# KarypisLab/SLIM

Measured on AMD Instinct MI355X. Metric: item-columns solved/sec (whole node), higher is better.
Workload: dtype f32

## Files before the change

### slim_amd/csrc/cd_gramr.hpp

```cpp
#pragma once
#include <utility>

#include "cd_tile.hpp"
#include "gram_pack.hpp"

#ifndef SLIM_GRAMR_AUX
#define SLIM_GRAMR_AUX 0
#endif
#ifndef SLIM_GRAMR_PROF
#define SLIM_GRAMR_PROF 0
#endif
#ifndef SLIM_GRAMR_FROM_PLANES
#define SLIM_GRAMR_FROM_PLANES 1
#endif
#ifndef SLIM_GRAMR_PREFETCH
#define SLIM_GRAMR_PREFETCH 0
#endif
#ifndef SLIM_GRAMR_LATE_GATHERS
#define SLIM_GRAMR_LATE_GATHERS 1
#endif
#ifndef SLIM_GRAMR_DRAIN
#define SLIM_GRAMR_DRAIN 0
#endif
#ifndef SLIM_GRAMR_SYNCROW
#define SLIM_GRAMR_SYNCROW 0
#endif

namespace slimamd {

typedef float gramr_v16 __attribute__((ext_vector_type(16)));

template <int N>
struct GramrRegs {
  gramr_v16 v;
  GramrRegs<N - 1> rest;
};
template <>
struct GramrRegs<0> {};
template <int I, int N>
__device__ __forceinline__ gramr_v16& gramr_reg(GramrRegs<N>& r) {
  if constexpr (I == 0) return r.v;
  else return gramr_reg<I - 1>(r.rest);
}
template <class F, int... Is>
__device__ __forceinline__ void static_for_impl(F&& f, std::integer_sequence<int, Is...>) {
  (f(std::integral_constant<int, Is>{}), ...);
}
template <int N, class F>
__device__ __forceinline__ void static_for(F&& f) {
  static_for_impl(f, std::make_integer_sequence<int, N>{});
}

template <int N, int KRA>
__device__ __forceinline__ float gramr_sel_from(GramrRegs<KRA>& gr, const int k, const int e) {
  if (k == N) {
    const gramr_v16 t = gramr_reg<N>(gr);
    asm volatile("" ::"v"(t));
    return t[e];
  }
  if constexpr (N + 1 < KRA) return gramr_sel_from<N + 1, KRA>(gr, k, e);
  return 0.0f;
}
template <int KRA>
__device__ __forceinline__ float gramr_sel(GramrRegs<KRA>& gr, const int k, const int e) {
  return gramr_sel_from<0, KRA>(gr, k, e);
}

#ifndef SLIM_GRAMR_ASMEXPORT
#define SLIM_GRAMR_ASMEXPORT 1
#endif
#define SLIM_GRAMR_EXPORT_ASM                                   \
  "s_mov_b32 %[sm0], m0\n\t"                                   \
  "s_mov_b64 %[sx], exec\n"                                     \
  "1:\n\t"                                                      \
  "s_ff1_i32_b64 %[sb], %[mine]\n\t"                            \
  "v_readlane_b32 %[sr], %[r], %[sb]\n\t"                       \
  "s_bitset0_b64 %[mine], %[sb]\n\t"                            \
  "s_bfe_u32 %[sl], %[sr], 0x60004\n\t"                         \
  "s_lshr_b32 %[sidx], %[sr], 13\n\t"                           \
  "s_and_b32 %[sr], %[sr], 15\n\t"                              \
  "s_lshl4_add_u32 %[sidx], %[sidx], %[sr]\n\t"                 \
  "s_set_gpr_idx_on %[sidx], gpr_idx(SRC0)\n\t"                 \
  "v_mov_b32 %[vt], v16\n\t"                                    \
  "s_set_gpr_idx_off\n\t"                                       \
  "v_readlane_b32 %[sv], %[vt], %[sl]\n\t"                      \
  "s_lshl_b64 exec, 1, %[sb]\n\t"                               \
  "v_mov_b32 %[res], %[sv]\n\t"                                 \
  "s_mov_b64 exec, %[sx]\n\t"                                   \
  "s_cmp_lg_u64 %[mine], 0\n\t"                                 \
  "s_cbranch_scc1 1b\n\t"                                       \
  "s_mov_b32 m0, %[sm0]\n"
#define SLIM_GRAMR_EXPORT_OUT                                                                           \
  [res] "+v"(res), [mine] "+s"(mine), [sb] "=&s"(sb), [sr] "=&s"(sr), [sl] "=&s"(sl), [sidx] "=&s"(sidx), \
      [sv] "=&s"(sv), [vt] "=&v"(vt), [sm0] "=&s"(sm0), [sx] "=&s"(sx)
template <int KRA>
__device__ __forceinline__ float gramr_export(GramrRegs<KRA>& gr, const int r, uint64_t mine) {
  float res = 0.0f, vt;
  int sb, sr, sl, sidx, sm0;
  float sv;
  uint64_t sx;
  static_assert(KRA == 1 || KRA == 3 || KRA == 6 || KRA == 10, "one operand list per instantiation");
  if constexpr (KRA == 1) {
    asm volatile(SLIM_GRAMR_EXPORT_ASM : SLIM_GRAMR_EXPORT_OUT : [r] "v"(r), "{v[16:31]}"(gramr_reg<0>(gr)) : "scc");
  } else if constexpr (KRA == 3) {
    asm volatile(SLIM_GRAMR_EXPORT_ASM
                 : SLIM_GRAMR_EXPORT_OUT
                 : [r] "v"(r), "{v[16:31]}"(gramr_reg<0>(gr)), "{v[32:47]}"(gramr_reg<1>(gr)),
                   "{v[48:63]}"(gramr_reg<2>(gr))
                 : "scc");
  } else if constexpr (KRA == 6) {
    asm volatile(SLIM_GRAMR_EXPORT_ASM
                 : SLIM_GRAMR_EXPORT_OUT
                 : [r] "v"(r), "{v[16:31]}"(gramr_reg<0>(gr)), "{v[32:47]}"(gramr_reg<1>(gr)),
                   "{v[48:63]}"(gramr_reg<2>(gr)), "{v[64:79]}"(gramr_reg<3>(gr)), "{v[80:95]}"(gramr_reg<4>(gr)),
                   "{v[96:111]}"(gramr_reg<5>(gr))
                 : "scc");
  } else {
    asm volatile(SLIM_GRAMR_EXPORT_ASM
                 : SLIM_GRAMR_EXPORT_OUT
                 : [r] "v"(r), "{v[16:31]}"(gramr_reg<0>(gr)), "{v[32:47]}"(gramr_reg<1>(gr)),
                   "{v[48:63]}"(gramr_reg<2>(gr)), "{v[64:79]}"(gramr_reg<3>(gr)), "{v[80:95]}"(gramr_reg<4>(gr)),
                   "{v[96:111]}"(gramr_reg<5>(gr)), "{v[112:127]}"(gramr_reg<6>(gr)),
                   "{v[128:143]}"(gramr_reg<7>(gr)), "{v[144:159]}"(gramr_reg<8>(gr)),
                   "{v[160:175]}"(gramr_reg<9>(gr))
                 : "scc");
  }
  return res;
}

constexpr int gramr_ring_bytes(int ah) { return (kGramrNT / 64) * (ah + 2) * 1024; }
constexpr int kGramrHdr = 1280;
constexpr int kGramrDump = SLIM_GRAMR_PREFETCH ? 256 : 0;
constexpr int gramr_hdr_bytes() { return (kGramrNT / 64) * (2 * kGramrHdr + kGramrDump); }

template <int KR, int KL, bool DMA = false, int WPS = ((KR <= 2 && KL == 0) ? 4 : 2), int AH = 2>
__global__ __launch_bounds__(kGramrNT, WPS) void cd_gramr_kernel(
    const DevMatrix A, const SolveArgs S, const GramPacked P) {
  constexpr int NT = kGramrNT, K = KR + KL;
  constexpr int kGramrAhead = AH, kGramrSlots = AH + 2;
  constexpr int KRA = KR > 0 ? KR : 1;
  constexpr int R0 = KR * kPackGroup;
  static_assert(KR <= 12, "register select covers 12 groups");
  static_assert(KR + KL <= 16, "one base byte per group in a 16-byte load");
  extern __shared__ __attribute__((aligned(16))) float g_lds[];
  __shared__ float s_gB[2][64];
  __shared__ int s_p, s_na;
  __shared__ unsigned long long s_D;
  __shared__ double s_e2[64], s_reg[64];
  __shared__ unsigned long long s_off;
  __shared__ int s_nz;

  const int tid = threadIdx.x;
  const int lane = tid & 63;
  const int wave = uni(tid >> 6);
  const int ncols = A.ncols;
#if !SLIM_GRAMR_FROM_PLANES
  const int n4 = S.ncols_pad >> 2;
#endif
  const int nchunks = P.nchunks;
  const float l1 = S.l1, l2 = S.l2;
#if !SLIM_GRAMR_FROM_PLANES
  const float* __restrict__ Gm = S.G;
  const int64_t ld = S.G_ld;
#endif
  float* const x = S.xslab + (int64_t)blockIdx.x * S.x_stride;
#if !SLIM_GRAMR_FROM_PLANES
  float4* const x4 = reinterpret_cast<float4*>(x);
#endif
  float4* const gl4 = reinterpret_cast<float4*>(g_lds);
  const int64_t* __restrict__ colptr = A.colptr;

  GramrRegs<KRA> gr;

  const uint32_t voff0 = 16u * (uint32_t)tid;
  const uint32_t vlast = 16u * (uint32_t)(nchunks - 1);
#if SLIM_GRAMR_DRAIN
#define SLIM_VMCNT(n) __builtin_amdgcn_s_waitcnt(0 | (7 << 4) | (15 << 8))
#else
#define SLIM_VMCNT(n) __builtin_amdgcn_s_waitcnt(((n) & 15) | (((n) >> 4) << 14) | (7 << 4) | (15 << 8))
#endif
  char* const ring_w = reinterpret_cast<char*>(g_lds) + KL * kPackGroup * 4 + wave * (kGramrSlots * 1024);
#if SLIM_GRAMR_PROF
  unsigned long long pt_first_v = 0, pt_mark_v = 0, pt_export_v = 0, pt_mark = 0;
  unsigned long long* const pt_first_p = &pt_first_v;
  unsigned long long* const pt_mark_p = &pt_mark_v;
#endif
  char* const hdr_w = reinterpret_cast<char*>(g_lds) + KL * kPackGroup * 4 + (DMA ? gramr_ring_bytes(AH) : 0) +
                      wave * (2 * kGramrHdr + kGramrDump);
  char* const dump_w = hdr_w + 2 * kGramrHdr;
  auto apply = [&](const uint8_t* __restrict__ plo, const uint8_t* __restrict__ phi,
                   const uint8_t* __restrict__ ph2, const uint8_t* __restrict__ pbase, const int hk,
                   const int h2k, const int cdiag, const int ediag, const float vdiag,
                   const float nd, const int rg, uint32_t (&gq)[4],
                   const uint8_t* __restrict__ plo_next) __attribute__((always_inline)) {
    const bool gin1 = rg < hk * kPackGroup, gin2 = rg < h2k * kPackGroup;
    auto gathers = [&]() __attribute__((always_inline)) {
      gq[0] = __hip_atomic_load(plo + rg, __ATOMIC_RELAXED, __HIP_MEMORY_SCOPE_WAVEFRONT);
      gq[1] = __hip_atomic_load(phi + (gin1 ? rg : 0), __ATOMIC_RELAXED, __HIP_MEMORY_SCOPE_WAVEFRONT);
      gq[2] = __hip_atomic_load(ph2 + (gin2 ? rg : 0), __ATOMIC_RELAXED, __HIP_MEMORY_SCOPE_WAVEFRONT);
      gq[3] = __hip_atomic_load(pbase + (((rg >> 4) & (NT - 1)) * 16 + (rg >> 13)), __ATOMIC_RELAXED,
                                __HIP_MEMORY_SCOPE_WAVEFRONT);
    };
    if constexpr (!(DMA && SLIM_GRAMR_LATE_GATHERS)) gathers();
    const int kdiag = cdiag / NT, tdiag = cdiag % NT;
    uint32_t bwords[4];
    if constexpr (DMA) {
      uint32_t vzb = voff0;
      asm volatile("" : "+v"(vzb));
      __builtin_amdgcn_global_load_lds(pbase + vzb, ring_w + (kGramrAhead + 1) * 1024, 16, 0, 0);
    } else {
      const uint4 bw = ld_off<uint4>(pbase, voff0);
      bwords[0] = bw.x;
      bwords[1] = bw.y;
      bwords[2] = bw.z;
      bwords[3] = bw.w;
    }
    auto consume = [&](auto kc, const uint4 lo, auto&& hi_of) __attribute__((always_inline)) {
      constexpr int k = decltype(kc)::value;
      float f[16];
      unpack16(lo, f);
      {
        typedef float gramr_v2 __attribute__((ext_vector_type(2)));
        const float bf = 16.0f * (float)((bwords[(k >> 2) & 3] >> (8 * (k & 3))) & 255u);
#pragma unroll
        for (int e = 0; e < 16; e += 2) {
          gramr_v2 v = {f[e], f[e + 1]};
          asm volatile("" : "+v"(v));
          v += (gramr_v2)(bf);
          f[e] = v.x;
          f[e + 1] = v.y;
        }
      }
      if (k < hk) {
        unpack16_add(hi_of(), 256.0f, f);
        if (k < h2k) {
          uint32_t vz = voff0;
          asm volatile("" : "+v"(vz));
          const uint32_t vo = min(vz + (uint32_t)(kPackGroup * k), vlast);
          unpack16_add(ld_off<uint4>(ph2, vo), 65536.0f, f);
        }
      }
      if (k == kdiag && tid == tdiag) {
#pragma unroll
        for (int e = 0; e < 16; ++e) f[e] = e == ediag ? vdiag : f[e];
      }
      if constexpr (k < KR) {
        gramr_v16& g = gramr_reg<k>(gr);
#pragma unroll
        for (int e = 0; e < 16; ++e) g[e] = fmaf(nd, f[e], g[e]);
        asm volatile("" : "+v"(g));
      } else {
        float4* const gp = gl4 + (k - KR) * 4 * NT + tid;
#pragma unroll
        for (int j = 0; j < 4; ++j) {
          float4 v = gp[j * NT];
          v.x = fmaf(nd, f[4 * j + 0], v.x);
          v.y = fmaf(nd, f[4 * j + 1], v.y);
          v.z = fmaf(nd, f[4 * j + 2], v.z);
          v.w = fmaf(nd, f[4 * j + 3], v.w);
          gp[j * NT] = v;
        }
      }
    };
    if constexpr (DMA) {
      constexpr int S = kGramrAhead + 1;
      uint4 h01[2];
      static_for<2>([&](auto kc) __attribute__((always_inline)) {
        constexpr int k = decltype(kc)::value;
        if constexpr (k < K) {
          if (k < hk) h01[k] = ld_off<uint4>(phi, min(voff0 + (uint32_t)(kPackGroup * k), vlast));
        }
      });
      auto request = [&](auto kc) __attribute__((always_inline)) {
        constexpr int k = decltype(kc)::value;
        uint32_t vz = voff0;
        asm volatile("" : "+v"(vz));
        const uint32_t vo = min(vz + (uint32_t)(kPackGroup * k), vlast);
        __builtin_amdgcn_global_load_lds(plo + vo, ring_w + (k % S) * 1024, 16, 0, SLIM_GRAMR_AUX);
      };
      static_for<(kGramrAhead < K ? kGramrAhead : K)>([&](auto kc) __attribute__((always_inline)) { request(kc); });
      constexpr int kLate = (SLIM_GRAMR_LATE_GATHERS ? 4 : 0) + (SLIM_GRAMR_PREFETCH ? 1 : 0);
      if constexpr (SLIM_GRAMR_LATE_GATHERS) gathers();
      if constexpr (SLIM_GRAMR_PREFETCH) {
        const int ln = lane < 8 * kGramrAhead ? lane : 0;
        const uint32_t po = min((uint32_t)(kPackGroup * (ln >> 3)) + 1024u * (uint32_t)wave + 128u * (uint32_t)(ln & 7), vlast);
        __builtin_amdgcn_global_load_lds(plo_next + po, dump_w, 4, 0, 0);
      }
      static_for<K>([&](auto kc) __attribute__((always_inline)) {
        constexpr int k = decltype(kc)::value;
        if constexpr (k + kGramrAhead < K) request(std::integral_constant<int, k + kGramrAhead>{});
        constexpr int ahead = (K - 1 - k) < kGramrAhead ? (K - 1 - k) : kGramrAhead;
        SLIM_VMCNT(ahead + (k < kGramrAhead ? kLate : 0));
        asm volatile("" ::: "memory");
        if constexpr (k == 0) {
          const uint4 bw = *reinterpret_cast<const uint4*>(ring_w + (kGramrAhead + 1) * 1024 + lane * 16);
          bwords[0] = bw.x;
          bwords[1] = bw.y;
          bwords[2] = bw.z;
          bwords[3] = bw.w;
        }
#if SLIM_GRAMR_PROF
        if constexpr (k == 0) *pt_first_p += __builtin_readcyclecounter() - *pt_mark_p;
#endif
        const uint4 lo = *reinterpret_cast<const uint4*>(ring_w + (k % S) * 1024 + lane * 16);
        consume(kc, lo, [&]() __attribute__((always_inline)) -> uint4 {
          if constexpr (k < 2) return h01[k];
          else {
            uint32_t vz = voff0;
            asm volatile("" : "+v"(vz));
            return ld_off<uint4>(phi, min(vz + (uint32_t)(kPackGroup * k), vlast));
          }
        });
        __builtin_amdgcn_sched_barrier(0);
      });
    } else {
      constexpr int GRP = 4;
      static_for<(K + GRP - 1) / GRP>([&](auto k0c) __attribute__((always_inline)) {
        constexpr int k0 = decltype(k0c)::value * GRP;
        uint4 l[GRP], h[GRP];
        static_for<GRP>([&](auto uc) __attribute__((always_inline)) {
          constexpr int u = decltype(uc)::value, k = k0 + u;
          if constexpr (k < K) {
            const uint32_t vo = min(voff0 + (uint32_t)(kPackGroup * k), vlast);
            l[u] = ld_off<uint4>(plo, vo);
            if (k < hk) h[u] = ld_off<uint4>(phi, vo);
          }
        });
        __builtin_amdgcn_sched_barrier(0);
        static_for<GRP>([&](auto uc) __attribute__((always_inline)) {
          constexpr int u = decltype(uc)::value, k = k0 + u;
          if constexpr (k < K)
            consume(std::integral_constant<int, k>{}, l[u], [&]() __attribute__((always_inline)) -> uint4 { return h[u]; });
          __builtin_amdgcn_sched_barrier(0);
        });
      });
    }
  };
#undef SLIM_VMCNT
  int nrows_read = 0, nhi16_read = 0;
  auto lds_index = [&](const int r) __attribute__((always_inline)) -> int {
    const int rr = r - R0;
    const int kk = rr >> 13, t = (rr >> 4) & (NT - 1), e = rr & 15;
    return ((kk * 4 + (e >> 2)) * NT + t) * 4 + (e & 3);
  };

  int gb_par = 0;
  auto fetch_g = [&](const bool want, const int r) __attribute__((always_inline)) -> float {
    float* const gb = s_gB[gb_par];
    gb_par ^= 1;
    const bool in_lds = r >= R0;
    const bool my_wave = (((r >> 4) & (NT - 1)) >> 6) == wave;
    if (KR > 0) {
      uint64_t mine = __ballot(want && !in_lds && my_wave);
#if SLIM_GRAMR_ASMEXPORT
      if (mine) {
        const bool own = want && !in_lds && my_wave;
        const float res = gramr_export<KRA>(gr, r, mine);
        if (own) gb[lane] = res;
      }
#else
      while (mine) {
        const int b = __builtin_ctzll(mine);
        mine &= mine - 1ull;
        const int rb = lane_bcast(r, b);
        const float v = gramr_sel<KRA>(gr, rb >> 13, rb & 15);
        if (lane == ((rb >> 4) & 63)) gb[b] = v;
      }
#endif
    }
    if (KL > 0 && want && in_lds && my_wave) gb[lane] = g_lds[lds_index(r)];
#if SLIM_GRAMR_PROF
    pt_export_v += __builtin_readcyclecounter() - pt_mark;
#endif
    asm volatile("" ::: "memory");
    __builtin_amdgcn_s_waitcnt(15 | (7 << 4) | (0 << 8) | (3 << 14));
    __builtin_amdgcn_s_barrier();
    asm volatile("" ::: "memory");
    return gb[lane];
  };

  for (;;) {
    if (tid == 0) {
      s_p = atomicAdd(S.queue, 1);
      s_na = 0;
      s_D = 0;
    }
    __syncthreads();
    const int p = s_p;
    if (p >= S.nwork) break;
    const int item = uni(S.order[p]);
    const int grp = p >> 5;
    const uint32_t gkey = (uint32_t)(grp * S.shard_count + S.shard_index);
    const int* __restrict__ ul = S.ulist + (int64_t)grp * S.u_stride;
    const int nunion = uni(S.tile_nunion[grp]);
#if SLIM_GRAMR_FROM_PLANES
    uint4 irec;
    {
      const uint4 mr = P.meta[item];
      irec = make_uint4(uni(mr.x), uni(mr.y), uni(mr.z), uni(mr.w));
    }
#endif
#if !SLIM_GRAMR_FROM_PLANES
    const float* __restrict__ arow = Gm + (int64_t)item * ld;
#endif

#if SLIM_GRAMR_FROM_PLANES
    {
      const int hk0 = (int)((irec.x >> 17) & 15u), h2k0 = (int)((irec.x >> 21) & 15u);
      const uint8_t* __restrict__ plo0 = P.lo + (int64_t)item * P.ldb;
      const uint8_t* __restrict__ phi0 = P.hi + (int64_t)irec.y * kPackGroup;
      const uint8_t* __restrict__ ph20 = phi0 + (int64_t)hk0 * kPackGroup;
      const uint8_t* __restrict__ pb0 = P.base + (int64_t)item * kPackGroup;
      int na = 0;
      int64_t dact = 0;
      for (int c = tid; c < nchunks; c += NT) {
        const int kg = c / NT;
        float f[16];
        unpack16(*reinterpret_cast<const uint4*>(plo0 + 16 * (int64_t)c), f);
        const float bf = 16.0f * (float)pb0[(c & (NT - 1)) * 16 + kg];
#pragma unroll
        for (int e = 0; e < 16; ++e) f[e] += bf;
        if (kg < hk0) unpack16_add(*reinterpret_cast<const uint4*>(phi0 + 16 * (int64_t)c), 256.0f, f);
        if (kg < h2k0) unpack16_add(*reinterpret_cast<const uint4*>(ph20 + 16 * (int64_t)c), 65536.0f, f);
        const int4* __restrict__ io = reinterpret_cast<const int4*>(P.item_of + 16 * (int64_t)c);
#pragma unroll
        for (int j = 0; j < 4; ++j) {
          const int4 q = io[j];
          const int it[4] = {q.x, q.y, q.z, q.w};
#pragma unroll
          for (int u = 0; u < 4; ++u) {
            if (it[u] >= 0) {
              const bool act = it[u] != item && f[4 * j + u] > l1;
              x[it[u]] = act ? 0.0f : kInactive;
              if (act) {
                ++na;
                dact += (int64_t)P.meta[it[u]].z;
              }
            }
          }
        }
      }
      na = (int)wave_sum((float)na);
      if (lane == 0 && na) atomicAdd(&s_na, na);
      if (dact) atomicAdd(&s_D, (unsigned long long)dact);
    }
#else
    {
      const float4* __restrict__ a4 = reinterpret_cast<const float4*>(arow);
      int na = 0;
      int64_t dact = 0;
      for (int c = tid; c < n4; c += NT) {
        const float4 a = a4[c];
        const int i0 = c << 2;
        float4 xs;
        const bool a0 = i0 + 0 < ncols && i0 + 0 != item && a.x > l1;
        const bool a1 = i0 + 1 < ncols && i0 + 1 != item && a.y > l1;
        const bool a2 = i0 + 2 < ncols && i0 + 2 != item && a.z > l1;
        const bool a3 = i0 + 3 < ncols && i0 + 3 != item && a.w > l1;
        xs.x = a0 ? 0.0f : kInactive;
        xs.y = a1 ? 0.0f : kInactive;
        xs.z = a2 ? 0.0f : kInactive;
        xs.w = a3 ? 0.0f : kInactive;
        na += (int)a0 + (int)a1 + (int)a2 + (int)a3;
        x4[c] = xs;
        if (a0 | a1 | a2 | a3) {
          const int64_t c0 = colptr[i0], c1 = colptr[i0 + 1];
          const int64_t c2 = i0 + 2 <= ncols ? colptr[i0 + 2] : c1, c3 = i0 + 3 <= ncols ? colptr[i0 + 3] : c2;
          const int64_t c4 = i0 + 4 <= ncols ? colptr[i0 + 4] : c3;
          dact += (a0 ? c1 - c0 : 0) + (a1 ? c2 - c1 : 0) + (a2 ? c3 - c2 : 0) + (a3 ? c4 - c3 : 0);
        }
      }
      na = (int)wave_sum((float)na);
      if (lane == 0 && na) atomicAdd(&s_na, na);
      if (dact) atomicAdd(&s_D, (unsigned long long)dact);
    }
#endif
    int64_t fe = 0, we = 0;
    auto warm_x = [&]() __attribute__((always_inline)) {
      if (S.icolptr != nullptr && item < S.incols) {
        __syncthreads();
        fe = uni(S.icolptr[item]);
        we = uni(S.icolptr[item + 1]);
        for (int64_t e = fe + tid; e < we; e += NT) {
          const int k = S.icolind[e];
          if (k < ncols && tile_active(x[k])) {
            const float v = S.icolval[e];
            x[k] = v < 0.0f ? 0.0f : v;
          }
        }
      }
    };
    warm_x();
    constexpr bool kCarry = K <= kGramrCarryMaxGroups;
    const bool carried = kCarry && S.g_load != nullptr;
    if (carried) {
      const float4* __restrict__ gs = reinterpret_cast<const float4*>(S.g_load + (int64_t)item * S.g_stride);
      static_for<KRA>([&](auto kc) __attribute__((always_inline)) {
        constexpr int k = decltype(kc)::value;
        gramr_v16 v;
#pragma unroll
        for (int j = 0; j < 4; ++j) {
          const float4 q = gs[(k * NT + tid) * 4 + j];
          v[4 * j] = q.x; v[4 * j + 1] = q.y; v[4 * j + 2] = q.z; v[4 * j + 3] = q.w;
        }
        gramr_reg<k>(gr) = v;
      });
#pragma unroll
      for (int k = 0; k < KL; ++k)
#pragma unroll
        for (int j = 0; j < 4; ++j) gl4[(k * 4 + j) * NT + tid] = gs[((KRA + k) * NT + tid) * 4 + j];
    } else {
    static_for<KRA>([&](auto kc) __attribute__((always_inline)) {
      gramr_reg<decltype(kc)::value>(gr) = (gramr_v16)(0.0f);
    });
#pragma unroll
    for (int k = 0; k < KL; ++k)
#pragma unroll
      for (int j = 0; j < 4; ++j) gl4[(k * 4 + j) * NT + tid] = make_float4(0.f, 0.f, 0.f, 0.f);
    }
    __syncthreads();

    int maxit = 0;
    {
      const int64_t cap = 50 * (uni(colptr[item + 1]) - uni(colptr[item]));
      maxit = cap < (int64_t)S.maxniters ? (int)cap : S.maxniters;
    }
    int niters = 0, conv = 0;
    nrows_read = 0;
    nhi16_read = 0;

    if (wave == 0) {
      s_e2[lane] = 0.0;
      s_reg[lane] = 0.0;
    }
    int phase = 0;
    bool init_row = !carried;
    if (carried) fe = we;
    int t = 0, p0 = 0;
    float dlt = 0.0f;
    PermCtx pc = perm_make(1u, 0u);
    int i_a = 0;
    int i_n = 0;
    int hw = 0;
    auto header_a = [&](const int q0) __attribute__((always_inline)) {
      const int pos = q0 + lane;
      i_a = pos < nunion ? ul[perm_index(pc, (uint32_t)pos)] : -1;
    };
    auto header_b = [&]() __attribute__((always_inline)) {
      i_n = i_a < 0 ? 0 : i_a;
      char* const hb = hdr_w + hw * kGramrHdr;
      __builtin_amdgcn_global_load_lds(x + i_n, hb, 4, 0, 0);
      __builtin_amdgcn_global_load_lds(P.meta + i_n, hb + 256, 16, 0, 0);
      hw ^= 1;
    };
    int ib = 0, wpos = 0, nz = 0;
    unsigned long long off = 0;
    bool fits = false;
    unsigned long long Uu = 0;
#if SLIM_GRAMR_PROF
    unsigned long long pt_fetch = 0, pt_dec = 0, pt_apply = 0;
    pt_first_v = 0;
    pt_export_v = 0;
#define SLIM_PT(acc) { const unsigned long long now_ = __builtin_readcyclecounter(); acc += now_ - pt_mark; pt_mark = now_; }
#else
#define SLIM_PT(acc)
#endif

    for (;;) {
      bool want = false;
      int r = 0, i = 0;
      uint4 mrow = make_uint4(0u, 0u, 0u, 0u);
      float xi = kInactive;
      bool part = false, keep = false;
      uint64_t mkeep = 0;
      if (phase == 1) {
        i = i_n;
        __builtin_amdgcn_s_waitcnt(0 | (7 << 4) | (15 << 8));
        asm volatile("" ::: "memory");
        {
          const char* const hcur = hdr_w + (hw ^ 1) * kGramrHdr;
          const bool valid = p0 + lane < nunion;
          int lz = lane;
          asm volatile("" : "+v"(lz));
          const float xv = *reinterpret_cast<const float*>(hcur + lz * 4);
          mrow = *reinterpret_cast<const uint4*>(hcur + 256 + lz * 16);
          r = (int)(mrow.x & 0x1FFFFu);
          xi = valid ? xv : kInactive;
        }
        asm volatile("" ::: "memory");
        part = tile_active(xi);
        header_b();
        header_a(p0 + 128);
        want = part;
      } else if (phase == 2) {
        i = ib + lane;
        xi = i < ncols ? x[i] : kInactive;
        const bool act = tile_active(xi);
        keep = act && fabsf(xi) > kEps;
        if (act && wave == 0)
          s_reg[lane] += 0.5 * (double)l2 * (double)xi * (double)xi + (double)l1 * (double)fabsf(xi);
        mkeep = __ballot(keep);
        if (mkeep == 0) {
          ib += 64;
          if (ib >= ncols) break;
          continue;
        }
        r = keep ? (int)(P.meta[i].x & 0x1FFFFu) : 0;
        want = keep;
      }
#if SLIM_GRAMR_PROF
      pt_mark = __builtin_readcyclecounter();
#endif
      const float g0 = fetch_g(want, r);
      SLIM_PT(pt_fetch)
      float gi = g0;
      uint64_t pend = 0;
      if (phase == 1) {
        pend = __ballot(part);
      }
      for (;;) {
        int row = 0;
        float nd = 0.0f;
        uint4 rec = make_uint4(0u, 0u, 0u, 0u);
        if (phase == 0) {
          bool have = false;
          if (init_row) {
            row = item;
            nd = 1.0f;
            have = true;
          } else {
            while (fe < we) {
              const int kk = uni(S.icolind[fe]);
              ++fe;
              if (kk < ncols) {
                const float xk = uni(x[kk]);
                if (xk > kEps) {
                  row = kk;
                  nd = -xk;
                  have = true;
                  break;
                }
              }
            }
          }
          if (!have) break;
        } else if (phase == 1) {
          if (pend == 0) break;
          const float xeff = (xi > kEps || xi < -kEps) ? xi : 0.0f;
          const float sq = __uint_as_float(mrow.w);
          const float cn = sqrtf(sq);
          const float num = cd_num(gi, xeff, sq);
          const float nx = num > l1 ? (num - l1) / cd_den(cn, l2) : 0.0f;
          const float neff = (nx > kEps || nx < -kEps) ? nx : 0.0f;
          const float d = neff - xeff;
          const uint64_t m = __ballot(part && nx != xi) & pend;
          if (m == 0) break;
          const int f = __builtin_ctzll(m);
          const float d_f = lane_bcast(d, f);
          const float nx_f = lane_bcast(nx, f), xi_f = lane_bcast(xi, f);
          dlt = fmaf(nx_f - xi_f, nx_f - xi_f, dlt);
          row = lane_bcast(i, f);
          if (wave == 0 && lane == f) x[row] = nx;
          pend = f == 63 ? 0ull : (pend & ~((2ull << f) - 1ull));
          if (d_f == 0.0f) continue;
          nd = -d_f;
          rec.x = (uint32_t)lane_bcast((int)mrow.x, f);
          rec.y = (uint32_t)lane_bcast((int)mrow.y, f);
          rec.z = (uint32_t)lane_bcast((int)mrow.z, f);
          rec.w = (uint32_t)lane_bcast((int)mrow.w, f);
          Uu += (unsigned long long)rec.z;
        } else {
          break;
        }
        if (phase == 0) {
          const uint4 mr = P.meta[row];
          rec.x = uni(mr.x);
          rec.y = uni(mr.y);
          rec.z = uni(mr.z);
          rec.w = uni(mr.w);
        }
        const int hk = (int)((rec.x >> 17) & 15u), h2k = (int)((rec.x >> 21) & 15u);
        const uint8_t* __restrict__ plo = P.lo + (int64_t)row * P.ldb;
        const uint8_t* __restrict__ phi = P.hi + (int64_t)rec.y * kPackGroup;
        const uint8_t* __restrict__ ph2 = phi + (int64_t)hk * kPackGroup;
        const uint8_t* __restrict__ pbase = P.base + (int64_t)row * kPackGroup;
        const bool in1 = r < hk * kPackGroup, in2 = r < h2k * kPackGroup;
        uint32_t gq[4];
        const int rdiag = (int)(rec.x & 0x1FFFFu);
        SLIM_PT(pt_dec)
#if SLIM_GRAMR_PROF
        pt_mark_v = pt_mark;
#endif
        const uint8_t* __restrict__ plo_next = plo;
        if (SLIM_GRAMR_PREFETCH && phase == 1) {
          const uint64_t cand = __ballot(part && xi != 0.0f) & pend;
          if (cand) plo_next = P.lo + (int64_t)lane_bcast(i, __builtin_ctzll(cand)) * P.ldb;
        }
        apply(plo, phi, ph2, pbase, hk, h2k, rdiag >> 4, rdiag & 15, __uint_as_float(rec.w), nd, r, gq, plo_next);
        float gsel = (float)gq[0] + 16.0f * (float)gq[3];
        gsel = in1 ? fmaf(256.0f, (float)gq[1], gsel) : gsel;
        gsel = in2 ? fmaf(65536.0f, (float)gq[2], gsel) : gsel;
        if (init_row) {
          init_row = false;
        } else {
          ++nrows_read;
          nhi16_read += min(hk * (kPackGroup / 16), nchunks) + min(h2k * (kPackGroup / 16), nchunks);
        }
        gi = fmaf(nd, gsel, gi);
#if SLIM_GRAMR_SYNCROW
        __syncthreads();
#endif
        SLIM_PT(pt_apply)
      }
      if (phase == 1) {
        p0 += 64;
        if (p0 < nunion) continue;
        if (dlt < S.opt_tol) {
          conv = 1;
          niters = t + 1;
        } else {
          ++t;
        }
      } else if (phase == 2) {
        if (keep) {
#if SLIM_GRAMR_FROM_PLANES
          float aty = 0.0f;
          if (wave == 0) {
            const int hk0 = (int)((irec.x >> 17) & 15u), h2k0 = (int)((irec.x >> 21) & 15u);
            const uint8_t* __restrict__ plo0 = P.lo + (int64_t)item * P.ldb;
            const uint8_t* __restrict__ phi0 = P.hi + (int64_t)irec.y * kPackGroup;
            const uint8_t* __restrict__ ph20 = phi0 + (int64_t)hk0 * kPackGroup;
            const uint8_t* __restrict__ pb0 = P.base + (int64_t)item * kPackGroup;
            const bool j1 = r < hk0 * kPackGroup, j2 = r < h2k0 * kPackGroup;
            aty = (float)plo0[r] + 16.0f * (float)pb0[((r >> 4) & (NT - 1)) * 16 + (r >> 13)];
            if (j1) aty = fmaf(256.0f, (float)phi0[r], aty);
            if (j2) aty = fmaf(65536.0f, (float)ph20[r], aty);
          }
          if (wave == 0) s_e2[lane] += (double)xi * ((double)aty + (double)g0);
#else
          if (wave == 0) s_e2[lane] += (double)xi * ((double)arow[i] + (double)g0);
#endif
          if (fits && wave == 0) {
            const int64_t dst = (int64_t)off + wpos + __popcll(mkeep & ((1ull << lane) - 1ull));
            S.out_ind[dst] = i;
            S.out_val[dst] = xi;
          }
        }
        wpos += __popcll(mkeep);
        ib += 64;
        if (ib >= ncols) break;
        continue;
      }
      bool sweep = false;
      if (!conv) {
        if (t >= maxit) {
          niters = maxit + 1;
        } else if (nunion == 0) {
          conv = 1;
          niters = t + 1;
        } else {
          sweep = true;
        }
      }
      if (sweep) {
        __syncthreads();
        phase = 1;
        p0 = 0;
        dlt = 0.0f;
        pc = perm_make((uint32_t)nunion, perm_key(S.seed, gkey, (uint32_t)t));
        header_a(0);
        header_b();
        header_a(64);
        continue;
      }
      if (wave == 0) {
        int cnt = 0;
        for (int jb = 0; jb < ncols; jb += 64) {
          const int j = jb + lane;
          const float xv = j < ncols ? x[j] : kInactive;
          cnt += __popcll(__ballot(tile_active(xv) && fabsf(xv) > kEps));
        }
        if (lane == 0) {
          s_off = atomicAdd(S.out_cursor, (unsigned long long)cnt);
          s_nz = cnt;
        }
      }
      __syncthreads();
      off = s_off;
      nz = s_nz;
      fits = (int64_t)(off + (unsigned long long)nz) <= S.out_cap;
      phase = 2;
      ib = 0;
      wpos = 0;
      if (ncols <= 0) break;
    }
    if (kCarry && S.g_save != nullptr) {
      float4* __restrict__ gs = reinterpret_cast<float4*>(S.g_save + (int64_t)item * S.g_stride);
      static_for<KRA>([&](auto kc) __attribute__((always_inline)) {
        constexpr int k = decltype(kc)::value;
        const gramr_v16 v = gramr_reg<k>(gr);
#pragma unroll
        for (int j = 0; j < 4; ++j)
          gs[(k * NT + tid) * 4 + j] = make_float4(v[4 * j], v[4 * j + 1], v[4 * j + 2], v[4 * j + 3]);
      });
#pragma unroll
      for (int k = 0; k < KL; ++k)
#pragma unroll
        for (int j = 0; j < 4; ++j) gs[((KRA + k) * NT + tid) * 4 + j] = gl4[(k * 4 + j) * NT + tid];
    }
    if (wave == 0) {
      double e2 = s_e2[lane], reg = s_reg[lane];
      for (int o = 32; o > 0; o >>= 1) {
        e2 += __shfl_xor(e2, o);
        reg += __shfl_xor(reg, o);
      }
      if (lane == 0) {
        const float err = (float)(0.5 * ((double)A.csq[item] - e2));
        if (!fits) atomicMax(S.overflow, 1);
        S.out_cnt[item] = fits ? nz : -nz - 1;
        S.out_off[item] = (int64_t)off;
        S.st_na[item] = s_na;
        S.st_sweeps[item] = niters;
        S.st_conv[item] = conv;
#if SLIM_GRAMR_PROF
        S.st_D[item] = (int64_t)pt_fetch;
        S.st_U[item] = (int64_t)pt_dec;
        S.st_B[item] = (int64_t)pt_apply;
        S.st_G[item] = (int)(pt_first_v >> 8);
        S.st_na[item] = (int)(pt_export_v >> 8);
#else
        S.st_D[item] = (int64_t)s_D * (int64_t)(conv ? niters : maxit);
        S.st_U[item] = (int64_t)Uu;
        S.st_G[item] = nrows_read;
        S.st_B[item] = (int64_t)nrows_read * (P.ldb + 16 * (int64_t)(nchunks < NT ? nchunks : NT)) + (int64_t)nhi16_read * 16 +
                       ((carried ? 4 : 0) + (kCarry && S.g_save != nullptr ? 4 : 0)) * S.g_stride;
#endif
        S.st_err[item] = err;
        S.st_obj[item] = err + (float)reg;
      }
    }
    __syncthreads();
  }
}

constexpr int kGramrUnionNT = 256;
#ifdef SLIM_GRAM_PACK_KERNELS
__global__ __launch_bounds__(kGramrUnionNT) void gramr_union_kernel(const DevMatrix A, const SolveArgs S,
                                                                     const GramPacked P) {
  constexpr int NT = kGramrUnionNT;
  constexpr int kWords = kGramrMaxGroups * kPackGroup / 32;
  __shared__ uint32_t s_bits[kWords];
  __shared__ int s_scan[NT];
  const int tid = threadIdx.x;
  const int grp = blockIdx.x;
  const int base = grp * 32;
  const int nprob = (S.nwork - base) < 32 ? (S.nwork - base) : 32;
  const int ncols = A.ncols;
  const int nwords = (ncols + 31) >> 5;
  const int nchunks = P.nchunks;
  int* __restrict__ ul = S.ulist + (int64_t)grp * S.u_stride;
  for (int w = tid; w < nwords; w += NT) s_bits[w] = 0u;
  __syncthreads();
  for (int q = 0; q < nprob; ++q) {
    const int it0 = uni(S.order[base + q]);
    const uint4 mr = P.meta[it0];
    const uint32_t rx = uni(mr.x), ry = uni(mr.y);
    const int hk = (int)((rx >> 17) & 15u), h2k = (int)((rx >> 21) & 15u);
    const uint8_t* __restrict__ plo = P.lo + (int64_t)it0 * P.ldb;
    const uint8_t* __restrict__ phi = P.hi + (int64_t)ry * kPackGroup;
    const uint8_t* __restrict__ ph2 = phi + (int64_t)hk * kPackGroup;
    const uint8_t* __restrict__ pb = P.base + (int64_t)it0 * kPackGroup;
    for (int c = tid; c < nchunks; c += NT) {
      const int kg = c / kGramrNT;
      float f[16];
      unpack16(*reinterpret_cast<const uint4*>(plo + 16 * (int64_t)c), f);
      const float bf = 16.0f * (float)pb[(c & (kGramrNT - 1)) * 16 + kg];
#pragma unroll
      for (int e = 0; e < 16; ++e) f[e] += bf;
      if (kg < hk) unpack16_add(*reinterpret_cast<const uint4*>(phi + 16 * (int64_t)c), 256.0f, f);
      if (kg < h2k) unpack16_add(*reinterpret_cast<const uint4*>(ph2 + 16 * (int64_t)c), 65536.0f, f);
      const int4* __restrict__ io = reinterpret_cast<const int4*>(P.item_of + 16 * (int64_t)c);
#pragma unroll
      for (int j = 0; j < 4; ++j) {
        const int4 qv = io[j];
        const int it[4] = {qv.x, qv.y, qv.z, qv.w};
#pragma unroll
        for (int u = 0; u < 4; ++u)
          if (it[u] >= 0 && it[u] != it0 && f[4 * j + u] > S.l1) atomicOr(&s_bits[it[u] >> 5], 1u << (it[u] & 31));
      }
    }
  }
  __syncthreads();
  const int W = (nwords + NT - 1) / NT;
  const int w0 = tid * W, w1 = min(nwords, w0 + W);
  int cnt = 0;
  for (int w = w0; w < w1; ++w) cnt += __popc(s_bits[w]);
  s_scan[tid] = cnt;
  __syncthreads();
  for (int o = 1; o < NT; o <<= 1) {
    const int v = tid >= o ? s_scan[tid - o] : 0;
    __syncthreads();
    s_scan[tid] += v;
    __syncthreads();
  }
  int pos = s_scan[tid] - cnt;
  for (int w = w0; w < w1; ++w) {
    uint32_t b = s_bits[w];
    while (b) {
      const int j = __builtin_ctz(b);
      b &= b - 1u;
      ul[pos++] = (w << 5) + j;
    }
  }
  if (tid == NT - 1) S.tile_nunion[grp] = s_scan[tid];
}
#endif

}
```

### slim_amd/csrc/cd_wave.hpp

```cpp
#pragma once
#include <hip/hip_runtime.h>

#include <cstdint>

#include "cd_perm.hpp"

namespace slimamd {

struct DevMatrix {
  int32_t nrows, ncols;
  int64_t nnz;
  const int64_t* rowptr;
  const int32_t* rowind;
  const float* rowval;
  const int64_t* colptr;
  const int32_t* colind;
  const float* colval;
  const float* cnorm;
  const float* csq;
};

struct SolveArgs {
  float l1, l2, opt_tol;
  int32_t maxniters;
  uint32_t seed;
  int32_t nnbrs;
  int32_t simtype;
  const int32_t* order;
  int32_t nwork;
  int32_t* queue;
  const int64_t* icolptr;
  const int32_t* icolind;
  const float* icolval;
  int32_t incols;
  float* slab;
  int64_t slab_stride;
  int32_t nrows_pad, ncols_pad;
  float* xslab;
  int64_t x_stride;
  int32_t* ulist;
  int64_t u_stride;
  int32_t ngroups;
  uint64_t* trace;
  int32_t cluster;
  const int32_t* ubounds;
  const int64_t* csplit;
  unsigned long long* mailbox;
  float* atypart;
  int32_t exact_gram;
  int32_t bm_shift, bm_words;
  int32_t nheavy;
  int32_t cluster_hi;
  const int32_t* ubounds_hi;
  const int64_t* csplit_hi;
  unsigned long long* mailbox_hi;
  int32_t* queue_hi;
  int64_t nnz_last;
  int32_t hi_prefetch;
  int32_t shard_count, shard_index;
  int32_t xcd_swizzle;
  float* gram;
  int32_t gram_mode;
  float* G;
  int64_t G_ld;
  int32_t* tile_nunion;
  const int32_t* gram_pos;
  int32_t gram_bits;
  int32_t gram_split_stride;
  int32_t gram_accum;
  const uint4* gview;
  const int64_t* gview_base;
  const uint16_t* gview_cnt;
  int32_t gview_ngroups;
  int32_t gview_range0;
  int32_t gview_sentinel;
  int32_t gram_part16;
  float* g_save;
  const float* g_load;
  int64_t g_stride;
  int32_t* out_cnt;
  int64_t* out_off;
  int32_t* out_ind;
  float* out_val;
  unsigned long long* out_cursor;
  int64_t out_cap;
  int32_t* overflow;
  int32_t* st_na;
  int32_t* st_sweeps;
  int32_t* st_conv;
  int64_t* st_G;
  int64_t* st_D;
  int64_t* st_U;
  int64_t* st_B;
  float* st_err;
  float* st_obj;
};

constexpr float kEps = 1e-7f;


__device__ __forceinline__ float cd_num(float g, float xeff, float sq) {
  float p = xeff * sq;
  asm volatile("" : "+v"(p));
  return g + p;
}
__device__ __forceinline__ float cd_den(float cn, float l2) { return fmaf(cn, cn, l2); }
__device__ __forceinline__ int uni(int v) { return __builtin_amdgcn_readfirstlane(v); }
__device__ __forceinline__ uint32_t uni(uint32_t v) {
  return (uint32_t)__builtin_amdgcn_readfirstlane((int)v);
}
__device__ __forceinline__ float uni(float v) {
  return __int_as_float(__builtin_amdgcn_readfirstlane(__float_as_int(v)));
}
__device__ __forceinline__ int64_t uni(int64_t v) {
  uint32_t lo = uni((uint32_t)v), hi = uni((uint32_t)((uint64_t)v >> 32));
  return (int64_t)(((uint64_t)hi << 32) | lo);
}
__device__ __forceinline__ int lane_bcast(int v, int src) {
  return __builtin_amdgcn_readlane(v, src);
}
__device__ __forceinline__ float lane_bcast(float v, int src) {
  return __int_as_float(__builtin_amdgcn_readlane(__float_as_int(v), src));
}
__device__ __forceinline__ int64_t lane_bcast(int64_t v, int src) {
  uint32_t lo = (uint32_t)__builtin_amdgcn_readlane((int)(uint32_t)v, src);
  uint32_t hi = (uint32_t)__builtin_amdgcn_readlane((int)(uint32_t)((uint64_t)v >> 32), src);
  return (int64_t)(((uint64_t)hi << 32) | lo);
}

template <int CTRL>
__device__ __forceinline__ float dpp_mov(float v) {
  return __int_as_float(
      __builtin_amdgcn_update_dpp(0, __float_as_int(v), CTRL, 0xF, 0xF, true));
}

__device__ __forceinline__ float wave_sum(float v) {
  v += dpp_mov<0xB1>(v);
  v += dpp_mov<0x4E>(v);
  v += dpp_mov<0x141>(v);
  v += dpp_mov<0x140>(v);
  return (lane_bcast(v, 0) + lane_bcast(v, 16)) + (lane_bcast(v, 32) + lane_bcast(v, 48));
}

template <bool USE_LDS>
__device__ __forceinline__ void wave_sync() {
  if (USE_LDS) {
    __builtin_amdgcn_fence(__ATOMIC_ACQ_REL, "wavefront");
    __builtin_amdgcn_wave_barrier();
  } else {
    __builtin_amdgcn_fence(__ATOMIC_ACQ_REL, "workgroup");
    __builtin_amdgcn_wave_barrier();
  }
}


template <bool USE_LDS, bool HAS_VAL>
__global__ __launch_bounds__(64) void cd_wave_kernel(const DevMatrix A, const SolveArgs S) {
  extern __shared__ __attribute__((aligned(16))) char smem[];
  const int lane = threadIdx.x;
  const uint64_t lane_lt = (1ull << lane) - 1ull;

  float* r;
  float* aty;
  float* x;
  if (USE_LDS) {
    r = reinterpret_cast<float*>(smem);
  } else {
    r = S.slab + (int64_t)blockIdx.x * S.slab_stride;
  }
  aty = r + S.nrows_pad;
  x = aty + S.ncols_pad;
  int* ids = reinterpret_cast<int*>(aty);

  const int nrows = A.nrows, ncols = A.ncols;
  const float l1 = S.l1, l2 = S.l2;

  for (;;) {
    int w = 0;
    if (lane == 0) w = atomicAdd(S.queue, 1);
    w = uni(w);
    if (w >= S.nwork) break;
    const int iC = uni(S.order[w]);
    const int64_t cs = uni(A.colptr[iC]), ce = uni(A.colptr[iC + 1]);

    for (int u = lane; u < nrows; u += 64) r[u] = 0.0f;
    for (int i = lane; i < ncols; i += 64) aty[i] = 0.0f;
    wave_sync<USE_LDS>();

    int64_t G = 0;
    if (S.exact_gram) {
      for (int64_t j = cs + lane; j < ce; j += 64) {
        const int u = A.colind[j];
        r[u] = HAS_VAL ? A.colval[j] : 1.0f;
        G += A.rowptr[u + 1] - A.rowptr[u];
      }
      for (int off = 32; off > 0; off >>= 1) G += __shfl_xor(G, off);
      wave_sync<USE_LDS>();
      for (int ib = 0; ib < ncols; ib += 64) {
        const int i = ib + lane;
        float acc = 0.0f;
        if (i < ncols) {
          const int64_t s = A.colptr[i], e = A.colptr[i + 1];
          bool co = false;
          for (int64_t k = s; k < e; ++k) {
            const float yv = r[A.colind[k]];
            acc += (HAS_VAL ? A.colval[k] : 1.0f) * yv;
            co = co || yv != 0.0f;
          }
          aty[i] = (acc == 0.0f && co) ? -0.0f : acc;
        }
      }
    } else {
    for (int64_t jb = cs; jb < ce; jb += 64) {
      const int64_t j = jb + lane;
      const bool ok = j < ce;
      const int u_l = ok ? A.colind[j] : 0;
      const float v_l = ok ? (HAS_VAL ? A.colval[j] : 1.0f) : 0.0f;
      const int64_t rs_l = ok ? A.rowptr[u_l] : 0;
      const int64_t re_l = ok ? A.rowptr[u_l + 1] : 0;
      if (ok) r[u_l] = v_l;
      const int cnt = (int)((ce - jb) < 64 ? (ce - jb) : 64);
      for (int k = 0; k < cnt; ++k) {
        const int64_t rs = lane_bcast(rs_l, k), re = lane_bcast(re_l, k);
        const float v = lane_bcast(v_l, k);
        G += re - rs;
        for (int64_t e = rs + lane; e < re; e += 64) {
          const float rv = HAS_VAL ? A.rowval[e] : 1.0f;
          atomicAdd(&aty[A.rowind[e]], v * rv);
        }
      }
    }
    }
// ... 238 lines not shown
```

### slim_amd/csrc/engine.hip

```cpp
#include <hip/hip_runtime.h>

#include <algorithm>
#include <atomic>
#include <chrono>
#include <cmath>
#include <cstdio>
#include <cstdlib>
#include <cstring>
#include <functional>
#include <mutex>
#include <new>
#include <numeric>
#include <memory>
#include <string>
#include <thread>

#include <rocprim/device/device_radix_sort.hpp>

#include "tile_inst.hpp"
#include "gram_inst.hpp"
#include "gramr_inst.hpp"
#include "fslim_gram_inst.hpp"
#include "cd_wave.hpp"
#include "engine.hpp"
#include "hip_check.hpp"
#include "host_csr.hpp"

inline uint64_t slimgpu_next_uid() {
  static std::atomic<uint64_t> n{0};
  return ++n;
}

using slimamd::DeviceBuffer;

struct UserSplit {
  DeviceBuffer<int32_t> ubounds;
  DeviceBuffer<int64_t> csplit;
  int32_t nranges = 0, max_rows = 0;
};

struct slimgpu_matrix {
  const uint64_t uid = slimgpu_next_uid();
  int device = 0;
  hipStream_t stream = nullptr;
  int32_t nrows = 0, ncols = 0;
  int64_t nnz = 0;
  bool binary = false;
  bool owns_csr = false;
  bool exact_gram = false;
  bool nonpositive = false;
  bool merged = false;
  int64_t* d_rowptr = nullptr;
  int32_t* d_rowind = nullptr;
  float* d_rowval = nullptr;
  DeviceBuffer<int64_t> d_colptr;
  DeviceBuffer<int32_t> d_colind;
  DeviceBuffer<float> d_colval, d_cnorm, d_csq;
  std::vector<int64_t> h_cost;
  std::vector<int64_t> h_rowptr;
  UserSplit split[6];
  UserSplit gsplit;
  double setup_ms = 0;
  int num_cus = 256;
  std::vector<slimgpu_matrix*> replicas;
  DeviceBuffer<float> ws_gram;
  std::vector<int32_t> gram_order;
  int gram_geom[6] = {0, 0, 0, 0, 0, 0};
  DeviceBuffer<float> ws_G;
  DeviceBuffer<int32_t> ws_nunion;
  int64_t G_ld = 0;
  bool G_ready = false;
  double G_build_ms = 0, G_alloc_ms = 0, G_sums_ms = 0, G_sums_kernel_ms = 0, G_pack_ms = 0;
  DeviceBuffer<uint8_t> ws_Glo, ws_Ghi, ws_Gbase;
  DeviceBuffer<float> ws_Gdiag;
  DeviceBuffer<uint4> ws_Gmeta;
  DeviceBuffer<int64_t> ws_hioff, ws_hi2off;
  DeviceBuffer<int32_t> ws_hik, ws_hi2k, ws_rankof, ws_itemof;
  int64_t Gp_ldb = 0, Gp_pool_bytes = 0;
  int32_t Gp_nchunks = 0;
  bool Gp_ready = false, Gp_tried = false;
  bool Gf_dropped = false;
  double Gp_bytes_per_row = 0;
  int expect_solves = 0;
  std::vector<int32_t> last_order;
  DeviceBuffer<int32_t> ws_order, ws_cnt, ws_stat_i, ws_misc, ws_arena_i, ws_ulist;
  DeviceBuffer<int64_t> ws_off, ws_stat_l, ws_icolptr;
  DeviceBuffer<float> ws_stat_f, ws_arena_v, ws_slab, ws_xslab, ws_part, ws_icolval;
  DeviceBuffer<int32_t> ws_fn, ws_fid, ws_fslot;
  DeviceBuffer<float> ws_faty;
  DeviceBuffer<uint64_t> ws_trace;
  DeviceBuffer<uint4> ws_gview;
  DeviceBuffer<int64_t> ws_gvbase;
  DeviceBuffer<int32_t> ws_gvrows;
  DeviceBuffer<uint16_t> ws_gvcnt;
  DeviceBuffer<unsigned long long> ws_mailbox;
  DeviceBuffer<int32_t> ws_icolind;
  DeviceBuffer<uint32_t> ws_tkeys[2];
  DeviceBuffer<uint64_t> ws_tpay[2];
  DeviceBuffer<uint8_t> ws_ttmp;

  ~slimgpu_matrix() {
    (void)hipSetDevice(device);
    if (owns_csr) {
      (void)hipFree(d_rowptr);
      (void)hipFree(d_rowind);
      (void)hipFree(d_rowval);
    }
  }
};

struct slimgpu_model {
  int device = 0;
  int32_t n = 0;
  int64_t nnz = 0;
  int32_t max_row = 0;
  bool rows_sorted = true;
  DeviceBuffer<int64_t> d_colptr, d_rowptr;
  DeviceBuffer<int32_t> d_colind, d_rowind;
  DeviceBuffer<float> d_colval, d_rowval;
  mutable DeviceBuffer<float> d_gsave;
  mutable bool gsave_valid = false;
  int64_t gsave_stride = 0;
  double gsave_l1 = 0;
  uint64_t gsave_owner = 0;
  std::thread fetcher;
  bool fetch_begun = false;
  slim_csr_t* fetched = nullptr;
  int32_t fetch_status = 0;
  std::string fetch_error;
  double fetch_ms = 0;

  ~slimgpu_model() { (void)hipSetDevice(device); }
};

namespace slimamd {

namespace {

thread_local slimgpu_stats_t g_stats;
thread_local ColumnStats g_colstats;

struct InputError {
  std::string msg;
};

double now_ms() {
  using namespace std::chrono;
  return duration<double, std::milli>(steady_clock::now().time_since_epoch()).count();
}

void report(const HipFail& e, const char* what) {
  set_error(std::string(what) + ": HIP error '" + hipGetErrorString(e.code) + "' in " + e.where +
            " -- the SLIM CD path needs a gfx950 GPU; there is no CPU fallback");
}

void drop_screen_cache(slimgpu_matrix* m) {
  m->ws_gram.reset();
  m->gram_order.clear();
}

auto evict_cache(slimgpu_matrix* m) {
  return [m] {
    if (!m->ws_gram.get()) return false;
    drop_screen_cache(m);
    return true;
  };
}


__global__ void k_gview_rows(const int32_t* __restrict__ order, int32_t nwork, const int64_t* __restrict__ csplit,
                             int32_t stride, int32_t ngroups, int32_t nblocks, int32_t* __restrict__ rows,
                             uint16_t* __restrict__ cnt) {
  const int b = (int)blockIdx.x * ((int)blockDim.x >> 6) + ((int)threadIdx.x >> 6);
  if (b >= nblocks) return;
  const int r = b / ngroups, pl = (b % ngroups) * 64 + ((int)threadIdx.x & 63);
  int len = 0;
  if (pl < nwork) {
    const int64_t* const c = csplit + (int64_t)order[pl] * stride + r;
    len = (int)(c[1] - c[0]);
  }
  int n = (len + 7) >> 3;
  cnt[(int64_t)b * 64 + (threadIdx.x & 63)] = (uint16_t)n;
  for (int off = 32; off > 0; off >>= 1) n += __shfl_xor(n, off);
  if ((threadIdx.x & 63) == 0) rows[b] = n;
}

__global__ void k_gview_fill(const int32_t* __restrict__ order, int32_t nwork, const int64_t* __restrict__ csplit,
                             int32_t stride, const int32_t* __restrict__ ubounds, const int32_t* __restrict__ ci,
                             int32_t ngroups, int32_t nblocks, const int64_t* __restrict__ base, uint32_t sentinel,
                             uint4* __restrict__ view) {
  const int b = (int)blockIdx.x * ((int)blockDim.x >> 6) + ((int)threadIdx.x >> 6);
  if (b >= nblocks) return;
  const int lane = (int)threadIdx.x & 63;
  const int r = b / ngroups, pl = (b % ngroups) * 64 + lane;
  const int64_t end = base[b + 1];
  const int32_t u0 = ubounds[r];
  int64_t cs = 0;
  int len = 0;
  if (pl < nwork) {
    const int64_t* const c = csplit + (int64_t)order[pl] * stride + r;
    cs = c[0];
    len = (int)(c[1] - cs);
  }
  int64_t at = base[b];
  for (int c = 0;; ++c) {
    const bool mine = 8 * c < len;
    const uint64_t who = __ballot(mine);
    if (who == 0ull) break;
    if (mine) {
      const int64_t slot = at + __popcll(who & ((1ull << lane) - 1ull));
      uint32_t id[8];
#pragma unroll
      for (int j = 0; j < 8; ++j) id[j] = 8 * c + j < len ? (uint32_t)(ci[cs + 8 * c + j] - u0) : sentinel;
      if (slot < end)
        view[slot] = make_uint4(id[0] | (id[1] << 16), id[2] | (id[3] << 16), id[4] | (id[5] << 16),
                                id[6] | (id[7] << 16));
    }
    at += __popcll(who);
  }
}


__global__ void k_max_index(const int32_t* __restrict__ ind, int64_t n, int32_t* out) {
  int32_t m = -1;
  for (int64_t k = (int64_t)blockIdx.x * blockDim.x + threadIdx.x; k < n;
       k += (int64_t)gridDim.x * blockDim.x)
    m = max(m, ind[k]);
  for (int off = 32; off > 0; off >>= 1) m = max(m, __shfl_xor(m, off));
  if ((threadIdx.x & 63) == 0) atomicMax(out, m);
}

constexpr int kBadRowptr = 1;
constexpr int kBadColumn = 2;
constexpr int kDupEntry = 4;

__global__ void k_pack_rows(int32_t nrows, int32_t ncols, int64_t nnz,
                            const int64_t* __restrict__ rowptr,
                            const int32_t* __restrict__ rowind,
// ... 479 lines not shown
  });
}

void matrix_free(slimgpu_matrix_t* m) { destroy(m); }

slimgpu_matrix_t* matrix_clone_to_device(const slimgpu_matrix_t* src, int32_t device,
                                         int32_t* status) {
  const double t0 = now_ms();
  return make_matrix("SLIMGPU_MatrixFromHost (device-to-device copy of the staged matrix)", status,
                     [&](slimgpu_matrix* m) {
    (void)hipGetLastError();
    LearnOptions o;
    o.device = device;
    pick_device(m, o);
    m->nrows = src->nrows;
    m->ncols = src->ncols;
    m->nnz = src->nnz;
    m->binary = src->binary;
    m->exact_gram = src->exact_gram;
    m->nonpositive = src->nonpositive;
    m->merged = src->merged;
    m->owns_csr = true;
    m->h_cost = src->h_cost;
    const size_t nz = (size_t)std::max<int64_t>(m->nnz, 1);
    m->d_rowptr = DeviceBuffer<int64_t>((size_t)m->nrows + 1).release();
    m->d_rowind = DeviceBuffer<int32_t>(nz).release();
    m->d_rowval = m->binary ? nullptr : DeviceBuffer<float>(nz).release();
    m->d_colptr = DeviceBuffer<int64_t>((size_t)m->ncols + 1);
    m->d_colind = DeviceBuffer<int32_t>(nz + 64);
    if (!m->binary) m->d_colval = DeviceBuffer<float>(nz);
    m->d_cnorm = DeviceBuffer<float>((size_t)m->ncols);
    m->d_csq = DeviceBuffer<float>((size_t)m->ncols);
    int can_peer = m->device == src->device ? 1 : 0;
    if (!can_peer) {
      if (hipDeviceCanAccessPeer(&can_peer, m->device, src->device) != hipSuccess) can_peer = 0;
      (void)hipGetLastError();
    }
    if (const char* e = std::getenv("SLIM_GPU_PEER")) can_peer = can_peer && std::atoi(e) != 0;
    void* bounce = nullptr;
    const size_t bounce_bytes = size_t(256) << 20;
    struct BounceFree {
      void** p;
      ~BounceFree() {
        if (*p) (void)hipHostFree(*p);
      }
    } bounce_guard{&bounce};
    auto peer = [&](void* dst, const void* from, size_t bytes) {
      if (bytes == 0 || !dst || !from) return;
      if (can_peer) {
        HIP_TRY(hipMemcpyPeerAsync(dst, m->device, from, src->device, bytes, m->stream));
        return;
      }
      if (!bounce) HIP_TRY(hipHostMalloc(&bounce, bounce_bytes, hipHostMallocDefault));
      for (size_t off = 0; off < bytes; off += bounce_bytes) {
        const size_t n = std::min(bounce_bytes, bytes - off);
        HIP_TRY(hipSetDevice(src->device));
        HIP_TRY(hipMemcpy(bounce, static_cast<const char*>(from) + off, n, hipMemcpyDeviceToHost));
        HIP_TRY(hipSetDevice(m->device));
        HIP_TRY(hipMemcpy(static_cast<char*>(dst) + off, bounce, n, hipMemcpyHostToDevice));
      }
    };
    peer(m->d_rowptr, src->d_rowptr, sizeof(int64_t) * ((size_t)m->nrows + 1));
    peer(m->d_colptr.get(), src->d_colptr.get(), sizeof(int64_t) * ((size_t)m->ncols + 1));
    peer(m->d_cnorm.get(), src->d_cnorm.get(), sizeof(float) * (size_t)m->ncols);
    peer(m->d_csq.get(), src->d_csq.get(), sizeof(float) * (size_t)m->ncols);
    if (m->nnz > 0) {
      peer(m->d_rowind, src->d_rowind, sizeof(int32_t) * (size_t)m->nnz);
      peer(m->d_colind.get(), src->d_colind.get(), sizeof(int32_t) * (size_t)m->nnz);
      peer(m->d_rowval, src->d_rowval, sizeof(float) * (size_t)m->nnz);
      peer(m->d_colval.get(), src->d_colval.get(), sizeof(float) * (size_t)m->nnz);
    }
    HIP_TRY(hipStreamSynchronize(m->stream));
    m->setup_ms = now_ms() - t0;
  });
}

void matrix_add_replica(slimgpu_matrix_t* m, slimgpu_matrix_t* replica) {
  m->replicas.push_back(replica);
}
const std::vector<slimgpu_matrix_t*>& matrix_replicas(const slimgpu_matrix_t* m) {
  return m->replicas;
}
void matrix_adopt_csr(slimgpu_matrix_t* m) { m->owns_csr = true; }
int32_t matrix_device(const slimgpu_matrix_t* m) { return m ? m->device : -1; }
void matrix_set_setup_ms(slimgpu_matrix_t* m, double ms) { m->setup_ms = ms; }

int32_t matrix_info(const slimgpu_matrix_t* m, int32_t* nrows, int32_t* ncols, int64_t* nnz) {
  if (!m) return SLIM_ERROR_INPUT;
  if (nrows) *nrows = m->nrows;
  if (ncols) *ncols = m->ncols;
  if (nnz) *nnz = m->nnz;
  return SLIM_OK;
}

double matrix_setup_ms(const slimgpu_matrix_t* m) { return m ? m->setup_ms : 0.0; }

void matrix_expect_solves(slimgpu_matrix_t* m, int32_t n) {
  if (!m) return;
  m->expect_solves = n;
  for (slimgpu_matrix* r : m->replicas) r->expect_solves = n;
}

int32_t matrix_column_cost(const slimgpu_matrix_t* m, int64_t* cost) {
  if (!m || !cost) return SLIM_ERROR_INPUT;
  std::memcpy(cost, m->h_cost.data(), sizeof(int64_t) * m->h_cost.size());
  return SLIM_OK;
}

int32_t matrix_get_column_view(const slimgpu_matrix_t* m, int64_t* colptr, int32_t* colind,
                               float* colval, float* cnorms) {
  if (!m) return SLIM_ERROR_INPUT;
  try {
    HIP_TRY(hipSetDevice(m->device));
    if (colptr)
      HIP_TRY(hipMemcpy(colptr, m->d_colptr.get(), sizeof(int64_t) * ((size_t)m->ncols + 1),
                        hipMemcpyDeviceToHost));
    if (colind && m->nnz)
      HIP_TRY(hipMemcpy(colind, m->d_colind.get(), sizeof(int32_t) * (size_t)m->nnz,
                        hipMemcpyDeviceToHost));
    if (colval && m->nnz && m->d_colval.get())
      HIP_TRY(hipMemcpy(colval, m->d_colval.get(), sizeof(float) * (size_t)m->nnz,
                        hipMemcpyDeviceToHost));
    if (cnorms)
      HIP_TRY(hipMemcpy(cnorms, m->d_cnorm.get(), sizeof(float) * (size_t)m->ncols,
                        hipMemcpyDeviceToHost));
    return SLIM_OK;
  } catch (const HipFail& e) {
    report(e, "SLIMGPU_MatrixGetColumnView");
    return status_of(e);
  }
}


namespace {

KernelFn pick_kernel(bool lds, bool has_val) {
  if (lds) return has_val ? cd_wave_kernel<true, true> : cd_wave_kernel<true, false>;
  return has_val ? cd_wave_kernel<false, true> : cd_wave_kernel<false, false>;
}

int round_up(int v, int q) { return (v + q - 1) / q * q; }

bool test_hook(const char* name) {
  const char* master = std::getenv("SLIM_GPU_TEST_HOOKS");
  return master && std::atoi(master) == 1 && std::getenv(name) != nullptr;
}

constexpr int kBitmapBytes = 64 * 1024;

}

namespace {

bool pack_gram(slimgpu_matrix* m) {
  if (std::getenv("SLIM_GPU_NO_GRAMR")) return false;
  m->Gp_tried = true;
  const int32_t ncols = m->ncols;
  hipStream_t st = m->stream;
  const double t0 = now_ms();
  std::vector<int64_t> cp((size_t)ncols + 1);
  HIP_TRY(hipMemcpy(cp.data(), m->d_colptr.get(), sizeof(int64_t) * cp.size(), hipMemcpyDeviceToHost));
  const int32_t nchunks = (ncols + 15) / 16;
  static_assert(kGramrMaxGroups <= 15 && kGramrMaxGroups * kPackGroup <= (1 << 17),
                "row record: 17 bits of rank, 4 bits per plane length; base bytes: 16 groups per thread");
  if ((nchunks + kGramrNT - 1) / kGramrNT > kGramrMaxGroups) return false;
  std::vector<int32_t> item_of((size_t)nchunks * 16, -1), rank_of((size_t)ncols);
  std::iota(item_of.begin(), item_of.begin() + ncols, 0);
  std::stable_sort(item_of.begin(), item_of.begin() + ncols, [&](int32_t a, int32_t b) {
    return cp[(size_t)a + 1] - cp[(size_t)a] > cp[(size_t)b + 1] - cp[(size_t)b];
  });
  for (int32_t r = 0; r < ncols; ++r) rank_of[(size_t)item_of[(size_t)r]] = r;
  int32_t* d_item_of = m->ws_itemof.reserve(item_of.size());
  int32_t* d_rank_of = m->ws_rankof.reserve(rank_of.size());
  HIP_TRY(hipMemcpyAsync(d_item_of, item_of.data(), sizeof(int32_t) * item_of.size(), hipMemcpyHostToDevice, st));
  HIP_TRY(hipMemcpyAsync(d_rank_of, rank_of.data(), sizeof(int32_t) * rank_of.size(), hipMemcpyHostToDevice, st));
  int32_t* d_hik = m->ws_hik.reserve((size_t)ncols + 1);
  int32_t* d_hi2k = m->ws_hi2k.reserve((size_t)ncols);
  int32_t* d_flag = d_hik + ncols;
  HIP_TRY(hipMemsetAsync(d_flag, 0, sizeof(int32_t), st));
  const float* dG = m->ws_G.get();
  int use_base = 1;
  if (const char* e = std::getenv("SLIM_GPU_PACK_BASE")) use_base = std::atoi(e) != 0;
  bool gather = false;
  if (const char* e = std::getenv("SLIM_GPU_PACK_GATHER")) gather = std::atoi(e) != 0;
  const dim3 tgrid(kGramrNT / kPackTS, (ncols + kPackJT - 1) / kPackJT);
  if (gather) {
    hipLaunchKernelGGL(gram_pack_scan_fn(), dim3(ncols), dim3(256), 0, st, dG, m->G_ld, ncols, d_item_of, nchunks,
                       use_base, d_hik, d_hi2k, d_flag);
    HIP_TRY(hipGetLastError());
  } else {
    HIP_TRY(hipMemsetAsync(d_hik, 0xff, sizeof(int32_t) * (size_t)ncols, st));
    HIP_TRY(hipMemsetAsync(d_hi2k, 0xff, sizeof(int32_t) * (size_t)ncols, st));
    hipLaunchKernelGGL(gram_pack_scan_t_fn(), tgrid, dim3(256), 0, st, dG, m->G_ld, ncols, d_item_of, d_rank_of,
                       nchunks, use_base, d_hik, d_hi2k, d_flag);
    HIP_TRY(hipGetLastError());
    hipLaunchKernelGGL(gram_pack_groups_fn(), dim3((ncols + 255) / 256), dim3(256), 0, st, ncols, d_hik, d_hi2k);
    HIP_TRY(hipGetLastError());
  }
  std::vector<int32_t> hk((size_t)ncols + 1), h2k((size_t)ncols);
  HIP_TRY(hipMemcpyAsync(hk.data(), d_hik, sizeof(int32_t) * hk.size(), hipMemcpyDeviceToHost, st));
  HIP_TRY(hipMemcpyAsync(h2k.data(), d_hi2k, sizeof(int32_t) * h2k.size(), hipMemcpyDeviceToHost, st));
  HIP_TRY(hipStreamSynchronize(st));
  if (hk[(size_t)ncols] != 0) return false;
  std::vector<int64_t> off1((size_t)ncols), off2((size_t)ncols);
  int64_t n1 = 0, n2 = 0, npool = 0;
  for (int32_t i = 0; i < ncols; ++i) {
    off1[(size_t)i] = npool;
    npool += (int64_t)hk[(size_t)i] * kPackGroup;
    off2[(size_t)i] = npool;
    npool += (int64_t)h2k[(size_t)i] * kPackGroup;
    n1 += (int64_t)hk[(size_t)i] * kPackGroup;
    n2 += (int64_t)h2k[(size_t)i] * kPackGroup;
  }
  const int64_t ldb = (int64_t)nchunks * 16;
  const size_t need = (size_t)ncols * ((size_t)ldb + kPackGroup) + (size_t)n1 + (size_t)n2 + 2 * (size_t)kPackGroup;
  size_t free_b = 0, total_b = 0;
  HIP_TRY(hipMemGetInfo(&free_b, &total_b));
  if (need + (size_t(4) << 30) > free_b + m->ws_Glo.bytes() + m->ws_Ghi.bytes() + m->ws_Gbase.bytes()) return false;
  uint8_t* d_lo = m->ws_Glo.reserve((size_t)ncols * (size_t)ldb);
  uint8_t* d_hi = m->ws_Ghi.reserve((size_t)npool + kPackGroup);
  uint8_t* d_hi2 = d_hi;
  uint8_t* d_base = m->ws_Gbase.reserve((size_t)ncols * kPackGroup);
  if (gather) {
    HIP_TRY(hipMemsetAsync(d_base, 0, (size_t)ncols * kPackGroup, st));
  }
  float* d_diag = m->ws_Gdiag.reserve((size_t)ncols);
  HIP_TRY(hipMemsetAsync(d_diag, 0, sizeof(float) * (size_t)ncols, st));
  int64_t* d_off1 = m->ws_hioff.reserve((size_t)ncols);
  int64_t* d_off2 = m->ws_hi2off.reserve((size_t)ncols);
  HIP_TRY(hipMemcpyAsync(d_off1, off1.data(), sizeof(int64_t) * off1.size(), hipMemcpyHostToDevice, st));
  HIP_TRY(hipMemcpyAsync(d_off2, off2.data(), sizeof(int64_t) * off2.size(), hipMemcpyHostToDevice, st));
  HIP_TRY(hipMemsetAsync(d_hi + npool, 0, kPackGroup, st));
  if (gather) {
    hipLaunchKernelGGL(gram_pack_write_fn(), dim3(ncols), dim3(256), 0, st, dG, m->G_ld, ncols, d_item_of, nchunks,
                       d_lo, ldb, d_hi, d_off1, d_hik, d_hi2, d_off2, d_hi2k, d_base, d_diag);
  } else {
    hipLaunchKernelGGL(gram_pack_write_t_fn(), tgrid, dim3(256), 0, st, dG, m->G_ld, ncols, d_item_of, d_rank_of,
                       nchunks, d_lo, ldb, d_hi, d_off1, d_hik, d_hi2, d_off2, d_hi2k, d_base, d_diag);
  }
  HIP_TRY(hipGetLastError());
  uint4* d_meta = m->ws_Gmeta.reserve((size_t)ncols);
  hipLaunchKernelGGL(gram_pack_meta_fn(), dim3((ncols + 255) / 256), dim3(256), 0, st, ncols, d_rank_of, d_hik,
                     d_hi2k, d_off1, d_diag, m->d_colptr.get(), m->d_csq.get(), m->d_cnorm.get(), d_meta, d_flag);
  HIP_TRY(hipGetLastError());
  int32_t meta_flag = 0;
  HIP_TRY(hipMemcpyAsync(&meta_flag, d_flag, sizeof(int32_t), hipMemcpyDeviceToHost, st));
  HIP_TRY(hipStreamSynchronize(st));
  if (meta_flag & 2) return false;
  m->Gp_ldb = ldb;
  m->Gp_pool_bytes = npool + kPackGroup;
  m->Gp_nchunks = nchunks;
  m->Gp_bytes_per_row = (double)ldb + 16.0 * std::min(nchunks, kGramrNT) + (double)(n1 + n2) / std::max(1, ncols);
  m->Gp_ready = true;
  if (const char* te = std::getenv("SLIM_GPU_TRACE"); te && std::atoi(te) >= 1)
    std::fprintf(stderr, "[trace] G packed (%s): lo %.2f GB + base %.2f GB + hi %.2f GB + hi2 %.3f GB = %.3f bytes per entry, %.1f ms\n",
                 gather ? "gathers" : "streamed tiles", (double)ncols * ldb * 1e-9, (double)ncols * kPackGroup * 1e-9, n1 * 1e-9, n2 * 1e-9,
                 m->Gp_bytes_per_row / std::max(1, ncols), now_ms() - t0);
  return true;
}

void drop_float_gram(slimgpu_matrix* m) {
  if (!m->Gp_ready || !m->ws_G.get() || std::getenv("SLIM_GPU_KEEP_G") || std::getenv("SLIM_GPU_NO_GRAMR")) return;
  if ((m->Gp_nchunks + kGramrNT - 1) / kGramrNT > kGramrMaxGroups) return;
  double min_gb = 8.0;
  if (const char* e = std::getenv("SLIM_GPU_DROP_G_MIN_GB")) min_gb = std::atof(e);
  if ((double)m->ws_G.bytes() < min_gb * 1073741824.0) return;
  (void)hipStreamSynchronize(m->stream);
  m->ws_G.reset();
  m->Gf_dropped = true;
}


struct Refusal {
  int32_t status;
  std::string msg;
};

int64_t gram_ld(int32_t ncols) { return round_up(round_up(ncols, 64), 64); }

struct WorkList {
  std::vector<int32_t> order;
  int32_t G_block = 0;
};

WorkList work_list(const slimgpu_matrix* m, const LearnOptions& opt, const int32_t* columns,
                   int32_t ncolumns) {
  const int32_t ncols = m->ncols;
  WorkList w;
  if (columns) {
    std::vector<char> seen((size_t)ncols, 0);
    for (int32_t k = 0; k < ncolumns; ++k) {
      if (columns[k] < 0 || columns[k] >= ncols || seen[(size_t)columns[k]])
        throw Refusal{SLIM_ERROR_INPUT, "SLIMGPU_LearnColumns: column ids must be distinct and inside [0, ncols)"};
      seen[(size_t)columns[k]] = 1;
    }
    w.order.assign(columns, columns + ncolumns);
  } else {
    int32_t cb = std::max(0, opt.col_begin);
    const int32_t ce = opt.col_end < 0 ? ncols : std::min(opt.col_end, ncols);
    if (cb > ce) cb = ce;
    w.order.resize((size_t)(ce - cb));
    std::iota(w.order.begin(), w.order.end(), cb);
  }
  if (opt.shard_index < 0 || opt.shard_index >= opt.shard_count)
    throw Refusal{SLIM_ERROR_INPUT, "SLIMGPU_Learn: shard index outside [0, shard count)"};
  std::vector<int32_t>& order = w.order;
  std::stable_sort(order.begin(), order.end(),
                   [&](int32_t a, int32_t b) { return m->h_cost[a] > m->h_cost[b]; });
  if (opt.shard_count > 1) {
    std::vector<int32_t> mine;
    for (int32_t t = 0; t < (int32_t)order.size(); ++t)
      if ((t / 32) % opt.shard_count == opt.shard_index) mine.push_back(order[(size_t)t]);
    order.swap(mine);
  }
  if (opt.build_G && opt.G_rows_end >= 0) {
    auto in_block = [&](int32_t c) { return c >= opt.G_rows_begin && c < opt.G_rows_end; };
    std::stable_partition(order.begin(), order.end(), in_block);
    w.G_block = (int32_t)std::count_if(order.begin(), order.end(), in_block);
  }
  return w;
}

int32_t build_gram(slimgpu_matrix* m, LearnOptions bo, bool zero_first, double* alloc_ms = nullptr) {
  if (zero_first) {
    const double t0 = now_ms();
    const int64_t G_ld = gram_ld(m->ncols);
    drop_screen_cache(m);
    float* dG = m->ws_G.reserve((size_t)m->ncols * (size_t)G_ld);
    if (alloc_ms) *alloc_ms = now_ms() - t0;
    HIP_TRY(hipMemsetAsync(dG, 0, sizeof(float) * (size_t)m->ncols * (size_t)G_ld, m->stream));
    m->G_ld = G_ld;
  }
  if (bo.G_rows_end >= 0 && bo.G_rows_begin == bo.G_rows_end) return SLIM_OK;
  bo.kernel = SLIMGPU_KERNEL_TILE;
  bo.build_G = true;
  bo.heavy_tiles = 0;
  int32_t st = SLIM_OK;
  if (slim_csr_t* none = learn_cd(m, bo, nullptr, &st, nullptr, 0, false)) csr_free(none);
  return st;
}

struct Path {
  int kernel = 0;
  bool use_gram = false, use_gramr = false, use_tile = false, use_lds = false;
  int nrows_pad = 0, ncols_pad = 0;
  size_t vec_floats = 0, lds_need = 0;
  int gram_nw = 0, gram_v = 0;
  GramrFn fn_r = nullptr;
  int gramr_kr = 0, gramr_kl = 0;
  size_t gram_lds = 0;
  KernelFn fn = nullptr;
  int tileP = 32, tileNW = 16;
  int req_cluster = 0;
  size_t gram_bits_lds = 0;
  int gram_passes = 1;
  int wg_slots = 0;
  int nwaves = 1;
  int trace_level = 0;
  bool has_imodel = false;
  bool exact_gram = false;
  bool use_fgram = false, f_block = false;
  int f_stride = 0, f_ustride = 0, f_tab_n = 0, f_waves = 1;
  size_t f_wave_lds = 0, f_union_lds = 0;
  FslimFn fn_f = nullptr;
};

Path choose_kernel(slimgpu_matrix* m, const LearnOptions& opt, int32_t nwork) {
  const int32_t ncols = m->ncols;
  Path p;
  p.nrows_pad = round_up(std::max(m->nrows, 1), 64);
  p.ncols_pad = round_up(ncols, 64);
  p.vec_floats = (size_t)p.nrows_pad + 2 * (size_t)p.ncols_pad;
  p.lds_need = p.vec_floats * sizeof(float);
  p.kernel = opt.kernel;
  const bool gram_fits =
      gram_geometry(p.ncols_pad, &p.gram_nw, &p.gram_v) && opt.nnbrs == 0 && !opt.build_G && ncols > 0;
  const size_t G_bytes = sizeof(float) * (size_t)ncols * (size_t)gram_ld(ncols);
  if (p.kernel == SLIMGPU_KERNEL_GRAM_FSLIM) {
    if (opt.nnbrs <= 0 || opt.build_G)
      throw Refusal{SLIM_ERROR_INPUT, "SLIMGPU_Learn: the item-space FSLIM kernel needs nnbrs > 0"};
    if (m->nonpositive)
      throw Refusal{SLIM_ERROR_INPUT, "SLIMGPU_Learn: the item-space FSLIM kernel needs ratings > 0: with a rating <= 0 "
                                      "a co-rating sum can cancel to 0 and G cannot mark the column as co-rated "
                                      "(the tile kernel solves such matrices)"};
    if (std::min(opt.nnbrs, ncols - 1) > kFslimMaxNbrs)
      throw Refusal{SLIM_ERROR_INPUT, "SLIMGPU_Learn: the item-space FSLIM kernel holds at most 4096 neighbours per "
                                      "problem in LDS (min(nnbrs, ncols - 1) is larger)"};
    if (m->G_ready && m->Gf_dropped) {
      m->G_ready = false;
      m->Gf_dropped = false;
    }
    size_t free_b = 0, total_b = 0;
    HIP_TRY(hipMemGetInfo(&free_b, &total_b));
    if (!m->G_ready && G_bytes + (size_t(4) << 30) > free_b + m->ws_gram.bytes())
      throw Refusal{SLIM_ERROR_MEMORY, "SLIMGPU_Learn: G = R^T R (4 ncols^2 bytes) does not fit the free HBM"};
    p.use_fgram = true;
    return p;
  }
  if (p.kernel == SLIMGPU_KERNEL_GRAM) {
    if (!gram_fits) throw Refusal{SLIM_ERROR_INPUT, "SLIMGPU_Learn: the item-space kernel has no FSLIM form"};
    size_t free_b = 0, total_b = 0;
    HIP_TRY(hipMemGetInfo(&free_b, &total_b));
    if (!m->G_ready && G_bytes + (size_t(4) << 30) > free_b + m->ws_gram.bytes())
      throw Refusal{SLIM_ERROR_MEMORY, "SLIMGPU_Learn: G = R^T R (4 ncols^2 bytes) does not fit the free HBM"};
    p.use_gram = true;
  } else if (p.kernel == SLIMGPU_KERNEL_AUTO && gram_fits && p.lds_need > 64 * 1024 &&
             !std::getenv("SLIM_GPU_NO_GRAMCD")) {
    const double rho = (double)ncols * (double)ncols / std::max(1.0, (double)m->nnz) / 45.0;
    const double solves = (double)std::max(1, m->expect_solves);
    const bool tile_geometry_asked = opt.cluster != 0 || opt.heavy_tiles >= 0 || opt.heavy_cluster != 0;
    bool item_space = rho < 1.0 && !tile_geometry_asked &&
                      (m->G_ready || (double)nwork * solves * (1.0 - rho) > (double)ncols / 32.0);
    if (const char* e = std::getenv("SLIM_GPU_GRAMCD"); e && std::strcmp(e, "never-first") == 0)
      item_space = item_space && (m->G_ready || m->expect_solves >= 2);
    if (item_space) {
      size_t free_b = 0, total_b = 0;
      HIP_TRY(hipMemGetInfo(&free_b, &total_b));
      p.use_gram = m->G_ready || G_bytes + (size_t(8) << 30) <= free_b + m->ws_gram.bytes();
    }
  }
  if (p.use_gram) p.kernel = SLIMGPU_KERNEL_GRAM;
  if (p.use_gram && m->G_ready && m->Gf_dropped && std::getenv("SLIM_GPU_NO_GRAMR")) {
    m->G_ready = false;
    m->Gf_dropped = false;
  }
  return p;
}

int32_t gram_for_solve(slimgpu_matrix* m, const LearnOptions& opt, int32_t trace_level, bool floats_only) {
  const double tb = now_ms();
  LearnOptions bo = opt;
  bo.col_begin = 0;
  bo.col_end = -1;
  bo.shard_count = 1;
  bo.shard_index = 0;
  bo.nnbrs = 0;
  bo.cluster = 0;
  bo.dbglvl = 0;
  double alloc_ms = 0;
  const int32_t st = build_gram(m, bo, true, &alloc_ms);
  if (st != SLIM_OK) return st;
  const double t_sums = now_ms();
  const double sums_kernel_ms = last_stats().kernel_ms;
  m->G_ready = true;
  m->Gf_dropped = false;
  if (!floats_only) {
    if (!m->Gp_ready) {
      m->Gp_tried = false;
      if (!pack_gram(m)) m->Gp_ready = false;
    }
    drop_float_gram(m);
  }
  m->G_build_ms = now_ms() - tb;
  m->G_alloc_ms = alloc_ms;
  m->G_sums_ms = t_sums - tb - alloc_ms;
  m->G_sums_kernel_ms = sums_kernel_ms;
  m->G_pack_ms = now_ms() - t_sums;
  if (trace_level >= 1)
    std::fprintf(stderr, "[trace] G = R^T R (%d x %d, %.2f GB) built in %.1f ms: allocation %.1f, sums %.1f "
                 "(kernel %.1f), byte planes %.1f\n", m->ncols, m->ncols,
                 sizeof(float) * (double)m->ncols * (double)m->G_ld * 1e-9, m->G_build_ms, m->G_alloc_ms,
                 m->G_sums_ms, sums_kernel_ms, m->G_pack_ms);
  return SLIM_OK;
}

void finish_path(slimgpu_matrix* m, const LearnOptions& opt, int32_t nwork, const slim_csr_t* imodel,
                 const slimgpu_model* warm_dev, Path& p) {
  p.exact_gram = m->exact_gram || std::getenv("SLIM_GPU_EXACT_GRAM") || (opt.nnbrs > 0 && m->nonpositive);
  if (p.kernel == SLIMGPU_KERNEL_AUTO)
    p.kernel = p.lds_need <= 64 * 1024 ? SLIMGPU_KERNEL_WAVE_LDS : SLIMGPU_KERNEL_TILE;
  if (p.kernel == SLIMGPU_KERNEL_WAVE_LDS && p.lds_need > 160 * 1024)
    throw Refusal{SLIM_ERROR_INPUT, "SLIMGPU_Learn: work vectors do not fit the 160 KiB LDS of a CU"};
  if (p.kernel < SLIMGPU_KERNEL_WAVE_LDS || p.kernel > SLIMGPU_KERNEL_GRAM_FSLIM)
    throw Refusal{SLIM_ERROR_INPUT, "SLIMGPU_Learn: unknown kernel selection"};
  if (p.use_fgram) {
    p.f_stride = std::max(64, round_up(std::min(opt.nnbrs, m->ncols - 1), 64));
    p.f_ustride = (int)std::min<int64_t>((int64_t)32 * p.f_stride, p.ncols_pad);
    p.f_block = p.f_stride <= kFslimBlockMaxStride;
    if (const char* e = std::getenv("SLIM_GPU_FSLIM_BLOCK")) p.f_block = p.f_block && std::atoi(e) != 0;
    p.f_tab_n = p.f_block ? round_up(p.f_ustride, 8) : 0;
    p.f_wave_lds = fslim_wave_lds(p.f_stride, p.f_block, p.f_tab_n);
    p.f_waves = (int)std::max<size_t>(1, std::min<size_t>(p.f_block ? kFslimMaxWaves : 4, (size_t(150) << 10) / p.f_wave_lds));
    p.fn_f = fslim_solve_fn(p.f_block);
    p.f_union_lds = fslim_union_lds(m->ncols);
    if (p.f_union_lds > (size_t(150) << 10))
      throw Refusal{SLIM_ERROR_INPUT, "SLIMGPU_Learn: the item-space FSLIM kernel's item bitmap does not fit the LDS of a CU"};
    HIP_TRY(hipFuncSetAttribute(reinterpret_cast<const void*>(fslim_union_fn()),
                                hipFuncAttributeMaxDynamicSharedMemorySize, (int)p.f_union_lds));
    const size_t lds = p.f_wave_lds * (size_t)p.f_waves;
    int per_cu = 0;
    HIP_TRY(hipFuncSetAttribute(reinterpret_cast<const void*>(p.fn_f), hipFuncAttributeMaxDynamicSharedMemorySize, (int)lds));
    HIP_TRY(hipOccupancyMaxActiveBlocksPerMultiprocessor(&per_cu, reinterpret_cast<const void*>(p.fn_f), 64 * p.f_waves, lds));
    if (per_cu < 1)
      throw Refusal{SLIM_ERROR, "SLIMGPU_Learn: the item-space FSLIM kernel does not fit a compute unit of this device"};
    p.nwaves = std::max(1, std::min((nwork + p.f_waves - 1) / p.f_waves, m->num_cus * per_cu));
    if (warm_dev && warm_dev->device != m->device)
      throw Refusal{SLIM_ERROR_INPUT, "SLIMGPU_LearnResident: the warm-start model lives on another device"};
    p.has_imodel = false;
    if (p.trace_level >= 1)
      std::fprintf(stderr, "[trace] item-space FSLIM: form %s, lists of %d, %d wavefronts per workgroup (%zu KB of LDS "
                   "each), %d workgroups per CU\n", p.f_block ? "block in LDS" : "gathered", p.f_stride, p.f_waves,
                   p.f_wave_lds >> 10, per_cu);
    return;
  }
  p.use_lds = p.kernel == SLIMGPU_KERNEL_WAVE_LDS;
  if (p.use_gram && p.gram_v == 0)
    if (const char* e = std::getenv("SLIM_GPU_GRAM_NW")) p.gram_nw = std::atoi(e) == 8 ? 8 : 16;
  if (p.use_gram && m->G_ready && !m->Gp_tried && !m->Gf_dropped) {
    (void)pack_gram(m);
    drop_float_gram(m);
  }
  size_t gramr_lds = 0;
  bool gramr_ring = false;
  int gramr_wps = 0;
  bool gramr_dma = (m->Gp_nchunks + kGramrNT - 1) / kGramrNT > 6;
  if (const char* e = std::getenv("SLIM_GPU_GRAMR_DMA")) gramr_dma = std::atoi(e) != 0;
  if (p.use_gram && m->Gp_ready && !std::getenv("SLIM_GPU_NO_GRAMR"))
    p.fn_r = gramr_kernel(m->Gp_nchunks, gramr_dma, &p.gramr_kr, &p.gramr_kl, &gramr_lds, &gramr_ring, &gramr_wps);
  p.use_gramr = p.fn_r != nullptr;
  if (p.use_gram && !p.use_gramr && m->Gf_dropped)
    throw Refusal{SLIM_ERROR, "SLIMGPU_Learn: the floats of G were dropped and the byte-plane kernel cannot run this solve"};
  if (p.use_gramr) {
    p.gram_nw = kGramrNT / 64;
    p.gram_v = 1;
  }
  p.gram_lds = p.use_gramr ? gramr_lds : (p.gram_v > 0 ? sizeof(float) * (size_t)p.ncols_pad : 0);
  if (p.use_gram && p.trace_level >= 1) {
    if (p.use_gramr)
      std::fprintf(stderr, "[trace] item-space kernel: packed <%d,%d>, %s loads, WPS %d\n", p.gramr_kr, p.gramr_kl,
                   gramr_ring ? "ring" : "register", gramr_wps);
    else
      std::fprintf(stderr, "[trace] item-space kernel: float <%d,%d>\n", p.gram_nw, p.gram_v);
  }
  p.tileP = p.kernel == SLIMGPU_KERNEL_TILE16 ? 16 : 32;
  if (p.kernel == SLIMGPU_KERNEL_TILE && ((int64_t)p.nrows_pad + 64) * 128 >= (int64_t(1) << 32)) p.tileP = 16;
  p.use_tile = p.kernel == SLIMGPU_KERNEL_TILE || p.kernel == SLIMGPU_KERNEL_TILE16;
  if (p.use_tile && ((int64_t)p.nrows_pad + 64) * 4 * p.tileP >= (int64_t(1) << 32)) {
    p.use_tile = false;
    p.kernel = SLIMGPU_KERNEL_WAVE_HBM;
  }
  if (p.use_tile && p.tileP == 16 && opt.nnbrs > 0) {
    p.use_tile = false;
    p.kernel = SLIMGPU_KERNEL_WAVE_HBM;
  }
  if (p.use_tile) p.kernel = p.tileP == 32 ? SLIMGPU_KERNEL_TILE : SLIMGPU_KERNEL_TILE16;
  if (opt.build_G && !p.use_tile)
    throw Refusal{SLIM_ERROR_INPUT, "SLIMGPU_Learn: G = R^T R is built by the tile kernel, which this matrix cannot use"};
  p.fn = p.use_gram ? gram_kernel(p.gram_nw, p.gram_v) : pick_kernel(p.use_lds, !m->binary);
  p.tileNW = (nwork + p.tileP - 1) / p.tileP >= 2 * m->num_cus ? 8 : 16;
  p.req_cluster = opt.cluster;
  if (opt.build_G && p.use_tile && p.tileP == 32 && m->binary && !std::getenv("SLIM_GPU_NO_GBITS")) {
    ensure_cluster_split(m, 5);
    const size_t need = sizeof(uint32_t) * (size_t)(round_up(m->split[5].max_rows, 64) + 64);
    size_t words_cap = 148 * 1024;
    if (test_hook("SLIM_GPU_TEST_GBITS_ROWS"))
      words_cap = sizeof(uint32_t) * (size_t)(round_up(std::max(64, std::atoi(std::getenv("SLIM_GPU_TEST_GBITS_ROWS"))), 64) + 64);
    if (need <= words_cap && m->num_cus >= 32) {
      p.gram_bits_lds = need;
      p.req_cluster = 32;
      p.tileNW = 16;
    } else if (m->num_cus >= 32 && !std::getenv("SLIM_GPU_NO_GPASSES")) {
      const int64_t rows_cap = (int64_t)(words_cap / sizeof(uint32_t)) - 128;
      int np = (int)((m->split[5].max_rows + rows_cap - 1) / rows_cap);
      for (; np <= 64; ++np) {
        ensure_split(m, m->gsplit, 32 * np, false);
        const size_t need_p = sizeof(uint32_t) * (size_t)(round_up(m->gsplit.max_rows, 64) + 64);
        if (need_p <= words_cap) {
          p.gram_bits_lds = need_p;
          p.req_cluster = 32;
          p.tileNW = 16;
          p.gram_passes = np;
          if (p.trace_level >= 1)
            std::fprintf(stderr, "[trace] G builder: %d user passes (32 members x %d users at most, %zu KB of words)\n",
                         np, m->gsplit.max_rows, need_p >> 10);
          break;
        }
      }
    }
  }
  if (const char* e = std::getenv("SLIM_GPU_TILE_NW")) p.tileNW = std::atoi(e) == 16 ? 16 : 8;
  if (warm_dev && warm_dev->device != m->device)
    throw Refusal{SLIM_ERROR_INPUT, "SLIMGPU_LearnResident: the warm-start model lives on another device"};
  p.has_imodel = warm_dev ? warm_dev->n > 0 : (imodel && imodel->colptr && imodel->ncols > 0);
  bool row_fold = true;
  if (const char* e = std::getenv("SLIM_GPU_FOLD")) row_fold = std::strcmp(e, "col") != 0;
  if (p.use_tile) {
    const bool prof = p.trace_level >= 2;
    const bool val = !m->binary;
    const bool nw16 = p.tileNW == 16;
    const char* form = "colfold";
    bool profiled = false;
    if (p.tileP == 32 && opt.nnbrs > 0) {
      p.fn = tile_kernel_p32_fslim(val, nw16);
      form = "fslim";
    } else if (p.tileP == 32 && !prof && !p.has_imodel) {
      p.fn = tile_kernel_p32_cold(val, nw16);
      form = "cold";
    } else if (p.tileP == 32 && !prof && row_fold) {
      p.fn = tile_kernel_p32_rowfold(val, nw16);
      form = "rowfold";
    } else if (p.tileP == 32) {
      p.fn = nw16 ? tile_kernel_p32_nw16(val, prof) : tile_kernel_p32_nw8(val, prof);
      profiled = prof;
    } else {
      p.fn = nw16 ? tile_kernel_p16_nw16(val, prof) : tile_kernel_p16_nw8(val, prof);
      profiled = prof;
    }
    if (p.trace_level >= 1)
      std::fprintf(stderr, "[trace] tile kernel: P %d, %d wavefronts, form %s, %s%s\n", p.tileP, nw16 ? 16 : 8,
                   form, val ? "valued" : "binary", profiled ? ", profiled" : "");
  }
  int waves_per_cu;
  if (p.use_gram) {
    int per_cu = 0;
    const void* kfn = p.use_gramr ? reinterpret_cast<const void*>(p.fn_r) : reinterpret_cast<const void*>(p.fn);
    HIP_TRY(hipFuncSetAttribute(kfn, hipFuncAttributeMaxDynamicSharedMemorySize, (int)p.gram_lds));
    HIP_TRY(hipOccupancyMaxActiveBlocksPerMultiprocessor(&per_cu, kfn, 64 * p.gram_nw, p.gram_lds));
    if (per_cu < 1)
      throw Refusal{SLIM_ERROR, "SLIMGPU_Learn: the item-space kernel does not fit a compute unit of this device"};
    waves_per_cu = per_cu;
  } else if (p.use_lds) {
    waves_per_cu = (int)std::min<size_t>(16, (160 * 1024) / std::max<size_t>(p.lds_need, 1));
    if (waves_per_cu < 1) waves_per_cu = 1;
    if (p.lds_need > 64 * 1024)
      HIP_TRY(hipFuncSetAttribute(reinterpret_cast<const void*>(p.fn),
                                  hipFuncAttributeMaxDynamicSharedMemorySize, (int)p.lds_need));
  } else {
    waves_per_cu = 8;
  }
  p.nwaves = std::max(1, std::min(nwork, m->num_cus * waves_per_cu));
  if (!p.use_gram && !p.use_tile && p.trace_level >= 1)
    std::fprintf(stderr, "[trace] wave kernel: %s, %s, sums %s, %d wavefronts, %zu bytes of LDS\n",
                 p.use_lds ? "lds" : "hbm", m->binary ? "binary" : "valued", p.exact_gram ? "ordered" : "atomic",
                 p.nwaves, p.use_lds ? p.lds_need : (size_t)0);
  p.wg_slots = m->num_cus * (16 / p.tileNW);
  if (p.use_tile) {
    int per_cu = 0;
    const size_t worst_lds = std::max<size_t>(kBitmapBytes, p.gram_bits_lds);
    HIP_TRY(hipFuncSetAttribute(reinterpret_cast<const void*>(p.fn),
                                hipFuncAttributeMaxDynamicSharedMemorySize, (int)worst_lds));
    HIP_TRY(hipOccupancyMaxActiveBlocksPerMultiprocessor(&per_cu, reinterpret_cast<const void*>(p.fn),
                                                         64 * p.tileNW, worst_lds));
    if (per_cu < 1)
      throw Refusal{SLIM_ERROR, "SLIMGPU_Learn: the tile kernel does not fit a compute unit of this device"};
    p.wg_slots = m->num_cus * std::min(per_cu, 16 / p.tileNW);
  }
}

struct TileGeom {
  bool force_k1 = false;
  int clusterK = 1, cluster_lg = 0, nclusters = 0;
  int clusterHi = 0, hi_lg = 0, nheavy = 0, nclusters_hi = 0;
  size_t tile_r = 0, tile_x = 0, tile_u = 0;
  int nwaves = 0;
};

TileGeom plan_tiles(slimgpu_matrix* m, const LearnOptions& opt, const Path& p,
                    const std::vector<int32_t>& order, bool force_k1) {
  const int32_t ncols = m->ncols, nwork = (int32_t)order.size();
  const int tileP = p.tileP;
  TileGeom t;
  t.force_k1 = force_k1;
  int auto_heavy = 0;
  const int ngroups_all = (nwork + tileP - 1) / tileP;
  const int req = p.req_cluster;
  if (force_k1) {
    t.clusterK = 1;
  } else if (req == 1 || req == 2 || req == 4 || req == 8 || req == 16 || req == 32) {
    t.clusterK = req;
  } else {
    int cap = 1;
    while (cap < 16 && (m->nnz / std::max(ncols, 1)) / (2 * cap) >= 512) cap *= 2;
    if (opt.heavy_tiles < 0 && p.tileNW == 16 && ngroups_all >= 16) {
      auto tile_cost = [&](int gI) {
        int64_t c = 0;
        for (int k = gI * tileP; k < std::min((gI + 1) * tileP, nwork); ++k) c += m->h_cost[order[(size_t)k]];
        return c;
      };
      const int64_t med = tile_cost(ngroups_all / 2);
      while (auto_heavy < ngroups_all / 16 && tile_cost(auto_heavy) >= 12 * med) ++auto_heavy;
    }
    const int64_t fill = auto_heavy > 0 ? 4 : 8;
    while (t.clusterK < cap && (int64_t)ngroups_all * t.clusterK < fill * (int64_t)p.wg_slots) t.clusterK *= 2;
  }
  while (t.clusterK > 1 && p.wg_slots / t.clusterK < 1) t.clusterK /= 2;
  for (t.cluster_lg = 0; (1 << t.cluster_lg) < t.clusterK; ++t.cluster_lg) {}
  ensure_cluster_split(m, t.cluster_lg);
  t.tile_r = (size_t)(round_up(m->split[t.cluster_lg].max_rows, 64) + 64) * tileP;
  if (opt.build_G && p.gram_bits_lds && t.clusterK == 32 && !force_k1) t.tile_r = (size_t)64 * tileP;
  t.tile_x = (size_t)p.ncols_pad * tileP;
  t.tile_u = (size_t)p.ncols_pad;
  t.nclusters = std::max(1, std::min(ngroups_all, p.wg_slots / t.clusterK));
  t.nheavy = std::min(opt.heavy_tiles < 0 ? auto_heavy : opt.heavy_tiles, ngroups_all);
  t.clusterHi = opt.heavy_cluster;
  if (const char* e = std::getenv("SLIM_GPU_HEAVY")) {
    int a = 0, b = 0;
    if (std::sscanf(e, "%d,%d", &a, &b) == 2) {
      t.nheavy = std::min(std::max(a, 0), ngroups_all);
      t.clusterHi = b;
    }
  }
  if (t.clusterHi != 2 && t.clusterHi != 4 && t.clusterHi != 8 && t.clusterHi != 16 && t.clusterHi != 32)
    t.clusterHi = std::max(16, std::min(4 * t.clusterK, kTileKMax));
  if (t.clusterHi <= t.clusterK || t.nclusters * t.clusterK < t.clusterHi || force_k1) t.nheavy = 0;
  if (t.nheavy > 0) {
    for (t.hi_lg = 0; (1 << t.hi_lg) < t.clusterHi; ++t.hi_lg) {}
    ensure_cluster_split(m, t.hi_lg);
    t.nclusters_hi = t.nclusters * t.clusterK / t.clusterHi;
    t.tile_r = std::max(t.tile_r, (size_t)(round_up(m->split[t.hi_lg].max_rows, 64) + 64) * tileP);
  }
  size_t free_b = 0, total_b = 0;
  HIP_TRY(hipMemGetInfo(&free_b, &total_b));
  const size_t per_cl = ((t.tile_r + 2 * t.tile_x) * sizeof(float) + t.tile_u * sizeof(int32_t)) * t.clusterK;
  const size_t have = free_b + m->ws_slab.bytes() + m->ws_xslab.bytes() + m->ws_ulist.bytes() +
                      m->ws_part.bytes() + m->ws_gram.bytes();
  const size_t budget = have > (size_t(6) << 30) ? have - (size_t(6) << 30) : have / 2;
  if ((size_t)t.nclusters * per_cl > budget) {
    t.nclusters = (int)std::max<size_t>(1, budget / per_cl);
    t.nclusters_hi = t.nclusters * t.clusterK / std::max(t.clusterHi, 1);
    if (t.nclusters_hi < 1) t.nheavy = 0;
  }
  t.nwaves = t.nclusters * t.clusterK;
  return t;
}

size_t mailbox_stride(int tileP) { return 2 * (size_t)kTileKMax * (size_t)tileP + 8; }

struct Slabs {
  float *slab = nullptr, *xslab = nullptr, *part = nullptr;
  int32_t *ulist = nullptr, *nunion = nullptr;
  unsigned long long* mailbox = nullptr;
  size_t mailbox_words = 0;
  int bm_shift = 0, bm_words = 1;
  size_t tile_lds = 0;
  int32_t *f_n = nullptr, *f_id = nullptr, *f_slot = nullptr;
  float* f_aty = nullptr;
  int f_slice_tiles = 0;
};

Slabs alloc_slabs(slimgpu_matrix* m, const LearnOptions& opt, const Path& p, const TileGeom& t, int32_t nwork,
                  int nwaves) {
  Slabs s;
  const auto evict = evict_cache(m);
  if (p.use_fgram) {
    const size_t ngroups0 = std::max<size_t>(1, ((size_t)nwork + 31) / 32);
    const size_t per_tile = (size_t)32 * (size_t)p.f_stride * 12;
    size_t free_b = 0, total_b = 0;
    HIP_TRY(hipMemGetInfo(&free_b, &total_b));
    const size_t have = free_b + m->ws_fid.bytes() + m->ws_faty.bytes() + m->ws_fslot.bytes();
    size_t tiles = ngroups0;
    if (tiles * per_tile > have / 4) tiles = std::max<size_t>(1, have / 4 / per_tile);
    if (const char* e = std::getenv("SLIM_GPU_FSLIM_SLICE_TILES"); e && std::atoi(e) > 0)
      tiles = std::min<size_t>(tiles, (size_t)std::atoi(e));
    s.f_slice_tiles = (int)tiles;
    const size_t npos = std::min<size_t>((size_t)std::max(nwork, 1), tiles * 32);
    s.f_n = m->ws_fn.reserve(npos, evict);
    s.f_id = m->ws_fid.reserve(npos * (size_t)p.f_stride, evict);
    s.f_aty = m->ws_faty.reserve(npos * (size_t)p.f_stride, evict);
    s.f_slot = m->ws_fslot.reserve(npos * (size_t)p.f_stride, evict);
    s.ulist = m->ws_ulist.reserve((size_t)p.f_ustride * tiles, evict);
    s.nunion = m->ws_nunion.reserve(tiles, evict);
  } else if (p.use_gram) {
    const size_t ngroups0 = ((size_t)nwork + 31) / 32;
    s.xslab = m->ws_xslab.reserve((size_t)p.ncols_pad * (size_t)nwaves, evict);
    if (p.gram_v == 0) s.slab = m->ws_slab.reserve((size_t)p.ncols_pad * (size_t)nwaves, evict);
    s.ulist = m->ws_ulist.reserve((size_t)p.ncols_pad * ngroups0, evict);
    s.nunion = m->ws_nunion.reserve(ngroups0, evict);
  } else if (p.use_tile) {
    s.mailbox_words = (size_t)(std::max(t.nclusters, 1) + t.nclusters_hi) * mailbox_stride(p.tileP);
    s.slab = m->ws_slab.reserve(t.tile_r * (size_t)nwaves, evict);
    s.xslab = m->ws_xslab.reserve(t.tile_x * (size_t)nwaves, evict);
    s.ulist = m->ws_ulist.reserve(t.tile_u * (size_t)nwaves, evict);
    s.mailbox = m->ws_mailbox.reserve(s.mailbox_words, evict);
    s.part = m->ws_part.reserve(t.tile_x * (size_t)nwaves, evict);
    const int64_t range = (int64_t)(t.tile_r / (size_t)p.tileP);
    auto words_at = [&](int sh) { return ((range >> sh) + 1 + 31) / 32; };
    while (words_at(s.bm_shift) * 4 > kBitmapBytes) ++s.bm_shift;
    s.bm_words = (int)words_at(s.bm_shift);
    if (opt.nnbrs > 0) s.bm_words = std::max(s.bm_words, p.tileP * 256);
    s.tile_lds = sizeof(uint32_t) * (size_t)s.bm_words;
    if (p.gram_bits_lds && t.clusterK == 32 && !t.force_k1) {
      s.bm_shift = 0;
      s.bm_words = (int)(p.gram_bits_lds / sizeof(uint32_t));
      s.tile_lds = p.gram_bits_lds;
    }
  } else if (!p.use_lds) {
    s.slab = m->ws_slab.reserve(p.vec_floats * (size_t)nwaves);
  }
  return s;
}

struct ArenaSeg {
  const int32_t* ind;
  const float* val;
  int64_t n;
  DeviceBuffer<int32_t> own_i;
  DeviceBuffer<float> own_v;
};

struct Launch {
  Path p;
  TileGeom t;
  Slabs s;
  int nwaves = 1;
  int32_t *order = nullptr, *cnt = nullptr, *sti = nullptr, *misc = nullptr;
  int64_t *off = nullptr, *stl = nullptr;
  float* stf = nullptr;
  const int64_t* icolptr = nullptr;
  const int32_t* icolind = nullptr;
  const float* icolval = nullptr;
  int32_t incols = 0;
  int gram_mode = 0;
  float* gram = nullptr;
  int gram_geom[6] = {0, 0, 0, 0, 0, 0};
  int gram_pass = 0;
  DeviceBuffer<float> carry;
  int64_t carry_stride = 0;
  bool carry_from_warm = false;
  bool cluster_fallback = false;
  int64_t arena_cap = 0;
  int32_t G_block = 0;
  bool gview_tried = false;
  const uint4* gview = nullptr;
  const int64_t* gview_base = nullptr;
  const uint16_t* gview_cnt = nullptr;
  int32_t gview_ngroups = 0, gview_sentinel = 0;
  size_t gview_bytes = 0;
  double gview_ms = 0;
  const char* gview_why = "";
};

void prepare_launch(slimgpu_matrix* m, const LearnOptions& opt, const std::vector<int32_t>& order,
                    const slim_csr_t* imodel, const slimgpu_model* warm_dev, bool resident, bool all_columns,
                    Launch& L) {
  const int32_t ncols = m->ncols, nwork = (int32_t)order.size();
  const Path& p = L.p;
  hipStream_t stream = m->stream;
  L.nwaves = p.nwaves;
  if (p.use_tile) {
    L.t = plan_tiles(m, opt, p, order, false);
    L.nwaves = L.t.nwaves;
  }
  L.order = m->ws_order.reserve((size_t)nwork);
  L.cnt = m->ws_cnt.reserve((size_t)ncols);
  L.off = m->ws_off.reserve((size_t)ncols);
  L.sti = m->ws_stat_i.reserve(3 * (size_t)ncols);
  L.stl = m->ws_stat_l.reserve(4 * (size_t)ncols);
  L.stf = m->ws_stat_f.reserve(2 * (size_t)ncols);
  L.misc = m->ws_misc.reserve(16);
  L.s = alloc_slabs(m, opt, p, L.t, nwork, L.nwaves);

  L.arena_cap = std::max<int64_t>(1 << 20, (int64_t)nwork * std::min<int64_t>(ncols, 8192));
  if (const char* env_cap = std::getenv("SLIM_GPU_ARENA")) L.arena_cap = std::max<int64_t>(1, std::atoll(env_cap));

  if (p.has_imodel && warm_dev) {
    L.incols = warm_dev->n;
    L.icolptr = warm_dev->d_colptr.get();
    L.icolind = warm_dev->d_colind.get();
    L.icolval = warm_dev->d_colval.get();
  } else if (p.has_imodel) {
    L.incols = imodel->ncols;
    const int64_t innz = imodel->colptr[L.incols];
    int64_t* cp = m->ws_icolptr.reserve((size_t)L.incols + 1);
    int32_t* ci = m->ws_icolind.reserve((size_t)innz);
    float* cv = m->ws_icolval.reserve((size_t)innz);
    HIP_TRY(hipMemcpyAsync(cp, imodel->colptr, sizeof(int64_t) * ((size_t)L.incols + 1),
                           hipMemcpyHostToDevice, stream));
    if (innz > 0) {
      HIP_TRY(hipMemcpyAsync(ci, imodel->colind, sizeof(int32_t) * (size_t)innz, hipMemcpyHostToDevice, stream));
      HIP_TRY(hipMemcpyAsync(cv, imodel->colval, sizeof(float) * (size_t)innz, hipMemcpyHostToDevice, stream));
    }
    L.icolptr = cp;
    L.icolind = ci;
    L.icolval = cv;
  }
  HIP_TRY(hipMemsetAsync(L.cnt, 0, sizeof(int32_t) * (size_t)ncols, stream));
  HIP_TRY(hipMemsetAsync(L.off, 0, sizeof(int64_t) * (size_t)ncols, stream));
  HIP_TRY(hipMemsetAsync(L.sti, 0, sizeof(int32_t) * 3 * (size_t)ncols, stream));
  HIP_TRY(hipMemsetAsync(L.stl, 0, sizeof(int64_t) * 4 * (size_t)ncols, stream));
  HIP_TRY(hipMemsetAsync(L.stf, 0, sizeof(float) * 2 * (size_t)ncols, stream));

  const TileGeom& t = L.t;
  const int geom[6] = {p.tileP, t.clusterK, t.nheavy > 0 ? t.clusterHi : 0, t.nheavy, opt.shard_count,
                       opt.shard_index};
  std::copy(geom, geom + 6, L.gram_geom);
  if (p.use_tile && !opt.build_G && !std::getenv("SLIM_GPU_NO_GRAM")) {
    const size_t ngroups0 = ((size_t)nwork + p.tileP - 1) / p.tileP;
    const size_t need = ngroups0 * t.tile_x * sizeof(float);
    if (!m->gram_order.empty() && m->gram_order == order && m->ws_gram.bytes() >= need &&
        std::equal(geom, geom + 6, m->gram_geom)) {
      L.gram_mode = 2;
      L.gram = m->ws_gram.get();
    } else {
      size_t free_b = 0, total_b = 0;
      HIP_TRY(hipMemGetInfo(&free_b, &total_b));
      if (need <= (size_t(32) << 30) && need <= (free_b + m->ws_gram.bytes()) / 4) {
        m->gram_order.clear();
        L.gram = m->ws_gram.reserve(need / sizeof(float));
        L.gram_mode = 1;
      }
    }
  }

  const int carry_groups = std::max(p.gramr_kr, 1) + p.gramr_kl;
  if (resident && p.use_gramr && carry_groups <= kGramrCarryMaxGroups && all_columns && nwork == ncols &&
      opt.shard_count == 1 && !std::getenv("SLIM_GPU_NO_CARRY")) {
    L.carry_stride = (int64_t)carry_groups * 8192;
    const size_t carry_bytes = sizeof(float) * (size_t)ncols * (size_t)L.carry_stride;
    if (warm_dev && warm_dev->d_gsave.get() && warm_dev->gsave_owner == m->uid &&
        warm_dev->gsave_stride == L.carry_stride && warm_dev->n == ncols) {
      L.carry_from_warm = warm_dev->gsave_valid && warm_dev->gsave_l1 == opt.l1r;
      L.carry = std::move(warm_dev->d_gsave);
      warm_dev->gsave_valid = false;
    } else {
      size_t free_b = 0, total_b = 0;
      HIP_TRY(hipMemGetInfo(&free_b, &total_b));
      if (carry_bytes <= (size_t(8) << 30) && carry_bytes * 4 <= free_b)
        L.carry = DeviceBuffer<float>((size_t)ncols * (size_t)L.carry_stride);
    }
  }
}

SolveArgs solve_args(slimgpu_matrix* m, const LearnOptions& opt, Launch& L, const std::vector<int32_t>& pending,
                     int attempt, int32_t* d_ai, float* d_av) {
  const Path& p = L.p;
  const TileGeom& t = L.t;
  const int32_t ncols = m->ncols, npend = (int32_t)pending.size();
  hipStream_t stream = m->stream;
  SolveArgs S;
  S.l1 = (float)opt.l1r;
  S.l2 = (float)opt.l2r;
  S.opt_tol = (float)opt.optTol;
  S.maxniters = opt.maxniters;
  S.seed = opt.seed;
  S.nnbrs = opt.nnbrs;
  S.simtype = opt.simtype;
  S.order = L.order;
  S.nwork = npend;
  S.queue = L.misc;
  S.icolptr = L.icolptr;
  S.icolind = L.icolind;
  S.icolval = L.icolval;
  S.incols = L.incols;
  S.slab = L.s.slab;
  S.slab_stride = p.use_tile ? (int64_t)t.tile_r : (int64_t)p.vec_floats;
  S.nrows_pad = p.nrows_pad;
  S.ncols_pad = p.ncols_pad;
  S.xslab = L.s.xslab;
  S.x_stride = (int64_t)t.tile_x;
  S.ulist = L.s.ulist;
  S.u_stride = (int64_t)t.tile_u;
  S.ngroups = (npend + p.tileP - 1) / p.tileP;
  if (opt.build_G && opt.G_rows_end >= 0) S.ngroups = (L.G_block + p.tileP - 1) / p.tileP;
  S.cluster = t.clusterK;
  S.ubounds = p.use_tile ? m->split[t.cluster_lg].ubounds.get() : nullptr;
  S.csplit = p.use_tile ? m->split[t.cluster_lg].csplit.get() : nullptr;
  S.mailbox = L.s.mailbox;
  S.exact_gram = p.exact_gram ? 1 : 0;
  S.atypart = L.s.part;
  S.bm_shift = L.s.bm_shift;
  S.bm_words = L.s.bm_words;
  S.nheavy = p.use_tile ? t.nheavy : 0;
  S.cluster_hi = t.clusterHi;
  S.ubounds_hi = t.nheavy > 0 ? m->split[t.hi_lg].ubounds.get() : nullptr;
  S.csplit_hi = t.nheavy > 0 ? m->split[t.hi_lg].csplit.get() : nullptr;
  S.mailbox_hi = L.s.mailbox ? L.s.mailbox + (size_t)std::max(t.nclusters, 1) * mailbox_stride(p.tileP) : nullptr;
  S.queue_hi = L.misc + 4;
  S.hi_prefetch = 1;
  S.shard_count = opt.shard_count;
  S.shard_index = opt.shard_index;
  S.nnz_last = m->nnz > 0 ? m->nnz - 1 : 0;
  S.xcd_swizzle = 0;
  S.gram_mode = (attempt == 0 && !L.cluster_fallback) ? L.gram_mode : 0;
  S.gram = L.gram;
  S.G = m->ws_G.get();
  S.G_ld = m->G_ld;
  S.tile_nunion = L.s.nunion;
  S.gram_pos = nullptr;
  S.gram_bits = (p.gram_bits_lds && t.clusterK == 32 && L.s.tile_lds == p.gram_bits_lds) ? 2 : 0;
  if (const char* e = std::getenv("SLIM_GPU_GBITS"); e && S.gram_bits) S.gram_bits = std::atoi(e) == 1 ? 1 : 2;
  S.gram_split_stride = t.clusterK + 1;
  S.gram_accum = 0;
  S.gview = nullptr;
  S.gview_base = nullptr;
  S.gview_cnt = nullptr;
  S.gview_ngroups = 0;
  S.gview_range0 = 0;
  S.gview_sentinel = 0;
  S.gram_part16 = S.gram_bits == 2 ? 1 : 0;
  if (const char* e = std::getenv("SLIM_GPU_GPART16"); e && std::atoi(e) == 0) S.gram_part16 = 0;
  S.g_save = nullptr;
  S.g_load = nullptr;
  S.g_stride = 0;
  if (L.carry.get()) {
    S.g_save = L.carry.get();
    S.g_stride = L.carry_stride;
    S.g_load = (L.carry_from_warm && attempt == 0) ? L.carry.get() : nullptr;
  }
  if (L.p.gram_passes > 1) {
    if (S.gram_bits) {
      S.ubounds = m->gsplit.ubounds.get() + 32 * L.gram_pass;
      S.csplit = m->gsplit.csplit.get() + 32 * L.gram_pass;
      S.gram_split_stride = 32 * L.p.gram_passes + 1;
      S.gram_accum = L.gram_pass > 0;
    } else {
      L.p.gram_passes = 1;
      L.gram_pass = 0;
    }
  }
  if (opt.build_G) {
    if (npend != ncols)
      throw Refusal{SLIM_ERROR, "SLIMGPU_Learn: internal: G = R^T R must be built over all columns at once"};
    std::vector<int32_t> pos((size_t)ncols, 0);
    for (int32_t k = 0; k < npend; ++k) pos[(size_t)pending[(size_t)k]] = k;
    int32_t* d_pos = m->ws_nunion.reserve((size_t)ncols, evict_cache(m));
    HIP_TRY(hipMemcpyAsync(d_pos, pos.data(), sizeof(int32_t) * (size_t)ncols, hipMemcpyHostToDevice, stream));
    HIP_TRY(hipStreamSynchronize(stream));
    S.gram_pos = d_pos;
    S.gram_mode = 3;
  }
  if (p.use_gram) {
    S.slab_stride = (int64_t)p.ncols_pad;
    S.x_stride = (int64_t)p.ncols_pad;
    S.u_stride = (int64_t)p.ncols_pad;
    S.ngroups = (npend + 31) / 32;
  }
  if (p.use_fgram) {
    S.u_stride = (int64_t)p.f_ustride;
    S.ngroups = (npend + 31) / 32;
  }
  if (const char* e = std::getenv("SLIM_GPU_HI_PREFETCH")) S.hi_prefetch = std::atoi(e);
  if (p.use_tile)
    HIP_TRY(hipMemsetAsync(L.s.mailbox, 0, sizeof(unsigned long long) * L.s.mailbox_words, stream));
  S.trace = nullptr;
  if (p.use_tile && p.trace_level >= 1) {
    S.trace = m->ws_trace.reserve(16 * (size_t)S.ngroups);
    HIP_TRY(hipMemsetAsync(S.trace, 0, sizeof(uint64_t) * 16 * (size_t)S.ngroups, stream));
  }
  S.out_cnt = L.cnt;
  S.out_off = L.off;
  S.out_ind = d_ai;
  S.out_val = d_av;
  S.out_cursor = reinterpret_cast<unsigned long long*>(L.misc + 2);
  S.out_cap = L.arena_cap;
  S.overflow = L.misc + 1;
  S.st_na = L.sti;
  S.st_sweeps = L.sti + ncols;
  S.st_conv = L.sti + 2 * (size_t)ncols;
  S.st_G = L.stl;
  S.st_D = L.stl + ncols;
  S.st_U = L.stl + 2 * (size_t)ncols;
  S.st_B = L.stl + 3 * (size_t)ncols;
  S.st_err = L.stf;
  S.st_obj = L.stf + ncols;
  return S;
}

void build_gview(slimgpu_matrix* m, Launch& L, const SolveArgs& S, const int32_t* d_colind) {
  L.gview_tried = true;
  if (const char* e = std::getenv("SLIM_GPU_GVIEW"); e && std::atoi(e) == 0) {
    L.gview_why = " (SLIM_GPU_GVIEW=0)";
    return;
  }
  hipStream_t stream = m->stream;
  const double t0 = now_ms();
  const int nranges = 32 * L.p.gram_passes;
  const int ngroups = (S.nwork + 63) / 64;
  const int sentinel = S.bm_words - 64;
  if ((int64_t)nranges * ngroups >= (int64_t(1) << 31) || sentinel >= 65536 || sentinel < 0) {
    L.gview_why = " (ranges beyond 16-bit ids)";
    return;
  }
  const int nblocks = nranges * ngroups;
  try {
    int32_t* d_rows = m->ws_gvrows.reserve((size_t)nblocks);
    int64_t* d_base = m->ws_gvbase.reserve((size_t)nblocks + 1);
    uint16_t* d_cnt = m->ws_gvcnt.reserve((size_t)nblocks * 64);
    const dim3 grid((unsigned)((nblocks + 3) / 4)), block(256);
    hipLaunchKernelGGL(k_gview_rows, grid, block, 0, stream, S.order, S.nwork, S.csplit, S.gram_split_stride, ngroups,
                       nblocks, d_rows, d_cnt);
    HIP_TRY(hipGetLastError());
    std::vector<int32_t> rows((size_t)nblocks);
    HIP_TRY(hipMemcpyAsync(rows.data(), d_rows, sizeof(int32_t) * rows.size(), hipMemcpyDeviceToHost, stream));
    HIP_TRY(hipStreamSynchronize(stream));
    std::vector<int64_t> base((size_t)nblocks + 1, 0);
    for (int b = 0; b < nblocks; ++b) base[(size_t)b + 1] = base[(size_t)b] + rows[(size_t)b];
    const int64_t total = base[(size_t)nblocks];
    uint4* d_view = m->ws_gview.reserve((size_t)std::max<int64_t>(total, 1), evict_cache(m));
    HIP_TRY(hipMemcpyAsync(d_base, base.data(), sizeof(int64_t) * base.size(), hipMemcpyHostToDevice, stream));
    hipLaunchKernelGGL(k_gview_fill, grid, block, 0, stream, S.order, S.nwork, S.csplit, S.gram_split_stride, S.ubounds,
                       d_colind, ngroups, nblocks, d_base, (uint32_t)sentinel, d_view);
    HIP_TRY(hipGetLastError());
    HIP_TRY(hipStreamSynchronize(stream));
    L.gview = d_view;
    L.gview_base = d_base;
    L.gview_cnt = d_cnt;
    L.gview_ngroups = ngroups;
    L.gview_sentinel = sentinel;
    L.gview_bytes = (size_t)total * 16;
    L.gview_ms = now_ms() - t0;
  } catch (const HipFail& e) {
    if (e.code != hipErrorOutOfMemory) throw;
    (void)hipGetLastError();
    m->ws_gview.reset();
    L.gview_why = " (no room for the 16-bit view)";
  }
}

void print_tile_trace(const slimgpu_matrix* m, const Launch& L, const SolveArgs& S, const std::vector<int32_t>& pending,
                      int launch_waves, float ms) {
  const int clusterK = L.t.clusterK, tileP = L.p.tileP, npend = (int)pending.size();
  std::vector<uint64_t> tr(16 * (size_t)S.ngroups);
  HIP_TRY(hipMemcpy(tr.data(), S.trace, sizeof(uint64_t) * tr.size(), hipMemcpyDeviceToHost));
  uint64_t t0 = ~0ull, t1 = 0;
  double busy = 0, setup = 0, sweeps = 0, fold = 0;
  std::vector<double> dur;
  for (int gI = 0; gI < S.ngroups; ++gI) {
    const uint64_t* e = &tr[8 * (size_t)gI];
    t0 = std::min(t0, e[0]);
    t1 = std::max(t1, e[3]);
    const double wk = double(e[6]) / clusterK;
    busy += double(e[3] - e[0]) * wk;
    setup += double(e[1] - e[0]) * wk;
    sweeps += double(e[2] - e[1]) * wk;
    fold += double(e[7] - e[1]) * wk;
    dur.push_back(double(e[3] - e[0]) * 1e-5);
  }
  std::sort(dur.begin(), dur.end());
  const double span = double(t1 - t0);
  std::fprintf(stderr,
               "[trace] tiles %d (%d heavy, clusters of %d) on %d workgroups (clusters of %d): span %.2f ms (event %.2f ms), busy/"
               "(span*wgs) %.2f, setup %.1f%% sweeps %.1f%% (fold %.1f%%) of busy; tile ms min %.2f med "
               "%.2f p90 %.2f max %.2f\n",
               S.ngroups, S.nheavy, S.nheavy > 0 ? L.t.clusterHi : 0, launch_waves, clusterK, span * 1e-5, ms,
               busy * clusterK / (span * launch_waves), 100 * setup / busy, 100 * sweeps / busy,
               100 * fold / busy,
               dur.front(), dur[dur.size() / 2], dur[dur.size() * 9 / 10], dur.back());
  if (S.ngroups >= 16) {
    std::fprintf(stderr, "[trace] tile cost -> ms, queue order:");
    for (int k = 0; k < 19; ++k) {
      const int gI = k < 12 ? k : (int)((int64_t)S.ngroups * (k - 11) / 8) - (k == 19 ? 1 : 0);
      if (gI >= S.ngroups) break;
      double c = 0;
      for (int j = gI * tileP; j < std::min((gI + 1) * tileP, npend); ++j)
        c += (double)m->h_cost[pending[(size_t)j]];
      std::fprintf(stderr, " [%d] %.3g -> %.0f", gI, c,
                   double(tr[8 * (size_t)gI + 3] - tr[8 * (size_t)gI]) * 1e-5);
    }
    std::fprintf(stderr, "\n");
  }
  if (L.p.trace_level >= 2) {
    double ph[7] = {0, 0, 0, 0, 0, 0, 0};
    for (int gI = 0; gI < S.ngroups; ++gI)
      for (int k = 0; k < 7; ++k) ph[k] += double(tr[8 * (size_t)S.ngroups + 8 * (size_t)gI + k]);
    const double tot = ph[0] + ph[1] + ph[2] + ph[3] + ph[4];
    std::fprintf(stderr,
                 "[trace] visit phases (shader clocks/visit): loads %.0f reduce+barrier %.0f "
                 "math %.0f stores %.0f closing barrier %.0f | total %.0f; visits %.0f, "
                 "%.1f%% with update\n",
                 ph[0] / ph[5], ph[1] / ph[5], ph[2] / ph[5], ph[3] / ph[5], ph[4] / ph[5],
                 tot / ph[5], ph[5], 100 * ph[6] / ph[5]);
  }
}

struct Entries {
  std::vector<int32_t> cnt;
  std::vector<int64_t> off;
  int64_t total = 0;
  std::vector<int32_t> ind;
  std::vector<float> val;
  std::vector<ArenaSeg> segs;
  double kernel_ms = 0, d2h_ms = 0;
};

Entries run_launches(slimgpu_matrix* m, const LearnOptions& opt, const std::vector<int32_t>& order, bool resident,
                     Launch& L) {
  const int32_t ncols = m->ncols;
  hipStream_t stream = m->stream;
  const Path& p = L.p;
  struct EventPair {
    hipEvent_t a = nullptr, b = nullptr;
    ~EventPair() {
      if (a) (void)hipEventDestroy(a);
      if (b) (void)hipEventDestroy(b);
    }
  } events;
  HIP_TRY(hipEventCreate(&events.a));
  HIP_TRY(hipEventCreate(&events.b));
  const hipEvent_t ev0 = events.a, ev1 = events.b;
  DevMatrix A;
  A.nrows = m->nrows;
  A.ncols = ncols;
  A.nnz = m->nnz;
  A.rowptr = m->d_rowptr;
  A.rowind = m->d_rowind;
  A.rowval = m->d_rowval;
  A.colptr = m->d_colptr.get();
  A.colind = m->d_colind.get();
  A.colval = m->d_colval.get();
  A.cnorm = m->d_cnorm.get();
  A.csq = m->d_csq.get();
  GramPacked P{};
  if (p.use_gramr) {
    P.lo = m->ws_Glo.get();
    P.ldb = m->Gp_ldb;
    P.hi = m->ws_Ghi.get();
    P.hi_off = m->ws_hioff.get();
    P.hi_k = m->ws_hik.get();
    P.hi2_off = m->ws_hi2off.get();
    P.hi2_k = m->ws_hi2k.get();
    P.base = m->ws_Gbase.get();
    P.diag = m->ws_Gdiag.get();
    P.meta = m->ws_Gmeta.get();
    P.rank_of = m->ws_rankof.get();
    P.item_of = m->ws_itemof.get();
    P.nchunks = m->Gp_nchunks;
  }

  struct DropView {
    slimgpu_matrix* m;
    ~DropView() {
      m->ws_gview.reset();
      m->ws_gvbase.reset();
      m->ws_gvrows.reset();
      m->ws_gvcnt.reset();
    }
  } drop_view{m};

  Entries E;
  E.cnt.assign((size_t)ncols, 0);
  E.off.assign((size_t)ncols, 0);
  std::vector<int32_t> h_cnt((size_t)ncols, 0);
  std::vector<int64_t> h_off((size_t)ncols, 0);
  std::vector<int32_t> pending = order;
  for (int attempt = 0; attempt < 8 && !pending.empty(); ++attempt) {
    const int32_t npend = (int32_t)pending.size();
    int32_t* d_ai = m->ws_arena_i.reserve((size_t)L.arena_cap, evict_cache(m));
    float* d_av = m->ws_arena_v.reserve((size_t)L.arena_cap, evict_cache(m));
    if (L.gram_mode != 0 && m->ws_gram.get() != L.gram) {
      L.gram_mode = 0;
      L.gram = nullptr;
    }
    HIP_TRY(hipMemcpyAsync(L.order, pending.data(), sizeof(int32_t) * (size_t)npend, hipMemcpyHostToDevice, stream));
    HIP_TRY(hipMemsetAsync(L.misc, 0, sizeof(int32_t) * 16, stream));
    if (attempt > 0) L.t.nheavy = 0;
    SolveArgs S = solve_args(m, opt, L, pending, attempt, d_ai, d_av);
    const int clusterK = L.t.clusterK;
    if (opt.build_G && S.gram_bits == 2 && !L.gview_tried) build_gview(m, L, S, A.colind);
    if (opt.build_G && S.gram_bits == 2 && L.gview) {
      S.gview = L.gview;
      S.gview_base = L.gview_base;
      S.gview_cnt = L.gview_cnt;
      S.gview_ngroups = L.gview_ngroups;
      S.gview_range0 = 32 * L.gram_pass;
      S.gview_sentinel = L.gview_sentinel;
    }
    if (opt.build_G && p.trace_level >= 1) {
      const bool in_passes = S.gram_bits != 0 && p.gram_passes > 1;
      std::fprintf(stderr, "[trace] G builder: form %s, clusters of %d, pass %d of %d, %d users at most per member\n",
                   S.gram_bits == 2 ? "bits2" : (S.gram_bits == 1 ? "bits1" : "lines"), clusterK, L.gram_pass + 1,
                   p.gram_passes, in_passes ? m->gsplit.max_rows : m->split[L.t.cluster_lg].max_rows);
      if (S.gview)
        std::fprintf(stderr, "[trace] G builder: ids from view, %zu bytes = %.3f x 2 bytes per nnz, built in %.1f ms\n",
                     L.gview_bytes, (double)L.gview_bytes / (2.0 * (double)std::max<int64_t>(m->nnz, 1)), L.gview_ms);
      else
        std::fprintf(stderr, "[trace] G builder: ids from csc%s\n", S.gram_bits == 2 ? L.gview_why : "");
    }

    const int launch_waves = p.use_tile ? std::max(1, std::min((npend + p.tileP - 1) / p.tileP, L.t.nclusters)) * clusterK
                                        : std::max(1, std::min(npend, L.nwaves));
    HIP_TRY(hipEventRecord(ev0, stream));
    if (p.use_gramr)
      hipLaunchKernelGGL(gramr_union_fn(), dim3(S.ngroups), dim3(gramr_union_threads()), 0, stream, A, S, P);
    else if (p.use_gram)
      hipLaunchKernelGGL(gram_union_fn(), dim3(S.ngroups), dim3(64), 0, stream, A, S);
    if (S.nheavy > 0 && launch_waves < L.t.clusterHi) S.nheavy = 0;
    int launch_now = launch_waves;
    if (p.use_tile && clusterK > 1 && !L.cluster_fallback && test_hook("SLIM_GPU_TEST_DROP_MEMBER")) {
      launch_now -= 1;
      S.nheavy = 0;
    }
    const int nxcd = m->num_cus % 32 == 0 ? m->num_cus / 32 : 1;
    if (p.use_tile && clusterK > 1 && nxcd == 8 && launch_now % 8 == 0 &&
        (launch_now / 8) % clusterK == 0 && (S.nheavy == 0 || (launch_now / 8) % L.t.clusterHi == 0)) {
      S.xcd_swizzle = 1;
      if (const char* e = std::getenv("SLIM_GPU_XCD")) S.xcd_swizzle = std::atoi(e) != 0;
    }
    if (p.use_fgram) {
      FslimArgs F{};
      F.stride = p.f_stride;
      F.nbr_n = L.s.f_n;
      F.nbr_id = L.s.f_id;
      F.nbr_aty = L.s.f_aty;
      F.nbr_slot = L.s.f_slot;
      F.wave_lds = (int32_t)p.f_wave_lds;
      F.tab_n = p.f_tab_n;
      const int slice = L.s.f_slice_tiles * 32;
      for (int pos0 = 0; pos0 < npend; pos0 += slice) {
        F.pos0 = pos0;
        F.npos = std::min(slice, npend - pos0);
        if (pos0 > 0) HIP_TRY(hipMemsetAsync(L.misc, 0, sizeof(int32_t), stream));
        hipLaunchKernelGGL(fslim_select_fn(), dim3(F.npos), dim3(kFslimSelectThreads), 0, stream, A, S, F);
        hipLaunchKernelGGL(fslim_union_fn(), dim3((F.npos + 31) / 32), dim3(kFslimUnionThreads), p.f_union_lds, stream,
                           A, S, F);
        hipLaunchKernelGGL(p.fn_f, dim3(std::max(1, std::min((F.npos + p.f_waves - 1) / p.f_waves, L.nwaves))),
                           dim3(64 * p.f_waves), p.f_wave_lds * (size_t)p.f_waves, stream, A, S, F);
        HIP_TRY(hipGetLastError());
      }
    } else if (p.use_gramr)
      hipLaunchKernelGGL(p.fn_r, dim3(launch_now), dim3(kGramrNT), p.gram_lds, stream, A, S, P);
    else
      hipLaunchKernelGGL(p.fn, dim3(launch_now), dim3(p.use_gram ? 64 * p.gram_nw : (p.use_tile ? 64 * p.tileNW : 64)),
                         p.use_gram ? p.gram_lds : (p.use_lds ? p.lds_need : (p.use_tile ? L.s.tile_lds : 0)),
                         stream, A, S);
    HIP_TRY(hipGetLastError());
    HIP_TRY(hipEventRecord(ev1, stream));

    int32_t h_misc[4];
    HIP_TRY(hipMemcpyAsync(h_misc, L.misc, sizeof(h_misc), hipMemcpyDeviceToHost, stream));
    HIP_TRY(hipMemcpyAsync(h_cnt.data(), L.cnt, sizeof(int32_t) * (size_t)ncols, hipMemcpyDeviceToHost, stream));
    HIP_TRY(hipMemcpyAsync(h_off.data(), L.off, sizeof(int64_t) * (size_t)ncols, hipMemcpyDeviceToHost, stream));
    HIP_TRY(hipStreamSynchronize(stream));
    float ms = 0;
    HIP_TRY(hipEventElapsedTime(&ms, ev0, ev1));
    E.kernel_ms += ms;
    if (S.trace) print_tile_trace(m, L, S, pending, launch_waves, ms);

    if (h_misc[1] == 2) {
      if (!L.cluster_fallback && (clusterK > 1 || L.t.nheavy > 0)) {
        L.cluster_fallback = true;
        std::fprintf(stderr, "[slim-gpu] tile cluster timed out (workgroups not co-resident); "
                             "re-solving %d columns without clusters\n", npend);
        L.t = plan_tiles(m, opt, p, order, true);
        L.nwaves = L.t.nwaves;
        L.s = alloc_slabs(m, opt, p, L.t, (int32_t)order.size(), L.nwaves);
        --attempt;
        continue;
      }
      throw Refusal{SLIM_ERROR, "SLIMGPU_Learn: a tile cluster timed out waiting for a member workgroup "
                                "(were all workgroups resident?)"};
    }
    if (p.gram_passes > 1 && ++L.gram_pass < p.gram_passes) {
      --attempt;
      continue;
    }
    if (S.gram_mode == 1) {
      m->gram_order = order;
      std::copy(L.gram_geom, L.gram_geom + 6, m->gram_geom);
    }
    unsigned long long cursor;
    std::memcpy(&cursor, h_misc + 2, sizeof(cursor));
    const int64_t used = std::min<int64_t>((int64_t)cursor, L.arena_cap);
    const int64_t base = E.total;
    const double t_d2h = now_ms();
    if (resident) {
      E.segs.push_back({d_ai, d_av, used, {}, {}});
    } else {
      E.ind.resize((size_t)(base + used));
      E.val.resize((size_t)(base + used));
      if (used > 0) {
        HIP_TRY(hipMemcpyAsync(E.ind.data() + base, d_ai, sizeof(int32_t) * (size_t)used, hipMemcpyDeviceToHost, stream));
        HIP_TRY(hipMemcpyAsync(E.val.data() + base, d_av, sizeof(float) * (size_t)used, hipMemcpyDeviceToHost, stream));
        HIP_TRY(hipStreamSynchronize(stream));
      }
    }
    E.d2h_ms += now_ms() - t_d2h;
    E.total += used;

    std::vector<int32_t> again;
    int64_t need = 0;
    for (int32_t c : pending) {
      if (h_cnt[c] >= 0) {
        E.cnt[c] = h_cnt[c];
        E.off[c] = base + h_off[c];
      } else {
        again.push_back(c);
        need += -(int64_t)h_cnt[c] - 1;
      }
    }
    pending.swap(again);
    if (!pending.empty()) L.arena_cap = std::max<int64_t>(L.arena_cap, need + 1024);
    if (resident && !pending.empty() && used > 0) {
      ArenaSeg& sg = E.segs.back();
      sg.own_i = DeviceBuffer<int32_t>((size_t)used);
      sg.own_v = DeviceBuffer<float>((size_t)used);
      HIP_TRY(hipMemcpyAsync(sg.own_i.get(), sg.ind, sizeof(int32_t) * (size_t)used, hipMemcpyDeviceToDevice, stream));
      HIP_TRY(hipMemcpyAsync(sg.own_v.get(), sg.val, sizeof(float) * (size_t)used, hipMemcpyDeviceToDevice, stream));
      HIP_TRY(hipStreamSynchronize(stream));
      sg.ind = sg.own_i.get();
      sg.val = sg.own_v.get();
    }
  }
  if (!pending.empty()) throw Refusal{SLIM_ERROR_MEMORY, "SLIMGPU_Learn: output arena overflow persisted"};
  return E;
}

struct Counters {
  std::vector<float> err, obj;
  int64_t gram_rows = 0;
  double gram_bytes = 0;
};

Counters read_counters(const slimgpu_matrix* m, const Launch& L, const std::vector<int32_t>& requested,
                       ColumnStats& cs) {
  const size_t ncols = (size_t)m->ncols;
  cs.nacols.assign(ncols, 0);
  cs.sweeps.assign(ncols, 0);
  cs.conv.assign(ncols, 0);
  cs.G.assign(ncols, 0);
  cs.D.assign(ncols, 0);
  cs.U.assign(ncols, 0);
  Counters k;
  k.err.resize(ncols);
  k.obj.resize(ncols);
  HIP_TRY(hipMemcpy(cs.nacols.data(), L.sti, sizeof(int32_t) * ncols, hipMemcpyDeviceToHost));
  HIP_TRY(hipMemcpy(cs.sweeps.data(), L.sti + ncols, sizeof(int32_t) * ncols, hipMemcpyDeviceToHost));
  HIP_TRY(hipMemcpy(cs.conv.data(), L.sti + 2 * ncols, sizeof(int32_t) * ncols, hipMemcpyDeviceToHost));
  HIP_TRY(hipMemcpy(cs.G.data(), L.stl, sizeof(int64_t) * ncols, hipMemcpyDeviceToHost));
  if (L.p.use_gram) {
    for (int32_t c : requested) k.gram_rows += cs.G[(size_t)c];
    if (L.p.use_gramr) {
      std::vector<int64_t> hb(ncols);
      HIP_TRY(hipMemcpy(hb.data(), L.stl + 3 * ncols, sizeof(int64_t) * ncols, hipMemcpyDeviceToHost));
      for (int32_t c : requested) k.gram_bytes += (double)hb[(size_t)c];
    } else {
      k.gram_bytes = (double)k.gram_rows * 4.0 * (double)L.p.ncols_pad;
    }
  }
  if (L.p.use_tile || L.p.use_gram || L.p.use_fgram)
    for (int32_t c : requested) cs.G[(size_t)c] = m->h_cost[(size_t)c];
  HIP_TRY(hipMemcpy(cs.D.data(), L.stl + ncols, sizeof(int64_t) * ncols, hipMemcpyDeviceToHost));
  HIP_TRY(hipMemcpy(cs.U.data(), L.stl + 2 * ncols, sizeof(int64_t) * ncols, hipMemcpyDeviceToHost));
  HIP_TRY(hipMemcpy(k.err.data(), L.stf, sizeof(float) * ncols, hipMemcpyDeviceToHost));
  HIP_TRY(hipMemcpy(k.obj.data(), L.stf + ncols, sizeof(float) * ncols, hipMemcpyDeviceToHost));
  return k;
}

slim_csr_t* assemble_host_model(int32_t ncols, const Entries& E, int64_t tnnz, bool row_view) {
  ssize_t* colptr = static_cast<ssize_t*>(std::malloc(sizeof(ssize_t) * ((size_t)ncols + 1)));
  int32_t* colind = static_cast<int32_t*>(std::malloc(sizeof(int32_t) * (size_t)std::max<int64_t>(tnnz, 1)));
  float* colval = static_cast<float*>(std::malloc(sizeof(float) * (size_t)std::max<int64_t>(tnnz, 1)));
  if (!colptr || !colind || !colval) {
    std::free(colptr); std::free(colind); std::free(colval);
    throw Refusal{SLIM_ERROR_MEMORY, "SLIMGPU_Learn: out of host memory for the model"};
  }
  colptr[0] = 0;
  for (int32_t c = 0; c < ncols; ++c) {
    const int64_t n = E.cnt[c];
    if (n > 0) {
      std::memcpy(colind + colptr[c], E.ind.data() + E.off[c], sizeof(int32_t) * (size_t)n);
      std::memcpy(colval + colptr[c], E.val.data() + E.off[c], sizeof(float) * (size_t)n);
    }
    colptr[c + 1] = colptr[c] + n;
  }
  return model_from_columns(ncols, colptr, colind, colval, row_view);
}

std::unique_ptr<slimgpu_model> assemble_resident_model(slimgpu_matrix* m, const LearnOptions& opt, Entries& E,
                                                       int64_t tnnz, Launch& L, bool row_view,
                                                       double* t_columns_done) {
  const int32_t ncols = m->ncols;
  hipStream_t stream = m->stream;
  std::unique_ptr<slimgpu_model> dm(new slimgpu_model());
  dm->device = m->device;
  dm->n = ncols;
  dm->nnz = tnnz;
  std::vector<int64_t> h_colptr((size_t)ncols + 1, 0);
  for (int32_t c = 0; c < ncols; ++c) h_colptr[(size_t)c + 1] = h_colptr[(size_t)c] + E.cnt[(size_t)c];
  const int32_t* src_i = E.segs.empty() ? nullptr : E.segs[0].ind;
  const float* src_v = E.segs.empty() ? nullptr : E.segs[0].val;
  DeviceBuffer<int32_t> cat_i;
  DeviceBuffer<float> cat_v;
  if (E.segs.size() > 1) {
    cat_i = DeviceBuffer<int32_t>((size_t)std::max<int64_t>(E.total, 1));
    cat_v = DeviceBuffer<float>((size_t)std::max<int64_t>(E.total, 1));
    int64_t at = 0;
    for (const ArenaSeg& sg : E.segs) {
      if (sg.n > 0) {
        HIP_TRY(hipMemcpyAsync(cat_i.get() + at, sg.ind, sizeof(int32_t) * (size_t)sg.n, hipMemcpyDeviceToDevice, stream));
        HIP_TRY(hipMemcpyAsync(cat_v.get() + at, sg.val, sizeof(float) * (size_t)sg.n, hipMemcpyDeviceToDevice, stream));
      }
      at += sg.n;
    }
    src_i = cat_i.get();
    src_v = cat_v.get();
  }
  dm->d_colptr = DeviceBuffer<int64_t>((size_t)ncols + 1);
  dm->d_colind = DeviceBuffer<int32_t>((size_t)std::max<int64_t>(tnnz, 1));
  dm->d_colval = DeviceBuffer<float>((size_t)std::max<int64_t>(tnnz, 1));
  int64_t* d_src = m->ws_off.reserve((size_t)ncols, evict_cache(m));
  HIP_TRY(hipMemcpyAsync(dm->d_colptr.get(), h_colptr.data(), sizeof(int64_t) * ((size_t)ncols + 1),
                         hipMemcpyHostToDevice, stream));
  HIP_TRY(hipMemcpyAsync(d_src, E.off.data(), sizeof(int64_t) * (size_t)ncols, hipMemcpyHostToDevice, stream));
  if (tnnz > 0) {
    hipLaunchKernelGGL(k_gather_columns, dim3(grid_for((int64_t)ncols * 64, 256, m->num_cus * 16)), dim3(256),
                       0, stream, ncols, dm->d_colptr.get(), d_src, src_i, src_v, dm->d_colind.get(),
                       dm->d_colval.get());
    HIP_TRY(hipGetLastError());
  }
  *t_columns_done = now_ms();
  if (row_view) {
    transpose_on_device(m, ncols, tnnz, dm->d_colptr.get(), dm->d_colind.get(), dm->d_colval.get(), dm->d_rowptr,
                        dm->d_rowind, dm->d_rowval);
    int32_t* d_facts = m->ws_misc.reserve(2);
    int32_t facts[2] = {0, 0};
    HIP_TRY(hipMemsetAsync(d_facts, 0, sizeof(facts), stream));
    queue_row_facts(stream, m->num_cus, ncols, dm->d_rowptr.get(), dm->d_rowind.get(), d_facts);
    HIP_TRY(hipMemcpyAsync(facts, d_facts, sizeof(facts), hipMemcpyDeviceToHost, stream));
    HIP_TRY(hipStreamSynchronize(stream));
    dm->max_row = facts[0];
    dm->rows_sorted = facts[1] == 0;
  }
  HIP_TRY(hipStreamSynchronize(stream));
  if (L.carry.get()) {
    dm->d_gsave = std::move(L.carry);
    dm->gsave_valid = true;
    dm->gsave_stride = L.carry_stride;
    dm->gsave_l1 = opt.l1r;
    dm->gsave_owner = m->uid;
  }
  return dm;
}

void print_progress(const slimgpu_matrix* m, const slim_csr_t* model, const std::vector<int32_t>& requested,
                    const ColumnStats& cs, const Counters& k) {
  const int32_t ncols = m->ncols;
  const ssize_t* colptr = model->colptr;
  const int32_t* colind = model->colind;
  const float* colval = model->colval;
  std::vector<int64_t> hp((size_t)m->nrows + 1);
  std::vector<int32_t> hi((size_t)std::max<int64_t>(m->nnz, 1));
  std::vector<float> hv(m->binary ? 0 : (size_t)std::max<int64_t>(m->nnz, 1));
  std::vector<int64_t> hcp((size_t)ncols + 1);
  HIP_TRY(hipMemcpy(hp.data(), m->d_rowptr, sizeof(int64_t) * hp.size(), hipMemcpyDeviceToHost));
  HIP_TRY(hipMemcpy(hcp.data(), m->d_colptr.get(), sizeof(int64_t) * hcp.size(), hipMemcpyDeviceToHost));
  if (m->nnz > 0) {
    HIP_TRY(hipMemcpy(hi.data(), m->d_rowind, sizeof(int32_t) * (size_t)m->nnz, hipMemcpyDeviceToHost));
    if (!m->binary)
      HIP_TRY(hipMemcpy(hv.data(), m->d_rowval, sizeof(float) * (size_t)m->nnz, hipMemcpyDeviceToHost));
  }
  std::vector<int32_t> sorted = requested;
  std::sort(sorted.begin(), sorted.end());
  std::vector<double> xd((size_t)ncols, 0.0);
  std::vector<float> scores;
  for (int32_t c : sorted) {
    double nrm1 = 0.0;
    for (ssize_t e = colptr[c]; e < colptr[c + 1]; ++e) {
      xd[(size_t)colind[e]] = colval[e];
      nrm1 += colval[e];
    }
    scores.clear();
    for (int32_t u = 0; u < m->nrows; ++u) {
      bool has = false;
      double r = 0.0;
      for (int64_t e = hp[(size_t)u]; e < hp[(size_t)u + 1]; ++e) {
        if (hi[(size_t)e] == c) has = true;
        r += xd[(size_t)hi[(size_t)e]] * (m->binary ? 1.0 : (double)hv[(size_t)e]);
      }
      if (!has) scores.push_back((float)r);
    }
    const size_t ntop = std::min<size_t>(10, scores.size());
    std::partial_sort(scores.begin(), scores.begin() + (ptrdiff_t)ntop, scores.end(), std::greater<float>());
    float a0 = 0.0f;
    for (size_t j = 0; j < ntop; ++j) a0 += scores[j];
    for (ssize_t e = colptr[c]; e < colptr[c + 1]; ++e) xd[(size_t)colind[e]] = 0.0;
    const size_t i = (size_t)c;
    std::printf("Col: %5d %5zd rs: %3d nits: %4d nnz: %4d rsd: %.2le obj: %.2le ff: %.3lf nrm1: "
                "%.3lf a0s: %.3lf tmr: %.2le\n",
                c, (ssize_t)(hcp[i + 1] - hcp[i]), cs.conv[i], cs.sweeps[i], (int)(colptr[c + 1] - colptr[c]),
                (double)k.err[i], (double)k.obj[i], k.obj[i] != 0 ? (double)k.err[i] / (double)k.obj[i] : 0.0,
                nrm1, ntop ? (double)a0 / (double)ntop : 0.0, 0.0);
  }
  std::fflush(stdout);
}

slimgpu_stats_t solve_stats(slimgpu_matrix* m, const Launch& L, const Entries& E, const Counters& k,
                            const ColumnStats& cs, const std::vector<int32_t>& requested, int64_t tnnz) {
  const Path& p = L.p;
  slimgpu_stats_t st;
  std::memset(&st, 0, sizeof(st));
  st.ncols_solved = (int32_t)requested.size();
  st.kernel = p.kernel;
  st.nwaves = L.nwaves;
  st.lds_bytes = p.use_lds ? (int32_t)p.lds_need : 0;
  st.setup_ms = m->setup_ms;
  st.kernel_ms = E.kernel_ms;
  for (int32_t c : requested) {
    st.G += cs.G[c];
    st.D += cs.D[c];
    st.U += cs.U[c];
    st.sweeps += cs.sweeps[c];
    st.error += k.err[c];
    st.objval += k.obj[c];
  }
  st.nnzW = tnnz;
  st.alg_bytes = m->binary ? 4.0 * st.G + 8.0 * st.D + 4.0 * st.U + 8.0 * st.nnzW
                           : 8.0 * st.G + 12.0 * st.D + 4.0 * st.U + 8.0 * st.nnzW;
  if (p.use_gram || p.use_fgram) {
    st.gram_build_ms = m->G_build_ms;
    st.gram_alloc_ms = m->G_alloc_ms;
    st.gram_sums_ms = m->G_sums_ms;
    st.gram_sums_kernel_ms = m->G_sums_kernel_ms;
    st.gram_pack_ms = m->G_pack_ms;
    m->G_build_ms = m->G_alloc_ms = m->G_sums_ms = m->G_sums_kernel_ms = m->G_pack_ms = 0.0;
  }
  st.gram_rows = k.gram_rows;
  st.gram_bytes = k.gram_bytes;
  return st;
}

}

slim_csr_t* learn_cd(slimgpu_matrix_t* m, const LearnOptions& opt, const slim_csr_t* imodel,
                     int32_t* status, const int32_t* columns, int32_t ncolumns, bool row_view,
                     ResidentIO* rio) {
  const double t_begin = now_ms();
  auto fail = [&](int32_t code) -> slim_csr_t* {
    if (status) *status = code;
    return nullptr;
  };
  if (!m) {
    set_error("SLIMGPU_Learn: null matrix");
    return fail(SLIM_ERROR_INPUT);
  }
  try {
    const WorkList w = work_list(m, opt, columns, ncolumns);
    const std::vector<int32_t>& requested = w.order;
    const int32_t nwork = (int32_t)requested.size();
    (void)hipGetLastError();
    HIP_TRY(hipSetDevice(m->device));
    static std::recursive_mutex device_lock[64];
    std::lock_guard<std::recursive_mutex> solve_guard(device_lock[m->device & 63]);

    const slimgpu_model* warm_dev = rio ? rio->warm : nullptr;
    const bool resident = rio && rio->out;
    const char* trace_env = std::getenv("SLIM_GPU_TRACE");
    Launch L;
    L.G_block = w.G_block;
    L.p = choose_kernel(m, opt, nwork);
    L.p.trace_level = trace_env ? std::atoi(trace_env) : 0;
    if ((L.p.use_gram || L.p.use_fgram) && !m->G_ready) {
      if (const int32_t st = gram_for_solve(m, opt, L.p.trace_level, L.p.use_fgram); st != SLIM_OK) return fail(st);
    }
    finish_path(m, opt, nwork, imodel, warm_dev, L.p);
    prepare_launch(m, opt, requested, imodel, warm_dev, resident, columns == nullptr, L);
    const double t_prep_done = now_ms();

    Entries E = run_launches(m, opt, requested, resident, L);
    const double t_kernel_done = now_ms();
    ColumnStats& cs = g_colstats;
    const Counters k = read_counters(m, L, requested, cs);
    const double t_counters_done = now_ms();
    int64_t tnnz = 0;
    for (int32_t c = 0; c < m->ncols; ++c) tnnz += E.cnt[c];
    slim_csr_t* model = nullptr;
    double t_columns_done = t_counters_done;
    if (resident) {
      *rio->out = assemble_resident_model(m, opt, E, tnnz, L, row_view, &t_columns_done).release();
    } else {
      model = assemble_host_model(m->ncols, E, tnnz, row_view);
      t_columns_done = now_ms();
    }
    if (L.p.trace_level >= 1)
      std::fprintf(stderr, "[slim_gpu trace] host phases: prep %.0f ms, launches + D2H %.0f ms (kernel %.0f, D2H of "
                   "%lld entries %.0f), counters %.0f ms, columns %.0f ms, row view %.0f ms\n",
                   t_prep_done - t_begin, t_kernel_done - t_prep_done, E.kernel_ms, (long long)E.total, E.d2h_ms,
                   t_counters_done - t_kernel_done, t_columns_done - t_counters_done, now_ms() - t_columns_done);
    if ((opt.dbglvl & SLIM_DBG_PROGRESS) && model) print_progress(m, model, requested, cs, k);

    slimgpu_stats_t st = solve_stats(m, L, E, k, cs, requested, tnnz);
    st.gather_ms = now_ms() - t_kernel_done;
    if (!opt.build_G) m->last_order = requested;
    st.total_ms = now_ms() - t_begin;
    g_stats = st;
    if (opt.dbglvl & SLIM_DBG_INFO)
      std::printf("Done estimation: loss: %.5le, fit: %.5le, ffrac: %.3lf,  #nzs: %zd\n", st.objval,
                  st.error, st.objval != 0 ? st.error / st.objval : 0.0, (ssize_t)tnnz);
    if (status) *status = SLIM_OK;
    return model;
  } catch (const Refusal& r) {
    set_error(r.msg);
    return fail(r.status);
  } catch (const HipFail& e) {
    report(e, "SLIMGPU_Learn");
    return fail(status_of(e));
  } catch (const std::bad_alloc&) {
    set_error("SLIMGPU_Learn: out of host memory");
    return fail(SLIM_ERROR_MEMORY);
  }
}

slimgpu_model* learn_resident(slimgpu_matrix_t* m, const LearnOptions& opt, const slimgpu_model* warm,
                              int32_t* status) {
  if (m && !m->replicas.empty()) {
    set_error("SLIMGPU_LearnResident: a model resident in HBM belongs to one device (ngpus = 1)");
    if (status) *status = SLIM_ERROR_INPUT;
    return nullptr;
  }
  slimgpu_model* out = nullptr;
  ResidentIO rio;
  rio.warm = warm;
  rio.out = &out;
  int32_t st = SLIM_ERROR;
  (void)learn_cd(m, opt, nullptr, &st, nullptr, 0, true, &rio);
  if (status) *status = st;
  if (st != SLIM_OK && out) {
    model_free(out);
    out = nullptr;
  }
  return out;
}

slimgpu_model* model_from_host(slimgpu_matrix_t* m, const slim_csr_t* W, int32_t* status) {
  auto fail = [&](int32_t st, const std::string& why) {
    set_error("SLIMGPU_ModelFromHost: " + why);
    if (status) *status = st;
    return static_cast<slimgpu_model*>(nullptr);
  };
  if (!m || !W || !W->rowptr || W->nrows < 0 || W->ncols < 0)
    return fail(SLIM_ERROR_INPUT, "bad arguments (a staged matrix, a model handle with a row view)");
  if (!m->replicas.empty()) return fail(SLIM_ERROR_INPUT, "a model resident in HBM belongs to one device (ngpus = 1)");
  const int32_t n = std::max(W->nrows, W->ncols);
  const int64_t nnz = W->rowptr[W->nrows];
  if (W->rowptr[0] != 0) return fail(SLIM_ERROR_INPUT, "the row pointer does not start at 0");
  for (int32_t r = 0; r < W->nrows; ++r)
    if (W->rowptr[r + 1] < W->rowptr[r]) return fail(SLIM_ERROR_INPUT, "the row pointer descends");
  if (nnz > 0 && (!W->rowind || !W->rowval)) return fail(SLIM_ERROR_INPUT, "the model has no values");
  for (int64_t j = 0; j < nnz; ++j)
    if (W->rowind[j] < 0 || W->rowind[j] >= n) return fail(SLIM_ERROR_INPUT, "an item id outside the model");
  try {
    (void)hipGetLastError();
    HIP_TRY(hipSetDevice(m->device));
    hipStream_t stream = m->stream;
    std::unique_ptr<slimgpu_model> dm(new slimgpu_model());
    dm->device = m->device;
    dm->n = n;
    dm->nnz = nnz;
    std::vector<int64_t> h_ptr((size_t)n + 1, nnz);
    for (int32_t r = 0; r <= W->nrows; ++r) h_ptr[(size_t)r] = W->rowptr[r];
    dm->d_rowptr = DeviceBuffer<int64_t>((size_t)n + 1);
    dm->d_rowind = DeviceBuffer<int32_t>((size_t)std::max<int64_t>(nnz, 1));
    dm->d_rowval = DeviceBuffer<float>((size_t)std::max<int64_t>(nnz, 1));
    HIP_TRY(hipMemcpyAsync(dm->d_rowptr.get(), h_ptr.data(), sizeof(int64_t) * ((size_t)n + 1), hipMemcpyHostToDevice,
                           stream));
    if (nnz > 0) {
      HIP_TRY(hipMemcpyAsync(dm->d_rowind.get(), W->rowind, sizeof(int32_t) * (size_t)nnz, hipMemcpyHostToDevice, stream));
      HIP_TRY(hipMemcpyAsync(dm->d_rowval.get(), W->rowval, sizeof(float) * (size_t)nnz, hipMemcpyHostToDevice, stream));
    }
    int32_t* d_facts = m->ws_misc.reserve(16);
    int32_t facts[2] = {0, 0};
    HIP_TRY(hipMemsetAsync(d_facts, 0, sizeof(facts), stream));
    queue_row_facts(stream, m->num_cus, n, dm->d_rowptr.get(), dm->d_rowind.get(), d_facts);
    HIP_TRY(hipMemcpyAsync(facts, d_facts, sizeof(facts), hipMemcpyDeviceToHost, stream));
    HIP_TRY(hipStreamSynchronize(stream));
    if (facts[1] != 0) return fail(SLIM_ERROR_INPUT, "the item ids of a model row do not ascend strictly");
    dm->max_row = facts[0];
    dm->rows_sorted = true;
    transpose_on_device(m, n, nnz, dm->d_rowptr.get(), dm->d_rowind.get(), dm->d_rowval.get(), dm->d_colptr,
                        dm->d_colind, dm->d_colval);
    HIP_TRY(hipStreamSynchronize(stream));
    if (status) *status = SLIM_OK;
    return dm.release();
  } catch (const HipFail& e) {
    report(e, "SLIMGPU_ModelFromHost");
    if (status) *status = status_of(e);
    return nullptr;
  } catch (const std::bad_alloc&) {
    return fail(SLIM_ERROR_MEMORY, "out of host memory");
  }
}

int32_t model_row_view(const slimgpu_model* w, DeviceRowView* out) {
  if (!w || !w->d_rowptr.get() || !out) {
    set_error("resident model: no row view");
    return SLIM_ERROR_INPUT;
  }
  out->nrows = out->ncols = w->n;
  out->nnz = w->nnz;
  out->max_row = w->max_row;
  out->rows_sorted = w->rows_sorted;
  out->device = w->device;
  out->d_ptr = w->d_rowptr.get();
  out->d_ind = w->d_rowind.get();
  out->d_val = w->d_rowval.get();
  return SLIM_OK;
}

int32_t matrix_csr_view(const slimgpu_matrix_t* m, DeviceCsrView* out) {
  if (!m || !m->d_rowptr || !out) {
    set_error("staged matrix: no CSR on the device");
    return SLIM_ERROR_INPUT;
  }
  out->device = m->device;
  out->stream = m->stream;
  out->num_cus = m->num_cus;
  out->nrows = m->nrows;
  out->ncols = m->ncols;
  out->nnz = m->nnz;
  out->merged = m->merged;
  out->d_ptr = m->d_rowptr;
  out->d_ind = m->d_rowind;
  out->d_val = m->binary ? nullptr : m->d_rowval;
  return SLIM_OK;
}

int64_t model_nnz(const slimgpu_model* w) { return w ? w->nnz : -1; }
int32_t model_ncols(const slimgpu_model* w) { return w ? w->n : -1; }

namespace {
void fetch_now(slimgpu_model* w) {
  const double t0 = now_ms();
  ssize_t *cp = nullptr, *rp = nullptr;
  int32_t *ci = nullptr, *ri = nullptr;
// ... 177 lines not shown
```

Before: 2048.

## Compact active columns into per-block list, overlap host ordering, hand model over on device

The solve kernel now builds a compacted list of nonzero columns with all waves in parallel and walks only that list in the final output phase. Before, it made a single-wave count pass and then a full scan over every column. The per-column accumulation moves into a lane-claim loop keyed by column. On the host, the popularity ordering is computed asynchronously while the Gram matrix is built. The model assembly gathers and transposes on the device and copies down through pinned bounce buffers with multiple threads. Statistics reads are batched, and a profiling path is added. These changes add memory for the column list and extra host threading complexity.

```diff
diff --git a/slim_amd/csrc/cd_gramr.hpp b/slim_amd/csrc/cd_gramr.hpp
--- a/slim_amd/csrc/cd_gramr.hpp
+++ b/slim_amd/csrc/cd_gramr.hpp
@@ -149,6 +149,7 @@
   __shared__ double s_e2[64], s_reg[64];
   __shared__ unsigned long long s_off;
   __shared__ int s_nz;
+  __shared__ int s_wnz[kGramrNT / 64], s_wkeep[kGramrNT / 64], s_pre[kGramrNT / 64 + 1], s_run[kGramrNT / 64], s_claim[64];
 
   const int tid = threadIdx.x;
   const int lane = tid & 63;
@@ -164,6 +165,7 @@
   const int64_t ld = S.G_ld;
 #endif
   float* const x = S.xslab + (int64_t)blockIdx.x * S.x_stride;
+  int* const kl = S.klist + (int64_t)blockIdx.x * S.x_stride;
 #if !SLIM_GRAMR_FROM_PLANES
   float4* const x4 = reinterpret_cast<float4*>(x);
 #endif
@@ -388,6 +390,10 @@
     __syncthreads();
     const int p = s_p;
     if (p >= S.nwork) break;
+#if SLIM_GRAMR_PROF
+    unsigned long long pt_setup = __builtin_readcyclecounter(), pt_count = 0, pt_out = 0;
+    bool pt_in_setup = true;
+#endif
     const int item = uni(S.order[p]);
     const int grp = p >> 5;
     const uint32_t gkey = (uint32_t)(grp * S.shard_count + S.shard_index);
@@ -553,7 +559,7 @@
       __builtin_amdgcn_global_load_lds(P.meta + i_n, hb + 256, 16, 0, 0);
       hw ^= 1;
     };
-    int ib = 0, wpos = 0, nz = 0;
+    int ib = 0, wpos = 0, nz = 0, nlist = 0;
     unsigned long long off = 0;
     bool fits = false;
     unsigned long long Uu = 0;
@@ -571,7 +577,7 @@
       int r = 0, i = 0;
       uint4 mrow = make_uint4(0u, 0u, 0u, 0u);
       float xi = kInactive;
-      bool part = false, keep = false;
+      bool part = false, keep = false, have = false;
       uint64_t mkeep = 0;
       if (phase == 1) {
         i = i_n;
@@ -593,18 +599,15 @@
         header_a(p0 + 128);
         want = part;
       } else if (phase == 2) {
-        i = ib + lane;
-        xi = i < ncols ? x[i] : kInactive;
-        const bool act = tile_active(xi);
-        keep = act && fabsf(xi) > kEps;
-        if (act && wave == 0)
-          s_reg[lane] += 0.5 * (double)l2 * (double)xi * (double)xi + (double)l1 * (double)fabsf(xi);
+        const int q = ib + lane;
+        have = q < nlist;
+        int w = 0;
+#pragma unroll
+        for (int u = 1; u < NT / 64; ++u) w += (int)(q >= s_pre[u]);
+        i = have ? kl[s_run[w] + q] : 0;
+        xi = have ? x[i] : kInactive;
+        keep = have && fabsf(xi) > kEps;
         mkeep = __ballot(keep);
-        if (mkeep == 0) {
-          ib += 64;
-          if (ib >= ncols) break;
-          continue;
-        }
         r = keep ? (int)(P.meta[i].x & 0x1FFFFu) : 0;
         want = keep;
       }
@@ -722,10 +725,10 @@
           ++t;
         }
       } else if (phase == 2) {
-        if (keep) {
+        if (wave == 0) {
+          float aty = 0.0f;
+          if (keep) {
 #if SLIM_GRAMR_FROM_PLANES
-          float aty = 0.0f;
-          if (wave == 0) {
             const int hk0 = (int)((irec.x >> 17) & 15u), h2k0 = (int)((irec.x >> 21) & 15u);
             const uint8_t* __restrict__ plo0 = P.lo + (int64_t)item * P.ldb;
             const uint8_t* __restrict__ phi0 = P.hi + (int64_t)irec.y * kPackGroup;
@@ -735,20 +738,30 @@
             aty = (float)plo0[r] + 16.0f * (float)pb0[((r >> 4) & (NT - 1)) * 16 + (r >> 13)];
             if (j1) aty = fmaf(256.0f, (float)phi0[r], aty);
             if (j2) aty = fmaf(65536.0f, (float)ph20[r], aty);
+#else
+            aty = arow[i];
+#endif
+            if (fits) {
+              const int64_t dst = (int64_t)off + wpos + __popcll(mkeep & ((1ull << lane) - 1ull));
+              S.out_ind[dst] = i;
+              S.out_val[dst] = xi;
+            }
           }
-          if (wave == 0) s_e2[lane] += (double)xi * ((double)aty + (double)g0);
-#else
-          if (wave == 0) s_e2[lane] += (double)xi * ((double)arow[i] + (double)g0);
-#endif
-          if (fits && wave == 0) {
-            const int64_t dst = (int64_t)off + wpos + __popcll(mkeep & ((1ull << lane) - 1ull));
-            S.out_ind[dst] = i;
-            S.out_val[dst] = xi;
+          const int key = i & 63;
+          bool pend = have;
+          while (__ballot(pend)) {
+            if (pend) s_claim[key] = 64;
+            if (pend) atomicMin(&s_claim[key], lane);
+            if (pend && s_claim[key] == lane) {
+              s_reg[key] += 0.5 * (double)l2 * (double)xi * (double)xi + (double)l1 * (double)fabsf(xi);
+              if (keep) s_e2[key] += (double)xi * ((double)aty + (double)g0);
+              pend = false;
+            }
           }
         }
         wpos += __popcll(mkeep);
         ib += 64;
-        if (ib >= ncols) break;
+        if (ib >= nlist) break;
         continue;
       }
       bool sweep = false;
@@ -763,6 +776,12 @@
         }
       }
       if (sweep) {
+#if SLIM_GRAMR_PROF
+        if (pt_in_setup) {
+          pt_setup = __builtin_readcyclecounter() - pt_setup;
+          pt_in_setup = false;
+        }
+#endif
         __syncthreads();
         phase = 1;
         p0 = 0;
@@ -773,27 +792,74 @@
         header_a(64);
         continue;
       }
-      if (wave == 0) {
-        int cnt = 0;
-        for (int jb = 0; jb < ncols; jb += 64) {
-          const int j = jb + lane;
-          const float xv = j < ncols ? x[j] : kInactive;
-          cnt += __popcll(__ballot(tile_active(xv) && fabsf(xv) > kEps));
+#if SLIM_GRAMR_PROF
+      if (pt_in_setup) {
+        pt_setup = __builtin_readcyclecounter() - pt_setup;
+        pt_in_setup = false;
+      }
+      pt_count = __builtin_readcyclecounter();
+#endif
+      __syncthreads();
+      int nc = ncols;
+      asm volatile("" : "+s"(nc));
+      const int nblk = (nc + 63) >> 6, bpw = (nblk + NT / 64 - 1) / (NT / 64);
+      {
+        const int lo = min(wave * bpw, nblk), hi = min(lo + bpw, nblk);
+        int* const klw = kl + lo * 64;
+        int cnz = 0, ckeep = 0;
+        for (int b = lo; b < hi; b += 4) {
+          float xv[4];
+#pragma unroll
+          for (int u = 0; u < 4; ++u) {
+            const int j = (b + u) * 64 + lane;
+            const bool in = b + u < hi && j < nc;
+            const float v = x[in ? j : 0];
+            xv[u] = in ? v : kInactive;
+          }
+#pragma unroll
+          for (int u = 0; u < 4; ++u) {
+            const bool nzf = tile_active(xv[u]) && xv[u] != 0.0f;
+            const uint64_t mnz = __ballot(nzf);
+            if (nzf) klw[cnz + __popcll(mnz & ((1ull << lane) - 1ull))] = (b + u) * 64 + lane;
+            cnz += __popcll(mnz);
+            ckeep += __popcll(__ballot(nzf && fabsf(xv[u]) > kEps));
+          }
         }
         if (lane == 0) {
-          s_off = atomicAdd(S.out_cursor, (unsigned long long)cnt);
-          s_nz = cnt;
-        }
+          s_wnz[wave] = cnz;
+          s_wkeep[wave] = ckeep;
+        }
+      }
+      __syncthreads();
+      if (tid == 0) {
+        int cnt = 0, at = 0;
+        for (int u = 0; u < NT / 64; ++u) {
+          s_pre[u] = at;
+          s_run[u] = min(u * bpw, nblk) * 64 - at;
+          at += s_wnz[u];
+          cnt += s_wkeep[u];
+        }
+        s_pre[NT / 64] = at;
+        s_off = atomicAdd(S.out_cursor, (unsigned long long)cnt);
+        s_nz = cnt;
       }
       __syncthreads();
       off = s_off;
       nz = s_nz;
+      nlist = s_pre[NT / 64];
       fits = (int64_t)(off + (unsigned long long)nz) <= S.out_cap;
       phase = 2;
       ib = 0;
       wpos = 0;
-      if (ncols <= 0) break;
-    }
+#if SLIM_GRAMR_PROF
+      pt_out = __builtin_readcyclecounter();
+      pt_count = pt_out - pt_count;
+#endif
+      if (nlist <= 0) break;
+    }
+#if SLIM_GRAMR_PROF
+    pt_out = __builtin_readcyclecounter() - pt_out;
+#endif
     if (kCarry && S.g_save != nullptr) {
       float4* __restrict__ gs = reinterpret_cast<float4*>(S.g_save + (int64_t)item * S.g_stride);
       static_for<KRA>([&](auto kc) __attribute__((always_inline)) {
@@ -835,8 +901,14 @@
         S.st_B[item] = (int64_t)nrows_read * (P.ldb + 16 * (int64_t)(nchunks < NT ? nchunks : NT)) + (int64_t)nhi16_read * 16 +
                        ((carried ? 4 : 0) + (kCarry && S.g_save != nullptr ? 4 : 0)) * S.g_stride;
 #endif
+#if SLIM_GRAMR_PROF
+        S.st_err[item] = (float)pt_setup;
+        S.st_obj[item] = (float)pt_count;
+        S.st_conv[item] = (int)(pt_out >> 8);
+#else
         S.st_err[item] = err;
         S.st_obj[item] = err + (float)reg;
+#endif
       }
     }
     __syncthreads();
diff --git a/slim_amd/csrc/cd_wave.hpp b/slim_amd/csrc/cd_wave.hpp
--- a/slim_amd/csrc/cd_wave.hpp
+++ b/slim_amd/csrc/cd_wave.hpp
@@ -78,6 +78,7 @@
   float* g_save;
   const float* g_load;
   int64_t g_stride;
+  int32_t* klist;
   int32_t* out_cnt;
   int64_t* out_off;
   int32_t* out_ind;
diff --git a/slim_amd/csrc/engine.hip b/slim_amd/csrc/engine.hip
--- a/slim_amd/csrc/engine.hip
+++ b/slim_amd/csrc/engine.hip
@@ -4,10 +4,12 @@
 #include <atomic>
 #include <chrono>
 #include <cmath>
+#include <condition_variable>
 #include <cstdio>
 #include <cstdlib>
 #include <cstring>
 #include <functional>
+#include <future>
 #include <mutex>
 #include <new>
 #include <numeric>
@@ -83,7 +85,7 @@
   double Gp_bytes_per_row = 0;
   int expect_solves = 0;
   std::vector<int32_t> last_order;
-  DeviceBuffer<int32_t> ws_order, ws_cnt, ws_stat_i, ws_misc, ws_arena_i, ws_ulist;
+  DeviceBuffer<int32_t> ws_order, ws_cnt, ws_stat_i, ws_misc, ws_arena_i, ws_ulist, ws_klist;
   DeviceBuffer<int64_t> ws_off, ws_stat_l, ws_icolptr;
   DeviceBuffer<float> ws_stat_f, ws_arena_v, ws_slab, ws_xslab, ws_part, ws_icolval;
   DeviceBuffer<int32_t> ws_fn, ws_fid, ws_fslot;
@@ -869,24 +871,40 @@
 
 namespace {
 
-bool pack_gram(slimgpu_matrix* m) {
+struct PopOrder {
+  std::vector<int32_t> item_of, rank_of;
+};
+PopOrder popularity_order(const std::vector<int64_t>& cp, int32_t ncols) {
+  const int32_t nchunks = (ncols + 15) / 16;
+  PopOrder o;
+  o.item_of.assign((size_t)nchunks * 16, -1);
+  o.rank_of.resize((size_t)ncols);
+  std::iota(o.item_of.begin(), o.item_of.begin() + ncols, 0);
+  std::stable_sort(o.item_of.begin(), o.item_of.begin() + ncols, [&](int32_t a, int32_t b) {
+    return cp[(size_t)a + 1] - cp[(size_t)a] > cp[(size_t)b + 1] - cp[(size_t)b];
+  });
+  for (int32_t r = 0; r < ncols; ++r) o.rank_of[(size_t)o.item_of[(size_t)r]] = r;
+  return o;
+}
+std::vector<int64_t> fetch_colptr(const slimgpu_matrix* m) {
+  std::vector<int64_t> cp((size_t)m->ncols + 1);
+  HIP_TRY(hipMemcpy(cp.data(), m->d_colptr.get(), sizeof(int64_t) * cp.size(), hipMemcpyDeviceToHost));
+  return cp;
+}
+
+bool pack_gram(slimgpu_matrix* m, std::future<PopOrder>* early = nullptr) {
   if (std::getenv("SLIM_GPU_NO_GRAMR")) return false;
   m->Gp_tried = true;
   const int32_t ncols = m->ncols;
   hipStream_t st = m->stream;
   const double t0 = now_ms();
-  std::vector<int64_t> cp((size_t)ncols + 1);
-  HIP_TRY(hipMemcpy(cp.data(), m->d_colptr.get(), sizeof(int64_t) * cp.size(), hipMemcpyDeviceToHost));
   const int32_t nchunks = (ncols + 15) / 16;
   static_assert(kGramrMaxGroups <= 15 && kGramrMaxGroups * kPackGroup <= (1 << 17),
                 "row record: 17 bits of rank, 4 bits per plane length; base bytes: 16 groups per thread");
   if ((nchunks + kGramrNT - 1) / kGramrNT > kGramrMaxGroups) return false;
-  std::vector<int32_t> item_of((size_t)nchunks * 16, -1), rank_of((size_t)ncols);
-  std::iota(item_of.begin(), item_of.begin() + ncols, 0);
-  std::stable_sort(item_of.begin(), item_of.begin() + ncols, [&](int32_t a, int32_t b) {
-    return cp[(size_t)a + 1] - cp[(size_t)a] > cp[(size_t)b + 1] - cp[(size_t)b];
-  });
-  for (int32_t r = 0; r < ncols; ++r) rank_of[(size_t)item_of[(size_t)r]] = r;
+  const PopOrder pop = early && early->valid() ? early->get() : popularity_order(fetch_colptr(m), ncols);
+  const std::vector<int32_t>& item_of = pop.item_of;
+  const std::vector<int32_t>& rank_of = pop.rank_of;
   int32_t* d_item_of = m->ws_itemof.reserve(item_of.size());
   int32_t* d_rank_of = m->ws_rankof.reserve(rank_of.size());
   HIP_TRY(hipMemcpyAsync(d_item_of, item_of.data(), sizeof(int32_t) * item_of.size(), hipMemcpyHostToDevice, st));
@@ -1154,6 +1172,9 @@
   bo.nnbrs = 0;
   bo.cluster = 0;
   bo.dbglvl = 0;
+  std::future<PopOrder> pop;
+  if (!floats_only && !m->Gp_ready && !std::getenv("SLIM_GPU_NO_GRAMR"))
+    pop = std::async(std::launch::async, [cp = fetch_colptr(m), ncols = m->ncols] { return popularity_order(cp, ncols); });
   double alloc_ms = 0;
   const int32_t st = build_gram(m, bo, true, &alloc_ms);
   if (st != SLIM_OK) return st;
@@ -1164,7 +1185,7 @@
   if (!floats_only) {
     if (!m->Gp_ready) {
       m->Gp_tried = false;
-      if (!pack_gram(m)) m->Gp_ready = false;
+      if (!pack_gram(m, &pop)) m->Gp_ready = false;
     }
     drop_float_gram(m);
   }
@@ -1446,6 +1467,7 @@
 struct Slabs {
   float *slab = nullptr, *xslab = nullptr, *part = nullptr;
   int32_t *ulist = nullptr, *nunion = nullptr;
+  int32_t* klist = nullptr;
   unsigned long long* mailbox = nullptr;
   size_t mailbox_words = 0;
   int bm_shift = 0, bm_words = 1;
@@ -1480,6 +1502,7 @@
   } else if (p.use_gram) {
     const size_t ngroups0 = ((size_t)nwork + 31) / 32;
     s.xslab = m->ws_xslab.reserve((size_t)p.ncols_pad * (size_t)nwaves, evict);
+    if (p.use_gramr) s.klist = m->ws_klist.reserve((size_t)p.ncols_pad * (size_t)nwaves, evict);
     if (p.gram_v == 0) s.slab = m->ws_slab.reserve((size_t)p.ncols_pad * (size_t)nwaves, evict);
     s.ulist = m->ws_ulist.reserve((size_t)p.ncols_pad * ngroups0, evict);
     s.nunion = m->ws_nunion.reserve(ngroups0, evict);
@@ -1709,6 +1732,7 @@
   S.g_save = nullptr;
   S.g_load = nullptr;
   S.g_stride = 0;
+  S.klist = L.s.klist;
   if (L.carry.get()) {
     S.g_save = L.carry.get();
     S.g_stride = L.carry_stride;
@@ -1887,8 +1911,27 @@
   std::vector<int32_t> ind;
   std::vector<float> val;
   std::vector<ArenaSeg> segs;
+  bool on_device = false;
   double kernel_ms = 0, d2h_ms = 0;
 };
+
+void fetch_segments(Entries& E, hipStream_t stream) {
+  const double t0 = now_ms();
+  E.ind.resize((size_t)E.total);
+  E.val.resize((size_t)E.total);
+  int64_t at = 0;
+  for (const ArenaSeg& sg : E.segs) {
+    if (sg.n > 0) {
+      HIP_TRY(hipMemcpyAsync(E.ind.data() + at, sg.ind, sizeof(int32_t) * (size_t)sg.n, hipMemcpyDeviceToHost, stream));
+      HIP_TRY(hipMemcpyAsync(E.val.data() + at, sg.val, sizeof(float) * (size_t)sg.n, hipMemcpyDeviceToHost, stream));
+    }
+    at += sg.n;
+  }
+  HIP_TRY(hipStreamSynchronize(stream));
+  E.segs.clear();
+  E.on_device = false;
+  E.d2h_ms += now_ms() - t0;
+}
 
 Entries run_launches(slimgpu_matrix* m, const LearnOptions& opt, const std::vector<int32_t>& order, bool resident,
                      Launch& L) {
@@ -1947,6 +1990,11 @@
   Entries E;
   E.cnt.assign((size_t)ncols, 0);
   E.off.assign((size_t)ncols, 0);
+  E.on_device = resident;
+  if (!resident) {
+    const char* e = std::getenv("SLIM_GPU_HANDOVER");
+    E.on_device = !(e && std::strcmp(e, "host") == 0);
+  }
   std::vector<int32_t> h_cnt((size_t)ncols, 0);
   std::vector<int64_t> h_off((size_t)ncols, 0);
   std::vector<int32_t> pending = order;
@@ -2070,7 +2118,7 @@
     const int64_t used = std::min<int64_t>((int64_t)cursor, L.arena_cap);
     const int64_t base = E.total;
     const double t_d2h = now_ms();
-    if (resident) {
+    if (E.on_device) {
       E.segs.push_back({d_ai, d_av, used, {}, {}});
     } else {
       E.ind.resize((size_t)(base + used));
@@ -2097,10 +2145,19 @@
     }
     pending.swap(again);
     if (!pending.empty()) L.arena_cap = std::max<int64_t>(L.arena_cap, need + 1024);
-    if (resident && !pending.empty() && used > 0) {
+    if (E.on_device && !pending.empty() && used > 0) {
       ArenaSeg& sg = E.segs.back();
-      sg.own_i = DeviceBuffer<int32_t>((size_t)used);
-      sg.own_v = DeviceBuffer<float>((size_t)used);
+      try {
+        sg.own_i = DeviceBuffer<int32_t>((size_t)used);
+        sg.own_v = DeviceBuffer<float>((size_t)used);
+      } catch (const HipFail& e) {
+        if (resident || e.code != hipErrorOutOfMemory) throw;
+        (void)hipGetLastError();
+        sg.own_i.reset();
+        sg.own_v.reset();
+        fetch_segments(E, stream);
+        continue;
+      }
       HIP_TRY(hipMemcpyAsync(sg.own_i.get(), sg.ind, sizeof(int32_t) * (size_t)used, hipMemcpyDeviceToDevice, stream));
       HIP_TRY(hipMemcpyAsync(sg.own_v.get(), sg.val, sizeof(float) * (size_t)used, hipMemcpyDeviceToDevice, stream));
       HIP_TRY(hipStreamSynchronize(stream));
@@ -2130,26 +2187,31 @@
   Counters k;
   k.err.resize(ncols);
   k.obj.resize(ncols);
-  HIP_TRY(hipMemcpy(cs.nacols.data(), L.sti, sizeof(int32_t) * ncols, hipMemcpyDeviceToHost));
-  HIP_TRY(hipMemcpy(cs.sweeps.data(), L.sti + ncols, sizeof(int32_t) * ncols, hipMemcpyDeviceToHost));
-  HIP_TRY(hipMemcpy(cs.conv.data(), L.sti + 2 * ncols, sizeof(int32_t) * ncols, hipMemcpyDeviceToHost));
-  HIP_TRY(hipMemcpy(cs.G.data(), L.stl, sizeof(int64_t) * ncols, hipMemcpyDeviceToHost));
+  const bool with_bytes = L.p.use_gram && L.p.use_gramr;
+  std::vector<int32_t> hi(3 * ncols);
+  std::vector<int64_t> hl((with_bytes ? 4 : 3) * ncols);
+  std::vector<float> hf(2 * ncols);
+  HIP_TRY(hipMemcpy(hi.data(), L.sti, sizeof(int32_t) * hi.size(), hipMemcpyDeviceToHost));
+  HIP_TRY(hipMemcpy(hl.data(), L.stl, sizeof(int64_t) * hl.size(), hipMemcpyDeviceToHost));
+  HIP_TRY(hipMemcpy(hf.data(), L.stf, sizeof(float) * hf.size(), hipMemcpyDeviceToHost));
+  std::copy(hi.begin(), hi.begin() + ncols, cs.nacols.begin());
+  std::copy(hi.begin() + ncols, hi.begin() + 2 * ncols, cs.sweeps.begin());
+  std::copy(hi.begin() + 2 * ncols, hi.end(), cs.conv.begin());
+  std::copy(hl.begin(), hl.begin() + ncols, cs.G.begin());
+  std::copy(hl.begin() + ncols, hl.begin() + 2 * ncols, cs.D.begin());
+  std::copy(hl.begin() + 2 * ncols, hl.begin() + 3 * ncols, cs.U.begin());
+  std::copy(hf.begin(), hf.begin() + ncols, k.err.begin());
+  std::copy(hf.begin() + ncols, hf.end(), k.obj.begin());
   if (L.p.use_gram) {
     for (int32_t c : requested) k.gram_rows += cs.G[(size_t)c];
     if (L.p.use_gramr) {
-      std::vector<int64_t> hb(ncols);
-      HIP_TRY(hipMemcpy(hb.data(), L.stl + 3 * ncols, sizeof(int64_t) * ncols, hipMemcpyDeviceToHost));
-      for (int32_t c : requested) k.gram_bytes += (double)hb[(size_t)c];
+      for (int32_t c : requested) k.gram_bytes += (double)hl[3 * ncols + (size_t)c];
     } else {
       k.gram_bytes = (double)k.gram_rows * 4.0 * (double)L.p.ncols_pad;
     }
   }
   if (L.p.use_tile || L.p.use_gram || L.p.use_fgram)
     for (int32_t c : requested) cs.G[(size_t)c] = m->h_cost[(size_t)c];
-  HIP_TRY(hipMemcpy(cs.D.data(), L.stl + ncols, sizeof(int64_t) * ncols, hipMemcpyDeviceToHost));
-  HIP_TRY(hipMemcpy(cs.U.data(), L.stl + 2 * ncols, sizeof(int64_t) * ncols, hipMemcpyDeviceToHost));
-  HIP_TRY(hipMemcpy(k.err.data(), L.stf, sizeof(float) * ncols, hipMemcpyDeviceToHost));
-  HIP_TRY(hipMemcpy(k.obj.data(), L.stf + ncols, sizeof(float) * ncols, hipMemcpyDeviceToHost));
   return k;
 }
 
@@ -2173,15 +2235,10 @@
   return model_from_columns(ncols, colptr, colind, colval, row_view);
 }
 
-std::unique_ptr<slimgpu_model> assemble_resident_model(slimgpu_matrix* m, const LearnOptions& opt, Entries& E,
-                                                       int64_t tnnz, Launch& L, bool row_view,
-                                                       double* t_columns_done) {
+void gather_columns_on_device(slimgpu_matrix* m, const Entries& E, int64_t tnnz, DeviceBuffer<int64_t>& o_ptr,
+                              DeviceBuffer<int32_t>& o_ind, DeviceBuffer<float>& o_val) {
   const int32_t ncols = m->ncols;
   hipStream_t stream = m->stream;
-  std::unique_ptr<slimgpu_model> dm(new slimgpu_model());
-  dm->device = m->device;
-  dm->n = ncols;
-  dm->nnz = tnnz;
   std::vector<int64_t> h_colptr((size_t)ncols + 1, 0);
   for (int32_t c = 0; c < ncols; ++c) h_colptr[(size_t)c + 1] = h_colptr[(size_t)c] + E.cnt[(size_t)c];
   const int32_t* src_i = E.segs.empty() ? nullptr : E.segs[0].ind;
@@ -2202,19 +2259,229 @@
     src_i = cat_i.get();
     src_v = cat_v.get();
   }
-  dm->d_colptr = DeviceBuffer<int64_t>((size_t)ncols + 1);
-  dm->d_colind = DeviceBuffer<int32_t>((size_t)std::max<int64_t>(tnnz, 1));
-  dm->d_colval = DeviceBuffer<float>((size_t)std::max<int64_t>(tnnz, 1));
+  o_ptr = DeviceBuffer<int64_t>((size_t)ncols + 1);
+  o_ind = DeviceBuffer<int32_t>((size_t)std::max<int64_t>(tnnz, 1));
+  o_val = DeviceBuffer<float>((size_t)std::max<int64_t>(tnnz, 1));
   int64_t* d_src = m->ws_off.reserve((size_t)ncols, evict_cache(m));
-  HIP_TRY(hipMemcpyAsync(dm->d_colptr.get(), h_colptr.data(), sizeof(int64_t) * ((size_t)ncols + 1),
+  HIP_TRY(hipMemcpyAsync(o_ptr.get(), h_colptr.data(), sizeof(int64_t) * ((size_t)ncols + 1),
                          hipMemcpyHostToDevice, stream));
   HIP_TRY(hipMemcpyAsync(d_src, E.off.data(), sizeof(int64_t) * (size_t)ncols, hipMemcpyHostToDevice, stream));
   if (tnnz > 0) {
     hipLaunchKernelGGL(k_gather_columns, dim3(grid_for((int64_t)ncols * 64, 256, m->num_cus * 16)), dim3(256),
-                       0, stream, ncols, dm->d_colptr.get(), d_src, src_i, src_v, dm->d_colind.get(),
-                       dm->d_colval.get());
+                       0, stream, ncols, o_ptr.get(), d_src, src_i, src_v, o_ind.get(), o_val.get());
     HIP_TRY(hipGetLastError());
   }
+  HIP_TRY(hipStreamSynchronize(stream));
+}
+
+struct Bounce {
+  char* slot[2] = {nullptr, nullptr};
+  hipEvent_t landed[2] = {nullptr, nullptr};
+  size_t chunk = 0;
+};
+constexpr size_t kBounceChunk = size_t(16) << 20;
+
+Bounce& bounce_for(int device) {
+  static Bounce all[64];
+  Bounce& b = all[device & 63];
+  size_t want = kBounceChunk;
+  if (const char* e = std::getenv("SLIM_GPU_HANDOVER_CHUNK")) want = (size_t)std::max<long long>(64, std::atoll(e));
+  want = (want + 63) & ~size_t(63);
+  if (b.chunk != want) {
+    for (int s = 0; s < 2; ++s) {
+      if (b.slot[s]) (void)hipHostFree(b.slot[s]);
+      b.slot[s] = nullptr;
+    }
+    b.chunk = 0;
+    for (int s = 0; s < 2; ++s) {
+      HIP_TRY(hipHostMalloc(reinterpret_cast<void**>(&b.slot[s]), want, hipHostMallocDefault));
+      if (!b.landed[s]) HIP_TRY(hipEventCreateWithFlags(&b.landed[s], hipEventDisableTiming));
+    }
+    b.chunk = want;
+  }
+  return b;
+}
+
+struct DownCopy {
+  void* dst;
+  const void* src;
+  size_t bytes;
+};
+void copy_down(hipStream_t stream, Bounce& b, const std::vector<DownCopy>& arrays) {
+  struct Piece {
+    char* dst;
+    const char* src;
+    size_t bytes;
+  };
+  std::vector<Piece> pieces;
+  size_t total = 0;
+  for (const DownCopy& a : arrays) {
+    for (size_t at = 0; at < a.bytes; at += b.chunk)
+      pieces.push_back({static_cast<char*>(a.dst) + at, static_cast<const char*>(a.src) + at, std::min(b.chunk, a.bytes - at)});
+    total += a.bytes;
+  }
+  const int64_t n = (int64_t)pieces.size();
+  if (n == 0) return;
+  const unsigned hw = std::thread::hardware_concurrency();
+  int T = total >= (size_t(8) << 22) ? (int)std::min<unsigned>(16u, std::max(1u, hw)) : 1;
+  if (const char* e = std::getenv("SLIM_GPU_HANDOVER_THREADS")) T = std::min(16, std::max(1, std::atoi(e)));
+  auto part = [&](const Piece& p, int t) {
+    const size_t per = ((p.bytes + (size_t)T - 1) / (size_t)T + 63) & ~size_t(63);
+    const size_t lo = std::min(p.bytes, per * (size_t)t), hi = std::min(p.bytes, lo + per);
+    return std::pair<size_t, size_t>(lo, hi);
+  };
+  struct Helpers {
+    std::mutex mu;
+    std::condition_variable cv;
+    int64_t ready = 0;
+    bool stop = false;
+    std::vector<int64_t> done;
+    std::vector<std::thread> th;
+    ~Helpers() {
+      {
+        std::lock_guard<std::mutex> g(mu);
+        stop = true;
+      }
+      cv.notify_all();
+      for (auto& x : th) x.join();
+    }
+  } H;
+  H.done.assign((size_t)T, 0);
+  for (int t = 1; t < T; ++t)
+    H.th.emplace_back([&, t]() {
+      for (int64_t k = 0; k < n; ++k) {
+        {
+          std::unique_lock<std::mutex> g(H.mu);
+          H.cv.wait(g, [&] { return H.stop || H.ready > k; });
+          if (H.ready <= k) return;
+        }
+        const auto [lo, hi] = part(pieces[(size_t)k], t);
+        if (hi > lo) std::memcpy(pieces[(size_t)k].dst + lo, b.slot[k & 1] + lo, hi - lo);
+        {
+          std::lock_guard<std::mutex> g(H.mu);
+          H.done[(size_t)t] = k + 1;
+        }
+        H.cv.notify_all();
+      }
+    });
+  auto left_slot = [&](int64_t k) {
+    std::unique_lock<std::mutex> g(H.mu);
+    H.cv.wait(g, [&] {
+      for (int t = 0; t < T; ++t)
+        if (H.done[(size_t)t] <= k) return false;
+      return true;
+    });
+  };
+  auto request = [&](int64_t k) {
+    HIP_TRY(hipMemcpyAsync(b.slot[k & 1], pieces[(size_t)k].src, pieces[(size_t)k].bytes, hipMemcpyDeviceToHost, stream));
+    HIP_TRY(hipEventRecord(b.landed[k & 1], stream));
+  };
+  request(0);
+  for (int64_t k = 0; k < n; ++k) {
+    if (k + 1 < n) {
+      if (k >= 1) left_slot(k - 1);
+      request(k + 1);
+    }
+    HIP_TRY(hipEventSynchronize(b.landed[k & 1]));
+    {
+      std::lock_guard<std::mutex> g(H.mu);
+      H.ready = k + 1;
+    }
+    H.cv.notify_all();
+    const auto [lo, hi] = part(pieces[(size_t)k], 0);
+    if (hi > lo) std::memcpy(pieces[(size_t)k].dst + lo, b.slot[k & 1] + lo, hi - lo);
+    {
+      std::lock_guard<std::mutex> g(H.mu);
+      H.done[0] = k + 1;
+    }
+    H.cv.notify_all();
+  }
+  left_slot(n - 1);
+}
+
+slim_csr_t* hand_over_on_device(slimgpu_matrix* m, const Entries& E, int64_t tnnz, bool row_view, int trace_level) {
+  const int32_t ncols = m->ncols;
+  hipStream_t stream = m->stream;
+  const double t0 = now_ms();
+  {
+    size_t free_b = 0, total_b = 0;
+    HIP_TRY(hipMemGetInfo(&free_b, &total_b));
+    const size_t held = m->ws_tkeys[0].bytes() + m->ws_tkeys[1].bytes() + m->ws_tpay[0].bytes() + m->ws_tpay[1].bytes();
+    const size_t need = (size_t)tnnz * (row_view ? 48 : 8) + (E.segs.size() > 1 ? (size_t)E.total * 8 : 0) + (size_t(1) << 30);
+    if (need > free_b + (row_view ? held : 0)) return nullptr;
+  }
+  struct HostArrays {
+    ssize_t *colptr = nullptr, *rowptr = nullptr;
+    int32_t *colind = nullptr, *rowind = nullptr;
+    float *colval = nullptr, *rowval = nullptr;
+    ~HostArrays() {
+      std::free(colptr); std::free(rowptr); std::free(colind); std::free(rowind); std::free(colval); std::free(rowval);
+    }
+  } h;
+  const size_t nz = (size_t)std::max<int64_t>(tnnz, 1);
+  h.colptr = static_cast<ssize_t*>(std::malloc(sizeof(ssize_t) * ((size_t)ncols + 1)));
+  h.colind = static_cast<int32_t*>(std::malloc(sizeof(int32_t) * nz));
+  h.colval = static_cast<float*>(std::malloc(sizeof(float) * nz));
+  if (row_view) {
+    h.rowptr = static_cast<ssize_t*>(std::malloc(sizeof(ssize_t) * ((size_t)ncols + 1)));
+    h.rowind = static_cast<int32_t*>(std::malloc(sizeof(int32_t) * nz));
+    h.rowval = static_cast<float*>(std::malloc(sizeof(float) * nz));
+  }
+  if (!h.colptr || !h.colind || !h.colval || (row_view && (!h.rowptr || !h.rowind || !h.rowval)))
+    throw Refusal{SLIM_ERROR_MEMORY, "SLIMGPU_Learn: out of host memory for the model"};
+  DeviceBuffer<int64_t> d_colptr, d_rowptr;
+  DeviceBuffer<int32_t> d_colind, d_rowind;
+  DeviceBuffer<float> d_colval, d_rowval;
+  try {
+    gather_columns_on_device(m, E, tnnz, d_colptr, d_colind, d_colval);
+    if (row_view) transpose_on_device(m, ncols, tnnz, d_colptr.get(), d_colind.get(), d_colval.get(), d_rowptr, d_rowind, d_rowval);
+    HIP_TRY(hipStreamSynchronize(stream));
+  } catch (const HipFail& e) {
+    if (e.code != hipErrorOutOfMemory) throw;
+    (void)hipGetLastError();
+    (void)hipStreamSynchronize(stream);
+    return nullptr;
+  }
+  const double t_views = now_ms();
+  static_assert(sizeof(ssize_t) == sizeof(int64_t), "the offsets come down as they are");
+  h.colptr[0] = 0;
+  for (int32_t c = 0; c < ncols; ++c) h.colptr[c + 1] = h.colptr[c] + E.cnt[(size_t)c];
+  Bounce& b = bounce_for(m->device);
+  std::vector<DownCopy> arrays;
+  arrays.push_back({h.colind, d_colind.get(), sizeof(int32_t) * (size_t)tnnz});
+  arrays.push_back({h.colval, d_colval.get(), sizeof(float) * (size_t)tnnz});
+  if (row_view) {
+    arrays.push_back({h.rowptr, d_rowptr.get(), sizeof(int64_t) * ((size_t)ncols + 1)});
+    arrays.push_back({h.rowind, d_rowind.get(), sizeof(int32_t) * (size_t)tnnz});
+    arrays.push_back({h.rowval, d_rowval.get(), sizeof(float) * (size_t)tnnz});
+  }
+  copy_down(stream, b, arrays);
+  HIP_TRY(hipStreamSynchronize(stream));
+  slim_csr_t* model = csr_new();
+  if (!model) throw Refusal{SLIM_ERROR_MEMORY, "SLIMGPU_Learn: out of host memory for the model"};
+  model->nrows = model->ncols = ncols;
+  model->colptr = std::exchange(h.colptr, nullptr);
+  model->colind = std::exchange(h.colind, nullptr);
+  model->colval = std::exchange(h.colval, nullptr);
+  model->rowptr = std::exchange(h.rowptr, nullptr);
+  model->rowind = std::exchange(h.rowind, nullptr);
+  model->rowval = std::exchange(h.rowval, nullptr);
+  if (trace_level >= 1)
+    std::fprintf(stderr, "[slim_gpu trace] hand-over on the device: views %.1f ms (gather%s), %lld entries down in %.1f ms "
+                 "(slots of %zu bytes)\n", t_views - t0, row_view ? " + transpose" : "", (long long)tnnz, now_ms() - t_views, b.chunk);
+  return model;
+}
+
+std::unique_ptr<slimgpu_model> assemble_resident_model(slimgpu_matrix* m, const LearnOptions& opt, Entries& E,
+                                                       int64_t tnnz, Launch& L, bool row_view,
+                                                       double* t_columns_done) {
+  const int32_t ncols = m->ncols;
+  hipStream_t stream = m->stream;
+  std::unique_ptr<slimgpu_model> dm(new slimgpu_model());
+  dm->device = m->device;
+  dm->n = ncols;
+  dm->nnz = tnnz;
+  gather_columns_on_device(m, E, tnnz, dm->d_colptr, dm->d_colind, dm->d_colval);
   *t_columns_done = now_ms();
   if (row_view) {
     transpose_on_device(m, ncols, tnnz, dm->d_colptr.get(), dm->d_colind.get(), dm->d_colval.get(), dm->d_rowptr,
@@ -2375,7 +2642,11 @@
     if (resident) {
       *rio->out = assemble_resident_model(m, opt, E, tnnz, L, row_view, &t_columns_done).release();
     } else {
-      model = assemble_host_model(m->ncols, E, tnnz, row_view);
+      if (E.on_device && tnnz > 0) model = hand_over_on_device(m, E, tnnz, row_view, L.p.trace_level);
+      if (!model) {
+        if (E.on_device) fetch_segments(E, m->stream);
+        model = assemble_host_model(m->ncols, E, tnnz, row_view);
+      }
       t_columns_done = now_ms();
     }
     if (L.p.trace_level >= 1)
```

Result: slower. 1797 (-12.2%).
